# LinXueyuanStdio/LaTeX_OCR

Measured on NVIDIA H100. Metric: formula-images/sec (train step, 128x512 px, seq<=150), higher is better.
Workload: dtype bf16

## Files before the change

### include/latex_ocr_b200.h

```cpp
#ifndef LATEX_OCR_B200_H
#define LATEX_OCR_B200_H

#include <stdint.h>

#ifdef __cplusplus
extern "C" {
#endif

#define LO_F32 0
#define LO_BF16 1

#define LO_OK 0
#define LO_EINVAL (-1)
#define LO_ECUDA (-2)
#define LO_ENOTSUP (-3)

#define LO_IMPL_SIMT 0
#define LO_IMPL_TC 1

int lo_version(void);
const char* lo_last_error(void);
int64_t lo_launch_count(void);
int lo_set_option(const char* name, int value);
int lo_get_option(const char* name);
const char* lo_option_name(int i);
int lo_set_l2_window(const void* base, int64_t bytes, float hit_ratio, void* stream);
int lo_debug_buffer(void* p);
int lo_tc_available(void);

int lo_gemm(const void* A, int dtA, const void* B, int dtB, void* C, int dtC,
            int M, int N, int K,
            int64_t sam, int64_t sak, int64_t sbk, int64_t sbn, int64_t ldc,
            int batch, int64_t sA, int64_t sB, int64_t sC,
            const float* bias, int accumulate, int relu, int impl, void* stream);

int lo_colsum(const void* X, int dt, float* out, int M, int N, int64_t ld, int accumulate, void* stream);

int lo_conv1_pool_forward(const float* img, const float* w, const float* bias, void* out, int dt,
                          int N, int H, int W, void* stream);
int lo_conv1_pool_forward_u8(const uint8_t* img, const float* w, const float* bias, void* out, int dt,
                             int N, int H, int W, void* stream);
int lo_conv1_pool_wgrad_u8(const uint8_t* img, const float* w, const float* bias, const void* dpool, int dt,
                           float* dw, float* db, int N, int H, int W, void* stream);
int lo_conv1_pool_wgrad(const float* img, const float* w, const float* bias, const void* dpool, int dt,
                        float* dw, float* db, int N, int H, int W, void* stream);
int lo_conv1_pool_forward_norm(const void* img, int img_is_u8, float scale, float offset, const float* w,
                               const float* bias, void* out, int dt, int N, int H, int W, void* stream);
int lo_conv1_pool_wgrad_norm(const void* img, int img_is_u8, float scale, float offset, const float* w,
                             const float* bias, const void* dpool, int dt, float* dw, float* db, int N, int H, int W,
                             void* stream);
int lo_conv1_pool_forward_code(const void* img, int img_is_u8, float scale, float offset, const float* w, const float* bias,
                               void* out, uint8_t* code, int dt, int N, int H, int W, void* stream);
int lo_conv1_pool_wgrad_code(const void* img, int img_is_u8, float scale, float offset, const uint8_t* code, const void* dpool,
                             int dt, float* dw, float* db, int N, int H, int W, void* stream);
int lo_conv1_pool_dgrad_code(const uint8_t* code, const void* dpool, int dt, const float* w, float scale, float* dimg,
                             int N, int H, int W, void* stream);
int lo_im2col(const void* x, void* col, int dt, int N, int H, int W, int C, int R, int S, int stride, int pad,
              void* stream);
int lo_col2im(const void* dcol, const void* mask, void* dx, int dt, int N, int H, int W, int C, int R, int S,
              int stride, int pad, void* stream);
int lo_transpose(const void* in, int64_t ld_in, void* out, int64_t ld_out, int dt, int K, int N, void* stream);
int lo_conv3x3(const void* x, const void* w, const float* bias, const void* mask, void* y, int dt,
               int N, int H, int W, int Cin, int Cout, int pad, int relu, int impl, void* stream);
int lo_conv3x3_wgrad(const void* x, const void* dy, float* dw, float* db, int dt,
                     int N, int H, int W, int Cin, int Cout, int pad, int impl, void* stream);
int lo_conv_weight_flip(const void* w, void* wt, int dt, int Cin, int Cout, void* stream);
int lo_maxpool_forward(const void* x, void* y, int dt, int N, int H, int W, int C, int kh, int kw, void* stream);
int lo_maxpool_backward(const void* x, const void* y, const void* dy, void* dx, int dt,
                        int N, int H, int W, int C, int kh, int kw, void* stream);
int lo_add_table(const void* y, const float* table, void* out, int dt, int N, int64_t HWC, void* stream);
int lo_relu_mask_cast(const float* g, const void* y, void* out, int dt, int64_t n, void* stream);

int64_t lo_attention_workspace_bytes(int B, int C);
int64_t lo_decoder_workspace_bytes(int B, int C);
int lo_attention_forward(const void* att1, const void* enc, int dt, const float* att2, int64_t att2_stride,
                         const float* wf, float* alpha, int64_t alpha_stride, float* ctx,
                         float* gate_pre, int64_t gate_stride, float* gctx,
                         int B, int R, int A, int C, void* work, void* stream);
int lo_attention_forward_mask(const void* att1, const void* enc, int dt, const float* att2, int64_t att2_stride,
                              const float* wf, float* alpha, int64_t alpha_stride, float* ctx,
                              float* gate_pre, int64_t gate_stride, float* gctx, uint8_t* relu_mask_out,
                              int B, int R, int A, int C, void* work, void* stream);

int lo_attention_backward(const void* att1, const void* enc, int dt, const float* att2, const float* gate, int64_t o1_stride,
                          const float* wf, const float* alpha, int64_t alpha_stride, const float* ctx, const float* dgctx,
                          int64_t dg_stride, const float* dreg, int64_t dreg_stride, const float* sreg, int64_t sreg_stride,
                          float* de, float* datt2, float* dgp, int64_t dcat_stride, float* dctx_out, float* dwf_part,
                          const uint8_t* relu_mask, int B, int R, int A, int C, void* work, void* stream);

int64_t lo_attention_step_workspace_bytes(int B, int R, int A, int C, int dt);
int lo_attention_step_backward(const void* enc, const void* att1, int dt, const float* h, const float* att2, const void* w_enc,
                               const void* w_dec, const float* wf, const float* alpha, const float* ctx, const float* dctx,
                               const float* dalpha, float* denc, float* dh, float* g_w_enc, float* g_b_enc, float* g_w_dec,
                               float* g_b_dec, float* g_w_full, float* g_b_full, float* de, float* datt2, void* datt1,
                               int B, int R, int A, int C, int D, int impl, void* work, void* stream);

typedef struct lo_decoder_args {
  int32_t B, T, R, C, A, D, E, V;
  int32_t dt;
  int32_t impl;
  int32_t has_dropout;
  int32_t ldl;
  float alpha_c;
  int32_t rows_per_img;
  int32_t phase;
  const int32_t* bt_host;
  const int64_t* caps;
  int64_t caps_stride;
  int64_t* fed;
  const float* ss_prob;
  const float* ss_u;
  const float* ss_temp;
  const float* ss_gu;
  const void* enc;
  const void* w_enc_att; const float* b_enc_att;
  const void* wcat1; const float* bcat1;
  const float* w_full;
  const void* emb;
  const void* w_ih; const float* b_ih;
  const void* w_init; const float* b_init;
  const void* w_fc; const float* b_fc;
  void* wbwd1;
  void* wbwd2;
  void* att1;
  float* ptab;
  float* mean;
  float* hall;
  float* call;
  float* out1;
  float* alphas;
  uint8_t* att_mask;
  float* ctx;
  float* gctx;
  float* gates;
  float* gtmp;
  const float* dropout_mask;
  const uint64_t* dropout_state;
  float dropout_p;
  float* hd;
  float* logits;
  float* row_loss;
  float* loss;
  float* dlogits;
  float* dhd;
  float* dreg;
  const float* dalpha_ext;
  const float* dpred_ext;
  int64_t dpred_stride;
  float* sreg;
  float* dcat;
  float* dxh;
  float* dc;
  float* dctx;
  float* de;
  float* dptab;
  void* datt1;
  float* denc;
  float* dinit;
  float* dmean;
  float* g_w_enc_att; float* g_b_enc_att;
  float* g_wcat1; float* g_bcat1;
  float* g_w_full; float* g_b_full;
  float* g_emb;
  float* g_w_ih; float* g_b_ih;
  float* g_w_init; float* g_b_init;
  float* g_w_fc; float* g_b_fc;
  const int32_t* reg_off;
  const int32_t* reg_off_host;
  void* work;
  void* bfwork;
} lo_decoder_args;

int64_t lo_decoder_bfwork_bytes(const lo_decoder_args* a);
int64_t lo_sizeof_decoder_args(void);
int lo_decoder_forward(const lo_decoder_args* a, int with_loss, void* stream);
int lo_decoder_backward(const lo_decoder_args* a, void* stream);
int lo_decoder_pack_bwd_weights(const lo_decoder_args* a, void* stream);

int lo_decoder_greedy(const lo_decoder_args* a, int64_t start_id, int64_t end_id, int max_steps,
                      int64_t* tokens, int32_t* finished, void* stream);
int lo_decoder_greedy_hist(const lo_decoder_args* a, int64_t start_id, int64_t end_id, int max_steps,
                           int64_t* tokens, int32_t* finished, int32_t* fin_hist, void* stream);

int lo_decoder_beam(const lo_decoder_args* a, int64_t start_id, int64_t end_id, int max_steps, int64_t* ids,
                    int64_t* parents, int32_t* fin_hist, float* logp, void* stream);
int lo_decoder_beam_div(const lo_decoder_args* a, int64_t start_id, int64_t end_id, int max_steps, int64_t* ids,
                        int64_t* parents, int32_t* fin_hist, float* logp, float div_gamma, float div_prob,
                        const float* div_u, const uint64_t* div_state, void* stream);

int lo_scst_edit_reward(const int64_t* hyp, int64_t hyp_stride, int Lh, const int64_t* greedy, int64_t greedy_stride, int Lg,
                        const int64_t* ref, int64_t ref_stride, int Lr, int B, int64_t end_id, float* r_sample, float* r_greedy,
                        float* adv, int32_t* n_len, void* stream);
int lo_scst_pg_grad(const float* preds, int64_t pred_stride, const int64_t* fed, int64_t fed_stride, const float* adv,
                    const int32_t* n_len, const float* temp, const float* r_sample, const float* r_greedy, int B, int T, int V,
                    float* dpred, int64_t dpred_stride, float* partial, float* stats, void* stream);
int lo_scst_edit_reward_tf(const int64_t* hyp, int64_t hyp_stride, int Lh, const int64_t* greedy, int64_t greedy_stride, int Lg,
                           const int64_t* ref, int64_t ref_stride, int Lr, int B, int64_t end_id, float* r_sample, float* r_greedy,
                           float* adv, int32_t* n_len, void* stream);
int lo_scst_pg_grad_tf(const float* logits, int64_t ldl, const int64_t* fed, int64_t fed_stride, const float* adv,
                       const int32_t* n_len, const float* temp, const float* r_sample, const float* r_greedy, int B, int T, int V,
                       float* dpred, int64_t dpred_stride, float* partial, float* stats, void* stream);

typedef struct lo_tfdec_args {
  int32_t B, T, R, C, A, D, O, E, V;
  int32_t dt;
  int32_t impl;
  int32_t ldl;
  int32_t rows_per_img;
  float inv_n_words;
  const void* enc;
  const int64_t* formula;
  int64_t formula_stride;
  const int32_t* lengths;
  const float* keep_h;
  const float* keep_o;
  const void* w_img;
  const void* w_cat2;
  const float* beta;
  const void* w_lstm;
  const float* b_lstm;
  const void* w_oc;
  const void* w_y;
  const void* w_init;
  const float* b_init;
  const void* emb;
  float* g_w_img; float* g_w_cat2; float* g_beta; float* g_w_lstm; float* g_b_lstm; float* g_w_oc; float* g_w_y;
  float* g_w_init; float* g_b_init; float* g_emb;
  float* logits;
  float* alphas;
  uint8_t* att_mask;
  float* loss;
  float* denc;
  int64_t* fed;
  const float* ss_prob;
  const float* ss_u;
  const float* ss_temp;
  const float* ss_gu;
  const uint64_t* ss_state;
  const int32_t* reg_off;
  const int32_t* reg_off_host;
  void* ws;
  const float* dlogits_ext;
  int64_t dlogits_stride;
  const float* dalpha_ext;
} lo_tfdec_args;

int64_t lo_sizeof_tfdec_args(void);
int64_t lo_tfdec_workspace_bytes(const lo_tfdec_args* a);
int lo_tfdec_forward(const lo_tfdec_args* a, int with_loss, void* stream);
int lo_tfdec_backward(const lo_tfdec_args* a, void* stream);
int lo_tfdec_greedy(const lo_tfdec_args* a, int64_t end_id, int max_steps, int64_t* tokens, int32_t* fin_hist, void* stream);
int lo_tfdec_beam(const lo_tfdec_args* a, int64_t end_id, int max_steps, int64_t* ids, int64_t* parents, int32_t* fin_hist,
                  float* logp, void* stream);
int lo_tfdec_beam_div(const lo_tfdec_args* a, int64_t end_id, int max_steps, int64_t* ids, int64_t* parents, int32_t* fin_hist,
                      float* logp, float div_gamma, float div_prob, const float* div_u, const uint64_t* div_state, void* stream);

typedef struct lo_lstm_seq_args {
  int32_t S, M, I, H;
  int32_t dt;
  int32_t impl;
  int32_t reverse;
  int32_t dx_accumulate;
  const void* x;
  int64_t x_row, x_step;
  const void* w_ih;
  const void* w_hh;
  const float* b_ih; const float* b_hh;
  const float* h0; const float* c0;
  float* hs;
  void* hs_st;
  int64_t hs_row, hs_step;
  const float* dhs;
  float* dx;
  int64_t dx_row, dx_step;
  float* g_w_ih; float* g_w_hh; float* g_b_ih; float* g_b_hh;
  float* dh0; float* dc0;
  void* ws;
} lo_lstm_seq_args;
int64_t lo_sizeof_lstm_seq_args(void);
int64_t lo_lstm_seq_workspace_bytes(const lo_lstm_seq_args* a);
int lo_lstm_seq_forward(const lo_lstm_seq_args* a, void* stream);
int lo_lstm_seq_backward(const lo_lstm_seq_args* a, void* stream);

int lo_adam_step(float* p, const float* g, float* m, float* v, void* shadow_bf16, int64_t n,
                 float* state_dev, float beta1, float beta2, float eps, float grad_scale, void* stream);
int lo_adam_step_ranges(float* p, const float* g, float* m, float* v, void* shadow_bf16, const int64_t* ranges,
                        int n_ranges, float* state_dev, float beta1, float beta2, float eps, float grad_scale,
                        void* stream);
int lo_tf_optim_step(int kind, float* p, const float* g, float* s1, float* s2, void* shadow_bf16, int64_t n,
                     float* state_dev, float beta1, float beta2, float eps, float grad_scale, void* stream);
int lo_cast(const void* src, int dt_src, void* dst, int dt_dst, int64_t n, void* stream);

#ifdef __cplusplus
}
#endif
#endif
```

### latex_ocr_b200/csrc/lo_common.cuh

```cuda
#pragma once
#include <cuda_runtime.h>
#include <cuda_bf16.h>
#include <stdint.h>
#include <stdio.h>
#include <string.h>

#include "../../include/latex_ocr_b200.h"

typedef __nv_bfloat16 bf16;

namespace lo {

extern char g_err[512];
extern int64_t g_launches;

inline int fail(int code, const char* fmt, const char* a = "", long b = 0, long c = 0) {
  snprintf(g_err, sizeof(g_err), fmt, a, b, c);
  return code;
}

#define LO_CHECK_ARG(cond, what)                                                        \
  do {                                                                                  \
    if (!(cond)) return lo::fail(LO_EINVAL, "%s: invalid argument: " what " (line %ld)", __func__, __LINE__); \
  } while (0)

#define LO_CUDA(call)                                                                   \
  do {                                                                                  \
    cudaError_t e__ = (call);                                                           \
    if (e__ != cudaSuccess)                                                             \
      return lo::fail(LO_ECUDA, "%s: CUDA error %ld at line %ld", cudaGetErrorString(e__), (long)e__, __LINE__); \
  } while (0)

#define LO_LAUNCH_OK()                                                                  \
  do {                                                                                  \
    lo::g_launches++;                                                                   \
    cudaError_t e__ = cudaGetLastError();                                               \
    if (e__ != cudaSuccess)                                                             \
      return lo::fail(LO_ECUDA, "%s: launch failed (%ld) at line %ld", cudaGetErrorString(e__), (long)e__, __LINE__); \
  } while (0)

#define LO_TRY(call)                                                                    \
  do {                                                                                  \
    int r__ = (call);                                                                   \
    if (r__ != LO_OK) return r__;                                                       \
  } while (0)

inline int cdiv(long a, long b) { return (int)((a + b - 1) / b); }

constexpr int LO_NUM_SMS = 132;

#define LO_OPTIONS(X)                                                                                           \
  X(g_opt_att_pipe, "att_pipe", 1)                 \
  X(g_opt_pdl, "pdl", 1)                                                   \
  X(g_opt_att_abi_pdl, "att_abi_pdl", 0)             \
  X(g_opt_att_l2_keep_mb, "att_l2_keep_mb", 24)    \
  X(g_opt_att_nsplit, "att_nsplit", 0)                       \
  X(g_opt_att_cluster, "att_cluster", 1)                      \
  X(g_opt_att_maskbits, "att_maskbits", 1)                 \
  X(g_opt_att_bwd_mma, "att_bwd_mma", 1)                     \
  X(g_opt_dec_streams, "dec_streams", 1)             \
  X(g_opt_dec_fuse, "dec_fuse", 0)                                        \
  X(g_opt_dec_fuse_bwd, "dec_fuse_bwd", 0)                               \
  X(g_opt_dec_cl, "dec_cl", 0)                                                 \
  X(g_opt_dec_cl_bwd, "dec_cl_bwd", 0)                                        \
  X(g_opt_fuse_lstm, "fuse_lstm", 0)                               \
  X(g_opt_skinny_mma, "skinny_mma", 1)                               \
  X(g_opt_skinny_tma, "skinny_tma", 1)                                    \
  X(g_opt_skinny8, "skinny8", 1)                                        \
  X(g_opt_conv_persist, "conv_persist", 1)                      \
  X(g_opt_conv_mt2, "conv_mt2", 1)                            \
  X(g_opt_conv_mc, "conv_mc", 1)                                     \
  X(g_opt_wgrad256, "wgrad256", 0)                                   \
  X(g_opt_det, "deterministic", 0)                                             \
  X(g_opt_dbg_skip, "dbg_skip", 0)                                  \
  X(g_opt_l2_persist_mb, "l2_persist_mb", 0)

#define LO_OPTION_EXTERN(var, name, def) extern int var;
LO_OPTIONS(LO_OPTION_EXTERN)
#undef LO_OPTION_EXTERN

template <typename... KArgs, typename... Args>
inline cudaError_t launch_pdl(void (*kernel)(KArgs...), dim3 grid, dim3 block, size_t smem, cudaStream_t st, Args... args) {
  cudaLaunchConfig_t cfg{};
  cfg.gridDim = grid;
  cfg.blockDim = block;
  cfg.dynamicSmemBytes = smem;
  cfg.stream = st;
  cudaLaunchAttribute attr[1];
  attr[0].id = cudaLaunchAttributeProgrammaticStreamSerialization;
  attr[0].val.programmaticStreamSerializationAllowed = 1;
  cfg.attrs = attr;
  cfg.numAttrs = g_opt_pdl ? 1 : 0;
  return cudaLaunchKernelEx(&cfg, kernel, KArgs(args)...);
}
template <typename... KArgs, typename... Args>
inline cudaError_t launch_cluster(void (*kernel)(KArgs...), dim3 grid, dim3 block, size_t smem, cudaStream_t st, dim3 cl, bool pdl,
                                  Args... args) {
  cudaLaunchConfig_t cfg{};
  cfg.gridDim = grid;
  cfg.blockDim = block;
  cfg.dynamicSmemBytes = smem;
  cfg.stream = st;
  cudaLaunchAttribute attr[2];
  int n = 0;
  attr[n].id = cudaLaunchAttributeClusterDimension;
  attr[n].val.clusterDim.x = cl.x;
  attr[n].val.clusterDim.y = cl.y;
  attr[n].val.clusterDim.z = cl.z;
  n++;
  if (pdl && g_opt_pdl) {
    attr[n].id = cudaLaunchAttributeProgrammaticStreamSerialization;
    attr[n].val.programmaticStreamSerializationAllowed = 1;
    n++;
  }
  cfg.attrs = attr;
  cfg.numAttrs = n;
  return cudaLaunchKernelEx(&cfg, kernel, KArgs(args)...);
}

__device__ __forceinline__ float ldf(const float* p) { return *p; }
__device__ __forceinline__ float ldf(const bf16* p) { return __bfloat162float(*p); }
__device__ __forceinline__ void stf(float* p, float v) { *p = v; }
__device__ __forceinline__ void stf(bf16* p, float v) { *p = __float2bfloat16_rn(v); }
__device__ __forceinline__ float roundto(float v, const float*) { return v; }
__device__ __forceinline__ float roundto(float v, const bf16*) { return __bfloat162float(__float2bfloat16_rn(v)); }

__device__ __forceinline__ void ld8(const float* p, float* v) {
  float4 a = *reinterpret_cast<const float4*>(p);
  float4 b = *reinterpret_cast<const float4*>(p + 4);
  v[0] = a.x; v[1] = a.y; v[2] = a.z; v[3] = a.w; v[4] = b.x; v[5] = b.y; v[6] = b.z; v[7] = b.w;
}
__device__ __forceinline__ void ld8(const bf16* p, float* v) {
  uint4 u = *reinterpret_cast<const uint4*>(p);
  const uint32_t w[4] = {u.x, u.y, u.z, u.w};
#pragma unroll
  for (int i = 0; i < 4; i++) {
    v[2 * i] = __uint_as_float(w[i] << 16);
    v[2 * i + 1] = __uint_as_float(w[i] & 0xffff0000u);
  }
}
__device__ __forceinline__ void lds8(uint32_t saddr, float* v, const float*) {
  float4 a, b;
  asm volatile("ld.shared.v4.f32 {%0, %1, %2, %3}, [%4];" : "=f"(a.x), "=f"(a.y), "=f"(a.z), "=f"(a.w) : "r"(saddr));
  asm volatile("ld.shared.v4.f32 {%0, %1, %2, %3}, [%4];" : "=f"(b.x), "=f"(b.y), "=f"(b.z), "=f"(b.w) : "r"(saddr + 16));
  v[0] = a.x; v[1] = a.y; v[2] = a.z; v[3] = a.w; v[4] = b.x; v[5] = b.y; v[6] = b.z; v[7] = b.w;
}
__device__ __forceinline__ void lds8(uint32_t saddr, float* v, const bf16*) {
  uint32_t w[4];
  asm volatile("ld.shared.v4.b32 {%0, %1, %2, %3}, [%4];" : "=r"(w[0]), "=r"(w[1]), "=r"(w[2]), "=r"(w[3]) : "r"(saddr));
#pragma unroll
  for (int i = 0; i < 4; i++) {
    v[2 * i] = __uint_as_float(w[i] << 16);
    v[2 * i + 1] = __uint_as_float(w[i] & 0xffff0000u);
  }
}
__device__ __forceinline__ void st8(float* p, const float* v) {
  *reinterpret_cast<float4*>(p) = make_float4(v[0], v[1], v[2], v[3]);
  *reinterpret_cast<float4*>(p + 4) = make_float4(v[4], v[5], v[6], v[7]);
}
__device__ __forceinline__ void st8(bf16* p, const float* v) {
  uint32_t w[4];
#pragma unroll
  for (int i = 0; i < 4; i++) {
    __nv_bfloat162 h = __floats2bfloat162_rn(v[2 * i], v[2 * i + 1]);
    w[i] = *reinterpret_cast<uint32_t*>(&h);
  }
  *reinterpret_cast<uint4*>(p) = make_uint4(w[0], w[1], w[2], w[3]);
}

__device__ __forceinline__ float warp_sum(float v) {
#pragma unroll
  for (int o = 16; o > 0; o >>= 1) v += __shfl_xor_sync(0xffffffffu, v, o);
  return v;
}
__device__ __forceinline__ float warp_max(float v) {
#pragma unroll
  for (int o = 16; o > 0; o >>= 1) v = fmaxf(v, __shfl_xor_sync(0xffffffffu, v, o));
  return v;
}
__device__ __forceinline__ float sigmoidf_(float x) { return 1.0f / (1.0f + expf(-x)); }

__device__ __forceinline__ uint4 philox4x32_10(uint4 c, uint2 k) {
#pragma unroll
  for (int r = 0; r < 10; r++) {
    const uint32_t hi0 = __umulhi(0xD2511F53u, c.x), lo0 = 0xD2511F53u * c.x;
    const uint32_t hi1 = __umulhi(0xCD9E8D57u, c.z), lo1 = 0xCD9E8D57u * c.z;
    c = make_uint4(hi1 ^ c.y ^ k.x, lo1, hi0 ^ c.w ^ k.y, lo0);
    k.x += 0x9E3779B9u;
    k.y += 0xBB67AE85u;
  }
  return c;
}
__device__ __forceinline__ float u01(uint32_t x) { return (float)(x >> 8) * (1.0f / 16777216.0f); }
__device__ __forceinline__ float philox_dropout_mult(const unsigned long long* state, int b, int t, int j, float p, float scale) {
  const unsigned long long seed = state[0], call = state[1];
  const uint4 r = philox4x32_10(make_uint4((uint32_t)(j >> 2), (uint32_t)t, (uint32_t)b, (uint32_t)call),
                                make_uint2((uint32_t)seed, (uint32_t)(seed >> 32)));
  const uint32_t w = (j & 3) == 0 ? r.x : ((j & 3) == 1 ? r.y : ((j & 3) == 2 ? r.z : r.w));
  return u01(w) >= p ? scale : 0.f;
}

#define LO_DISPATCH_DT(dt, T, ...)                   \
  do {                                               \
    if ((dt) == LO_F32) { typedef float T; __VA_ARGS__; } \
    else if ((dt) == LO_BF16) { typedef bf16 T; __VA_ARGS__; } \
    else return lo::fail(LO_EINVAL, "%s: bad dtype %ld", __func__, (long)(dt)); \
  } while (0)

struct GemmDesc {
  int M, N, K;
  int64_t sam, sak, sbk, sbn, ldc;
  int batch;
  int64_t sA, sB, sC;
  const float* bias;
  int accumulate, relu;
};
int gemm(const void* A, int dtA, const void* B, int dtB, void* C, int dtC, const GemmDesc& d, int impl, cudaStream_t st);
int gemm_nt(const void* A, int dtA, int64_t lda, const void* W, int dtW, int64_t ldw, void* C, int dtC, int64_t ldc,
            int M, int N, int K, const float* bias, int accumulate, int relu, int impl, cudaStream_t st);
int gemm_tn(const void* A, int dtA, int64_t lda, const void* B, int dtB, int64_t ldb, void* C, int dtC, int64_t ldc,
            int M, int N, int K, int accumulate, int impl, cudaStream_t st);
int gemm_nn(const void* A, int dtA, int64_t lda, const void* B, int dtB, int64_t ldb, void* C, int dtC, int64_t ldc,
            int M, int N, int K, int accumulate, int impl, cudaStream_t st);
int colsum(const void* X, int dt, float* out, int M, int N, int64_t ld, int accumulate, cudaStream_t st);

struct AttFwdArgs {
  const void *att1, *enc;
  const float* att2; int64_t att2_stride;
  const float* wf;
  float* alpha; int64_t alpha_stride;
  float* ctx; float* gate_pre; int64_t gate_stride; float* gctx; bf16* gctx_bf;
  int B, R;
  void* work;
  int rows_per_img;
  int nsplit_hint;
  int act;
  int a_ch;
  uint8_t* mask_out;
  int abi = 0;
};
struct AttBwdArgs {
  const void *att1, *enc;
  const float *att2, *gate; int64_t o1_stride;
  const float* wf; const float* alpha; int64_t alpha_stride;
  const float* ctx; const float* dgctx; int64_t dg_stride;
  const float* dreg; int64_t dreg_stride; const float* sreg; int64_t sreg_stride;
  float* de; float* datt2; float* dgp; int64_t dcat_stride; bf16* datt2_bf; bf16* dgp_bf; float* dctx_out;
  int B, R;
  void* work;
  float* dwf_part;
  int nsplit_hint;
  int act;
  int a_ch;
  const uint8_t* mask_in;
  int abi = 0;
  void* datt1 = nullptr;
  int ordered_dwf = 0;
};
int attention_fwd_pipe(const AttFwdArgs& x, int dt, int C, cudaStream_t st);
int attention_bwd_pipe(const AttBwdArgs& x, int dt, int C, cudaStream_t st);
inline int64_t att_partials_offset(int B) { return B <= 1024 ? 4096 : ((int64_t)B * 4 + 255) / 256 * 256; }
struct AttRagged {
  const int32_t* reg_off;
  const int32_t* reg_off_host;
  void* map;
  int ctas;
};
int64_t attention_ragged_map_bytes(int B);
int attention_ragged_prepare(AttRagged& rg, int B, int rpi, cudaStream_t st);
int attention_fwd_ragged(const AttFwdArgs& x, const AttRagged& rg, int dt, int C, cudaStream_t st);

bool tc_available();
int tc_gemm_nt(const bf16* A, int64_t lda, const bf16* W, int64_t ldw, void* C, int dtC, int64_t ldc,
               int M, int N, int K, const float* bias, int accumulate, int relu, cudaStream_t st);
int tc_gemm_nt_ex(const bf16* A, int64_t lda, const bf16* W, int64_t ldw, void* C, int dtC, int64_t ldc, int M, int N, int K,
                  const float* bias, int accumulate, int relu, int splits, int atomic_acc, int small_n_tile, cudaStream_t st);
struct TcLstmEpi {
  const float* ptab; const int64_t* tok; int64_t tok_stride;
  const float* hh; int64_t hh_stride;
  const float* c_prev; float* gates; float* c_out; float* h_out; bf16* h_bf;
  float* hd; int64_t hd_stride; const float* dmask;
  int D, V;
  const unsigned long long* dstate; float dp; int row0, t_idx;
};
struct DecStepFwd {
  const bf16* gctx; int64_t ld_gctx;
  const bf16* wil; int64_t ld_wil;
  TcLstmEpi e;
  const bf16* wcat; int64_t ld_wcat;
  const float* bcat; float* o1_next; int64_t ld_o1; int N2;
  unsigned int* bar; unsigned int bar_target;
  int M, K;
};
int dec_step_fwd(const DecStepFwd& p, cudaStream_t st);
struct DecStepBwd {
  const bf16* dcat_a; int64_t ld_dcat;
  const bf16* wbwd2; int64_t ld_w2; int K2;
  int Ma;
  const float* dhd; int64_t dhd_stride; const float* dmask; const unsigned long long* dstate; float dp; int t_idx;
  float* dc; const float* gates; const float* c_prev; const float* c_cur;
  float* dG; bf16* dG_bf; int64_t dG_stride;
  const bf16* wbwd1; int64_t ld_w1; int K1;
  int Mb;
  float* dxh; int C, D;
  unsigned int* bar; unsigned int bar_target;
};
int dec_step_bwd(const DecStepBwd& p, cudaStream_t st);
bool dec_cl_fwd_ok(int D, int C, int N2);
bool dec_cl_bwd_ok(int D, int C, int A);
int dec_cl_fwd(const DecStepFwd& p, cudaStream_t st);
int dec_cl_bwd(const DecStepBwd& p, cudaStream_t st);
int cl_set_ts(long long* p);
int sk_set_ts(long long* p);
int tc_gemm_nt_lstm(const bf16* A, int64_t lda, const bf16* Wil, int64_t ldw, int M, int D, int K, const TcLstmEpi& e, cudaStream_t st);
int skinny_gemm_nt_lstm(const bf16* A, int64_t lda, const bf16* Wil, int64_t ldw, int M, int D, int K, const TcLstmEpi& e, cudaStream_t st);
int skinny_gemm_nt(const bf16* A, int64_t lda, const bf16* W, int64_t ldw, float* C, int64_t ldc, int M, int N, int K, const float* bias,
                   int splits, int atomic_acc, cudaStream_t st);
int tc_gemm_tn(const bf16* A, int64_t lda, const bf16* B, int64_t ldb, float* C, int64_t ldc, int M, int N, int K, cudaStream_t st);
int tc_gemm_tn_batched(const bf16* A, int64_t sAk, int64_t sAb, const bf16* B, int64_t sBk, int64_t sBb, float* C, int64_t ldc,
                       int64_t sCb, int M, int N, int K, int batch, cudaStream_t st);
int tc_conv3x3_wgrad(const bf16* x, const bf16* dy, float* dw, int N, int H, int W, int Cin, int Cout, int pad, cudaStream_t st);
int tc_conv3x3(const bf16* x, const bf16* w, const float* bias, const bf16* mask, bf16* y,
               int N, int H, int W, int Cin, int Cout, int pad, int relu, cudaStream_t st);

}
```

### latex_ocr_b200/csrc/lo_conv.cu

```cuda
#include "lo_common.cuh"

namespace lo {

__device__ __forceinline__ float ldpix(const float* p) { return *p; }
__device__ __forceinline__ float ldpix(const uint8_t* p) { return (float)*p; }

template <typename T, typename TI>
__global__ void __launch_bounds__(256) conv1_pool_fwd_kernel(const TI* __restrict__ img, const float* __restrict__ w,
                                                              const float* __restrict__ bias, T* __restrict__ out,
                                                              int N, int H, int W, float pscale, float poff,
                                                              uint8_t* __restrict__ code) {
  __shared__ float sw[64 * 9];
  __shared__ float sb[64];
  for (int i = threadIdx.x; i < 64 * 9; i += blockDim.x) sw[i] = w[i];
  if (threadIdx.x < 64) sb[threadIdx.x] = bias[threadIdx.x];
  __syncthreads();
  const int Hp = H / 2, Wp = W / 2;
  const int64_t total = (int64_t)N * Hp * Wp * 8;
  for (int64_t idx = blockIdx.x * (int64_t)blockDim.x + threadIdx.x; idx < total; idx += (int64_t)gridDim.x * blockDim.x) {
    const int cg = (int)(idx & 7);
    int64_t p = idx >> 3;
    const int wo = (int)(p % Wp); p /= Wp;
    const int ho = (int)(p % Hp);
    const int n = (int)(p / Hp);
// ... 198 lines not shown
#pragma unroll
    for (int a = 0; a < 2; a++) {
      const int ho = ((y + 1) >> 1) - 1 + a;
      if (ho < 0 || ho >= Hp) continue;
#pragma unroll
      for (int b = 0; b < 2; b++) {
        const int wo = ((x + 1) >> 1) - 1 + b;
        if (wo < 0 || wo >= Wp) continue;
        s += patch[((ho - h0 + 1) * C1D_EW + (wo - w0 + 1)) * C1D_PS + (y - 2 * ho + 1) * 4 + (x - 2 * wo + 1)];
      }
    }
    dimg[((int64_t)n * H + y) * W + x] = s * scale;
  }
}

template <typename T, typename TI>
__global__ void __launch_bounds__(256) conv1_pool_wgrad_kernel(const TI* __restrict__ img, const float* __restrict__ w,
                                                                const float* __restrict__ bias, const T* __restrict__ dpool,
                                                                float* __restrict__ dw, float* __restrict__ db,
                                                                int N, int H, int W, float pscale, float poff, int ordered) {
  __shared__ float sw[64 * 9];
  __shared__ float sb[64];
  for (int i = threadIdx.x; i < 64 * 9; i += blockDim.x) sw[i] = w[i];
  if (threadIdx.x < 64) sb[threadIdx.x] = bias[threadIdx.x];
  __syncthreads();
  const int Hp = H / 2, Wp = W / 2;
  const int lane = threadIdx.x & 31, cg = threadIdx.x >> 5;
  const int64_t npos = (int64_t)N * Hp * Wp;
  float gw[8][9];
  float gb[8];
#pragma unroll
  for (int c = 0; c < 8; c++) {
    gb[c] = 0.f;
#pragma unroll
    for (int k = 0; k < 9; k++) gw[c][k] = 0.f;
  }
  for (int64_t p0 = (int64_t)blockIdx.x * 32; p0 < npos; p0 += (int64_t)gridDim.x * 32) {
    const int64_t pp = p0 + lane;
    if (pp >= npos) continue;
    int64_t p = pp;
    const int wo = (int)(p % Wp); p /= Wp;
    const int ho = (int)(p % Hp);
    const int n = (int)(p / Hp);
    float x[4][4];
    const TI* ib = img + (int64_t)n * H * W;
#pragma unroll
    for (int dy = 0; dy < 4; dy++) {
      const int hi = 2 * ho - 1 + dy;
#pragma unroll
      for (int dx = 0; dx < 4; dx++) {
        const int wi = 2 * wo - 1 + dx;
        x[dy][dx] = (hi >= 0 && hi < H && wi >= 0 && wi < W) ? fmaf(ldpix(ib + (int64_t)hi * W + wi), pscale, poff) : 0.f;
      }
    }
    float g[8];
    ld8(dpool + pp * 64 + cg * 8, g);
#pragma unroll
    for (int c = 0; c < 8; c++) {
      const float* wc = sw + (cg * 8 + c) * 9;
      float best = -INFINITY;
      int bi = 0;
#pragma unroll
      for (int py = 0; py < 2; py++)
#pragma unroll
        for (int px = 0; px < 2; px++) {
          float s = sb[cg * 8 + c];
#pragma unroll
          for (int r = 0; r < 3; r++)
#pragma unroll
            for (int q = 0; q < 3; q++) s = fmaf(wc[r * 3 + q], x[py + r][px + q], s);
          if (s > best) { best = s; bi = py * 2 + px; }
        }
      const float gg = (best > 0.f) ? g[c] : 0.f;
      gb[c] += gg;
#pragma unroll
      for (int py = 0; py < 2; py++)
#pragma unroll
        for (int px = 0; px < 2; px++) {
          const float sel = (bi == py * 2 + px) ? gg : 0.f;
#pragma unroll
          for (int r = 0; r < 3; r++)
#pragma unroll
            for (int q = 0; q < 3; q++) gw[c][r * 3 + q] = fmaf(sel, x[py + r][px + q], gw[c][r * 3 + q]);
        }
    }
  }
  conv1_wgrad_block_partial(gw, gb, cg, lane, dw, db, ordered);
}

template <typename T>
__global__ void __launch_bounds__(256) conv3x3_igemm_kernel(const T* __restrict__ x, const T* __restrict__ w,
                                                             const float* __restrict__ bias, const T* __restrict__ mask,
                                                             T* __restrict__ y, int N, int H, int W, int Cin, int Cout,
                                                             int pad, int relu) {
  constexpr int BM = 64, BN = 64, BK = 16;
  __shared__ __align__(16) float As[BK][BM + 4];
  __shared__ __align__(16) float Bs[BK][BN + 4];
  const int Ho = H + 2 * pad - 2, Wo = W + 2 * pad - 2;
  const int64_t Mtot = (int64_t)N * Ho * Wo;
  const int K = 9 * Cin;
  const int tid = threadIdx.x;
  const int tx = tid % 16, ty = tid / 16;
  const int64_t m0 = (int64_t)blockIdx.y * BM;
  const int n0 = blockIdx.x * BN;
  const int lk = tid % BK;
  int a_h[4], a_w[4];
  int64_t a_img[4];
  bool a_ok[4];
#pragma unroll
  for (int j = 0; j < 4; j++) {
    const int64_t m = m0 + tid / BK + 16 * j;
    a_ok[j] = m < Mtot;
    int64_t p = a_ok[j] ? m : 0;
    a_w[j] = (int)(p % Wo); p /= Wo;
    a_h[j] = (int)(p % Ho);
    a_img[j] = (p / Ho) * (int64_t)H * W;
  }
  float acc[4][4];
#pragma unroll
  for (int i = 0; i < 4; i++)
#pragma unroll
    for (int j = 0; j < 4; j++) acc[i][j] = 0.f;

  for (int k0 = 0; k0 < K; k0 += BK) {
    const int tap = k0 / Cin, ci0 = k0 % Cin;
    const int r = tap / 3 - pad, s = tap % 3 - pad;
#pragma unroll
    for (int j = 0; j < 4; j++) {
      const int hi = a_h[j] + r, wi = a_w[j] + s;
      float v = 0.f;
      if (a_ok[j] && hi >= 0 && hi < H && wi >= 0 && wi < W)
        v = ldf(x + (a_img[j] + (int64_t)hi * W + wi) * Cin + ci0 + lk);
      As[lk][tid / BK + 16 * j] = v;
    }
#pragma unroll
    for (int j = 0; j < 4; j++) {
      const int n = tid / BK + 16 * j;
      float v = 0.f;
      if (n0 + n < Cout) v = ldf(w + (int64_t)(n0 + n) * K + k0 + lk);
      Bs[lk][n] = v;
    }
    __syncthreads();
#pragma unroll
    for (int k = 0; k < BK; k++) {
      const float4 a = *reinterpret_cast<const float4*>(&As[k][ty * 4]);
      const float4 b = *reinterpret_cast<const float4*>(&Bs[k][tx * 4]);
      const float av[4] = {a.x, a.y, a.z, a.w}, bv[4] = {b.x, b.y, b.z, b.w};
#pragma unroll
      for (int i = 0; i < 4; i++)
#pragma unroll
        for (int j = 0; j < 4; j++) acc[i][j] = fmaf(av[i], bv[j], acc[i][j]);
    }
    __syncthreads();
  }
#pragma unroll
  for (int i = 0; i < 4; i++) {
    const int64_t m = m0 + ty * 4 + i;
    if (m >= Mtot) continue;
#pragma unroll
    for (int j = 0; j < 4; j++) {
      const int n = n0 + tx * 4 + j;
      if (n >= Cout) continue;
      float v = acc[i][j];
      if (bias) v += bias[n];
      if (relu) v = fmaxf(v, 0.f);
      if (mask && !(ldf(mask + m * Cout + n) > 0.f)) v = 0.f;
      stf(y + m * Cout + n, v);
    }
  }
}

template <typename T>
__global__ void __launch_bounds__(256) conv3x3_wgrad_kernel(const T* __restrict__ x, const T* __restrict__ dy,
                                                             float* __restrict__ dw, int N, int H, int W, int Cin, int Cout,
                                                             int pad, int splits) {
  constexpr int BM = 64, BN = 64, BK = 16;
  __shared__ __align__(16) float As[BK][BM + 4];
  __shared__ __align__(16) float Bs[BK][BN + 4];
  const int Ho = H + 2 * pad - 2, Wo = W + 2 * pad - 2;
  const int64_t P = (int64_t)N * Ho * Wo;
  const int tap = blockIdx.z / splits, sp = blockIdx.z % splits;
  const int r = tap / 3 - pad, s = tap % 3 - pad;
  const int64_t per = ((P + splits - 1) / splits + BK - 1) / BK * BK;
  const int64_t pbeg = sp * per, pend = min(P, pbeg + per);
  const int tid = threadIdx.x, tx = tid % 16, ty = tid / 16;
  const int co0 = blockIdx.y * BM, ci0 = blockIdx.x * BN;
  const int lc = tid % 64;
  const int lp = tid / 64;
  float acc[4][4];
#pragma unroll
  for (int i = 0; i < 4; i++)
#pragma unroll
    for (int j = 0; j < 4; j++) acc[i][j] = 0.f;
  for (int64_t p0 = pbeg; p0 < pend; p0 += BK) {
#pragma unroll
    for (int j = 0; j < 4; j++) {
      const int kk = lp + 4 * j;
      const int64_t pos = p0 + kk;
      float va = 0.f, vb = 0.f;
      if (pos < pend) {
        if (co0 + lc < Cout) va = ldf(dy + pos * Cout + co0 + lc);
        int64_t q = pos;
        const int wo = (int)(q % Wo); q /= Wo;
        const int ho = (int)(q % Ho);
        const int64_t n = q / Ho;
        const int hi = ho + r, wi = wo + s;
        if (hi >= 0 && hi < H && wi >= 0 && wi < W && ci0 + lc < Cin)
          vb = ldf(x + ((n * H + hi) * W + wi) * Cin + ci0 + lc);
      }
      As[kk][lc] = va;
      Bs[kk][lc] = vb;
    }
    __syncthreads();
#pragma unroll
    for (int k = 0; k < BK; k++) {
      const float4 a = *reinterpret_cast<const float4*>(&As[k][ty * 4]);
      const float4 b = *reinterpret_cast<const float4*>(&Bs[k][tx * 4]);
      const float av[4] = {a.x, a.y, a.z, a.w}, bv[4] = {b.x, b.y, b.z, b.w};
#pragma unroll
      for (int i = 0; i < 4; i++)
#pragma unroll
        for (int j = 0; j < 4; j++) acc[i][j] = fmaf(av[i], bv[j], acc[i][j]);
    }
    __syncthreads();
  }
#pragma unroll
  for (int i = 0; i < 4; i++) {
    const int co = co0 + ty * 4 + i;
    if (co >= Cout) continue;
#pragma unroll
    for (int j = 0; j < 4; j++) {
      const int ci = ci0 + tx * 4 + j;
      if (ci >= Cin) continue;
      atomicAdd(dw + ((int64_t)co * 9 + tap) * Cin + ci, acc[i][j]);
    }
  }
}

template <typename T>
__global__ void weight_flip_kernel(const T* __restrict__ w, T* __restrict__ wt, int Cin, int Cout) {
  const int64_t total = (int64_t)Cin * 9 * Cout;
  for (int64_t i = blockIdx.x * (int64_t)blockDim.x + threadIdx.x; i < total; i += (int64_t)gridDim.x * blockDim.x) {
    const int co = (int)(i % Cout);
    int64_t q = i / Cout;
    const int tap = (int)(q % 9);
    const int ci = (int)(q / 9);
    wt[i] = w[((int64_t)co * 9 + (8 - tap)) * Cin + ci];
  }
}

template <typename T>
__global__ void maxpool_fwd_kernel(const T* __restrict__ x, T* __restrict__ y, int N, int H, int W, int C, int kh, int kw) {
  const int Ho = H / kh, Wo = W / kw, C8 = C / 8;
  const int64_t total = (int64_t)N * Ho * Wo * C8;
  for (int64_t idx = blockIdx.x * (int64_t)blockDim.x + threadIdx.x; idx < total; idx += (int64_t)gridDim.x * blockDim.x) {
    const int c8 = (int)(idx % C8);
    int64_t p = idx / C8;
    const int wo = (int)(p % Wo); p /= Wo;
    const int ho = (int)(p % Ho);
    const int64_t n = p / Ho;
    float best[8];
#pragma unroll
    for (int c = 0; c < 8; c++) best[c] = -INFINITY;
    for (int a = 0; a < kh; a++)
      for (int b = 0; b < kw; b++) {
        float v[8];
        ld8(x + ((n * H + ho * kh + a) * W + wo * kw + b) * C + c8 * 8, v);
#pragma unroll
        for (int c = 0; c < 8; c++) best[c] = fmaxf(best[c], v[c]);
      }
    st8(y + ((n * Ho + ho) * Wo + wo) * C + c8 * 8, best);
  }
}

template <typename T>
__global__ void maxpool_bwd_kernel(const T* __restrict__ x, const T* __restrict__ dy, T* __restrict__ dx,
                                   int N, int H, int W, int C, int kh, int kw) {
  const int Ho = H / kh, Wo = W / kw, C8 = C / 8;
  const int64_t total = (int64_t)N * Ho * Wo * C8;
  for (int64_t idx = blockIdx.x * (int64_t)blockDim.x + threadIdx.x; idx < total; idx += (int64_t)gridDim.x * blockDim.x) {
    const int c8 = (int)(idx % C8);
    int64_t p = idx / C8;
    const int wo = (int)(p % Wo); p /= Wo;
    const int ho = (int)(p % Ho);
    const int64_t n = p / Ho;
    float g[8], best[8];
    int bi[8];
    ld8(dy + ((n * Ho + ho) * Wo + wo) * C + c8 * 8, g);
#pragma unroll
    for (int c = 0; c < 8; c++) { best[c] = -INFINITY; bi[c] = 0; }
    for (int a = 0; a < kh; a++)
      for (int b = 0; b < kw; b++) {
        float v[8];
        ld8(x + ((n * H + ho * kh + a) * W + wo * kw + b) * C + c8 * 8, v);
#pragma unroll
        for (int c = 0; c < 8; c++)
          if (v[c] > best[c]) { best[c] = v[c]; bi[c] = a * kw + b; }
      }
    for (int a = 0; a < kh; a++)
      for (int b = 0; b < kw; b++) {
        float o[8];
#pragma unroll
        for (int c = 0; c < 8; c++) o[c] = (bi[c] == a * kw + b && best[c] > 0.f) ? g[c] : 0.f;
        st8(dx + ((n * H + ho * kh + a) * W + wo * kw + b) * C + c8 * 8, o);
      }
  }
}

template <typename T>
__global__ void add_table_kernel(const T* __restrict__ y, const float* __restrict__ table, T* __restrict__ out,
                                 int64_t total8, int64_t hwc8) {
  for (int64_t i = blockIdx.x * (int64_t)blockDim.x + threadIdx.x; i < total8; i += (int64_t)gridDim.x * blockDim.x) {
    float v[8], t[8];
    ld8(y + i * 8, v);
    ld8(table + (i % hwc8) * 8, t);
#pragma unroll
    for (int c = 0; c < 8; c++) v[c] += t[c];
    st8(out + i * 8, v);
  }
}

template <typename T>
__global__ void relu_mask_cast_kernel(const float* __restrict__ g, const T* __restrict__ y, T* __restrict__ out, int64_t n8) {
  for (int64_t i = blockIdx.x * (int64_t)blockDim.x + threadIdx.x; i < n8; i += (int64_t)gridDim.x * blockDim.x) {
    float a[8], b[8];
    ld8(g + i * 8, a);
    ld8(y + i * 8, b);
#pragma unroll
    for (int c = 0; c < 8; c++) a[c] = b[c] > 0.f ? a[c] : 0.f;
    st8(out + i * 8, a);
  }
}

static inline int grid_for(int64_t work, int threads) {
  int64_t b = (work + threads - 1) / threads;
  const int64_t cap = LO_NUM_SMS * 16;
  return (int)(b < 1 ? 1 : (b > cap ? cap : b));
}


template <typename T>
__global__ void im2col_kernel(const T* __restrict__ x, T* __restrict__ col, int N, int H, int W, int C, int R, int S, int stride,
                              int pad, int Ho, int Wo) {
  const int C8 = C / 8;
  const int64_t total = (int64_t)N * Ho * Wo * R * S * C8;
  for (int64_t i = blockIdx.x * (int64_t)blockDim.x + threadIdx.x; i < total; i += (int64_t)gridDim.x * blockDim.x) {
    const int c8 = (int)(i % C8);
    int64_t q = i / C8;
    const int s = (int)(q % S); q /= S;
    const int r = (int)(q % R); q /= R;
    const int wo = (int)(q % Wo); q /= Wo;
    const int ho = (int)(q % Ho);
    const int n = (int)(q / Ho);
    const int hi = ho * stride - pad + r, wi = wo * stride - pad + s;
    float v[8] = {0.f, 0.f, 0.f, 0.f, 0.f, 0.f, 0.f, 0.f};
    if (hi >= 0 && hi < H && wi >= 0 && wi < W) ld8(x + (((int64_t)n * H + hi) * W + wi) * C + c8 * 8, v);
    st8(col + i * 8, v);
  }
}
template <typename T>
__global__ void col2im_kernel(const T* __restrict__ dcol, const T* __restrict__ mask, T* __restrict__ dx, int N, int H, int W, int C,
                              int R, int S, int stride, int pad, int Ho, int Wo) {
  const int C8 = C / 8;
  const int64_t total = (int64_t)N * H * W * C8;
  for (int64_t i = blockIdx.x * (int64_t)blockDim.x + threadIdx.x; i < total; i += (int64_t)gridDim.x * blockDim.x) {
    const int c8 = (int)(i % C8);
    int64_t q = i / C8;
    const int wi = (int)(q % W); q /= W;
    const int hi = (int)(q % H);
    const int n = (int)(q / H);
    float acc[8] = {0.f, 0.f, 0.f, 0.f, 0.f, 0.f, 0.f, 0.f};
    for (int r = 0; r < R; r++) {
      const int hn = hi + pad - r;
      if (hn < 0 || hn % stride) continue;
      const int ho = hn / stride;
      if (ho >= Ho) continue;
      for (int s2 = 0; s2 < S; s2++) {
        const int wn = wi + pad - s2;
        if (wn < 0 || wn % stride) continue;
        const int wo = wn / stride;
        if (wo >= Wo) continue;
        float v[8];
        ld8(dcol + (((((int64_t)n * Ho + ho) * Wo + wo) * R + r) * S + s2) * C + c8 * 8, v);
#pragma unroll
        for (int k = 0; k < 8; k++) acc[k] += v[k];
      }
    }
    if (mask) {
      float m[8];
      ld8(mask + i * 8, m);
#pragma unroll
      for (int k = 0; k < 8; k++) acc[k] = m[k] > 0.f ? acc[k] : 0.f;
    }
    st8(dx + i * 8, acc);
  }
}
template <typename T>
__global__ void transpose2d_kernel(const T* __restrict__ in, int64_t ld_in, T* __restrict__ out, int64_t ld_out, int K, int Nn) {
  __shared__ float tile[32][33];
  const int k0 = blockIdx.y * 32, n0 = blockIdx.x * 32;
  for (int i = threadIdx.y; i < 32; i += 8)
    if (k0 + i < K && n0 + threadIdx.x < Nn) tile[i][threadIdx.x] = ldf(in + (int64_t)(k0 + i) * ld_in + n0 + threadIdx.x);
  __syncthreads();
  for (int i = threadIdx.y; i < 32; i += 8)
    if (n0 + i < Nn && k0 + threadIdx.x < K) stf(out + (int64_t)(n0 + i) * ld_out + k0 + threadIdx.x, tile[threadIdx.x][i]);
}

}

using namespace lo;

extern "C" {

static int conv1_fwd(const void* img, int u8, const float* w, const float* bias, void* out, int dt, int N, int H, int W, cudaStream_t st,
                     float pscale = 1.f, float poff = 0.f, uint8_t* code = nullptr) {
  LO_CHECK_ARG(img && w && bias && out, "null pointer");
  LO_CHECK_ARG(N > 0 && H >= 2 && W >= 2, "shape");
  const int64_t work = (int64_t)N * (H / 2) * (W / 2) * 8;
  const int grid = grid_for(work, 256);
  if (u8) {
    LO_DISPATCH_DT(dt, T, (conv1_pool_fwd_kernel<T, uint8_t><<<grid, 256, 0, st>>>((const uint8_t*)img, w, bias, (T*)out, N, H, W, pscale, poff, code)));
  } else {
    LO_DISPATCH_DT(dt, T, (conv1_pool_fwd_kernel<T, float><<<grid, 256, 0, st>>>((const float*)img, w, bias, (T*)out, N, H, W, pscale, poff, code)));
  }
  LO_LAUNCH_OK();
  return LO_OK;
}

static int conv1_wgrad(const void* img, int u8, const float* w, const float* bias, const void* dpool, int dt, float* dw, float* db,
                       int N, int H, int W, cudaStream_t st, float pscale = 1.f, float poff = 0.f, const uint8_t* code = nullptr) {
  LO_CHECK_ARG(img && w && bias && dpool && dw && db, "null pointer");
  const int ordered = g_opt_det;
  if (!ordered) {
    LO_CUDA(cudaMemsetAsync(dw, 0, 64 * 9 * sizeof(float), st));
    LO_CUDA(cudaMemsetAsync(db, 0, 64 * sizeof(float), st));
  }
  const int64_t npos = (int64_t)N * (H / 2) * (W / 2);
  int grid = (int)((npos + 31) / 32);
  if (grid > C1_MAXBLOCKS) grid = C1_MAXBLOCKS;
  if (code) {
    if (u8) {
      LO_DISPATCH_DT(dt, T, (conv1_pool_wgrad_code_kernel<T, uint8_t><<<grid, 256, 0, st>>>((const uint8_t*)img, code, (const T*)dpool, dw, db, N, H, W, pscale, poff, ordered)));
    } else {
      LO_DISPATCH_DT(dt, T, (conv1_pool_wgrad_code_kernel<T, float><<<grid, 256, 0, st>>>((const float*)img, code, (const T*)dpool, dw, db, N, H, W, pscale, poff, ordered)));
    }
    LO_LAUNCH_OK();
  } else if (u8) {
    LO_DISPATCH_DT(dt, T, (conv1_pool_wgrad_kernel<T, uint8_t><<<grid, 256, 0, st>>>((const uint8_t*)img, w, bias, (const T*)dpool, dw, db, N, H, W, pscale, poff, ordered)));
    LO_LAUNCH_OK();
  } else {
    LO_DISPATCH_DT(dt, T, (conv1_pool_wgrad_kernel<T, float><<<grid, 256, 0, st>>>((const float*)img, w, bias, (const T*)dpool, dw, db, N, H, W, pscale, poff, ordered)));
    LO_LAUNCH_OK();
  }
  if (ordered) {
    conv1_wgrad_reduce_kernel<<<cdiv(C1_PART, 128), 128, 0, st>>>(dw, db, grid);
    LO_LAUNCH_OK();
  }
  return LO_OK;
}

int lo_conv1_pool_forward(const float* img, const float* w, const float* bias, void* out, int dt, int N, int H, int W,
                          void* stream) {
  return conv1_fwd(img, 0, w, bias, out, dt, N, H, W, (cudaStream_t)stream);
}
int lo_conv1_pool_forward_u8(const uint8_t* img, const float* w, const float* bias, void* out, int dt, int N, int H, int W,
                             void* stream) {
  return conv1_fwd(img, 1, w, bias, out, dt, N, H, W, (cudaStream_t)stream);
}
int lo_conv1_pool_wgrad(const float* img, const float* w, const float* bias, const void* dpool, int dt, float* dw,
                        float* db, int N, int H, int W, void* stream) {
  return conv1_wgrad(img, 0, w, bias, dpool, dt, dw, db, N, H, W, (cudaStream_t)stream);
}
int lo_conv1_pool_wgrad_u8(const uint8_t* img, const float* w, const float* bias, const void* dpool, int dt, float* dw,
                           float* db, int N, int H, int W, void* stream) {
  return conv1_wgrad(img, 1, w, bias, dpool, dt, dw, db, N, H, W, (cudaStream_t)stream);
}

int lo_conv1_pool_forward_norm(const void* img, int img_is_u8, float scale, float offset, const float* w, const float* bias, void* out,
                               int dt, int N, int H, int W, void* stream) {
  return conv1_fwd(img, img_is_u8, w, bias, out, dt, N, H, W, (cudaStream_t)stream, scale, offset);
}
int lo_conv1_pool_forward_code(const void* img, int img_is_u8, float scale, float offset, const float* w, const float* bias, void* out,
                               uint8_t* code, int dt, int N, int H, int W, void* stream) {
  return conv1_fwd(img, img_is_u8, w, bias, out, dt, N, H, W, (cudaStream_t)stream, scale, offset, code);
}
int lo_conv1_pool_wgrad_code(const void* img, int img_is_u8, float scale, float offset, const uint8_t* code, const void* dpool, int dt,
                             float* dw, float* db, int N, int H, int W, void* stream) {
  LO_CHECK_ARG(code, "null code");
  static const float dummy[1] = {0.f};
  return conv1_wgrad(img, img_is_u8, dummy, dummy, dpool, dt, dw, db, N, H, W, (cudaStream_t)stream, scale, offset, code);
}
int lo_conv1_pool_wgrad_norm(const void* img, int img_is_u8, float scale, float offset, const float* w, const float* bias,
                             const void* dpool, int dt, float* dw, float* db, int N, int H, int W, void* stream) {
  return conv1_wgrad(img, img_is_u8, w, bias, dpool, dt, dw, db, N, H, W, (cudaStream_t)stream, scale, offset);
}
int lo_conv1_pool_dgrad_code(const uint8_t* code, const void* dpool, int dt, const float* w, float scale, float* dimg, int N, int H,
                             int W, void* stream) {
  LO_CHECK_ARG(code && dpool && w && dimg, "null pointer");
  LO_CHECK_ARG(dt == LO_F32 || dt == LO_BF16, "dt must be LO_F32 or LO_BF16");
  LO_CHECK_ARG(N >= 1 && H >= 2 && W >= 2, "shape (N >= 1, H >= 2, W >= 2)");
  LO_CHECK_ARG(N <= 65535 && (H / 2 + C1D_TH - 1) / C1D_TH <= 65535, "shape (N or H too large for the grid)");
  cudaStream_t st = (cudaStream_t)stream;
  const dim3 grid(cdiv(W / 2, C1D_TW), cdiv(H / 2, C1D_TH), N);
  LO_DISPATCH_DT(dt, T, (conv1_pool_dgrad_code_kernel<T><<<grid, 256, 0, st>>>(code, (const T*)dpool, w, scale, dimg, H, W)));
  LO_LAUNCH_OK();
  return LO_OK;
}

int lo_im2col(const void* x, void* col, int dt, int N, int H, int W, int C, int R, int S, int stride, int pad, void* stream) {
  LO_CHECK_ARG(x && col && N > 0 && C % 8 == 0 && R > 0 && S > 0 && stride > 0 && pad >= 0, "null pointer / shape (C%8)");
  const int Ho = (H + 2 * pad - R) / stride + 1, Wo = (W + 2 * pad - S) / stride + 1;
  LO_CHECK_ARG(Ho > 0 && Wo > 0, "empty output");
  cudaStream_t st = (cudaStream_t)stream;
  const int64_t work = (int64_t)N * Ho * Wo * R * S * (C / 8);
  LO_DISPATCH_DT(dt, T, (im2col_kernel<T><<<grid_for(work, 256), 256, 0, st>>>((const T*)x, (T*)col, N, H, W, C, R, S, stride, pad, Ho, Wo)));
  LO_LAUNCH_OK();
  return LO_OK;
}
int lo_col2im(const void* dcol, const void* mask, void* dx, int dt, int N, int H, int W, int C, int R, int S, int stride, int pad,
              void* stream) {
  LO_CHECK_ARG(dcol && dx && N > 0 && C % 8 == 0 && R > 0 && S > 0 && stride > 0 && pad >= 0, "null pointer / shape (C%8)");
  const int Ho = (H + 2 * pad - R) / stride + 1, Wo = (W + 2 * pad - S) / stride + 1;
  LO_CHECK_ARG(Ho > 0 && Wo > 0, "empty output");
  cudaStream_t st = (cudaStream_t)stream;
  const int64_t work = (int64_t)N * H * W * (C / 8);
  LO_DISPATCH_DT(dt, T, (col2im_kernel<T><<<grid_for(work, 256), 256, 0, st>>>((const T*)dcol, (const T*)mask, (T*)dx, N, H, W, C, R, S,
                                                                                  stride, pad, Ho, Wo)));
  LO_LAUNCH_OK();
  return LO_OK;
}
int lo_transpose(const void* in, int64_t ld_in, void* out, int64_t ld_out, int dt, int K, int N, void* stream) {
  LO_CHECK_ARG(in && out && K > 0 && N > 0 && ld_in >= N && ld_out >= K, "null pointer / shape");
  cudaStream_t st = (cudaStream_t)stream;
  LO_DISPATCH_DT(dt, T, (transpose2d_kernel<T><<<dim3(cdiv(N, 32), cdiv(K, 32)), dim3(32, 8), 0, st>>>((const T*)in, ld_in, (T*)out, ld_out,
                                                                                                          K, N)));
  LO_LAUNCH_OK();
  return LO_OK;
}

int lo_conv3x3(const void* x, const void* w, const float* bias, const void* mask, void* y, int dt, int N, int H, int W,
               int Cin, int Cout, int pad, int relu, int impl, void* stream) {
  LO_CHECK_ARG(x && w && y, "null pointer");
  LO_CHECK_ARG(pad >= 0 && pad <= 2 && Cin % 16 == 0 && Cout % 8 == 0, "pad in 0..2, Cin%16==0, Cout%8==0");
  LO_CHECK_ARG(H + 2 * pad - 2 > 0 && W + 2 * pad - 2 > 0, "output would be empty");
  cudaStream_t st = (cudaStream_t)stream;
  if (impl == LO_IMPL_TC) {
    LO_CHECK_ARG(dt == LO_BF16, "wgmma path needs bf16 storage");
    if (!tc_available()) return fail(LO_ENOTSUP, "%s: wgmma path requires an sm_90 device", __func__);
    return tc_conv3x3((const bf16*)x, (const bf16*)w, bias, (const bf16*)mask, (bf16*)y, N, H, W, Cin, Cout, pad, relu, st);
  }
  const int Ho = H + 2 * pad - 2, Wo = W + 2 * pad - 2;
  dim3 grid(cdiv(Cout, 64), cdiv((int64_t)N * Ho * Wo, 64));
  LO_DISPATCH_DT(dt, T, (conv3x3_igemm_kernel<T><<<grid, 256, 0, st>>>((const T*)x, (const T*)w, bias, (const T*)mask, (T*)y,
                                                                       N, H, W, Cin, Cout, pad, relu)));
  LO_LAUNCH_OK();
  return LO_OK;
}

int lo_conv3x3_wgrad(const void* x, const void* dy, float* dw, float* db, int dt, int N, int H, int W, int Cin, int Cout,
                     int pad, int impl, void* stream) {
  LO_CHECK_ARG(x && dy && dw, "null pointer");
  LO_CHECK_ARG(pad >= 0 && pad <= 2 && Cin % 8 == 0 && Cout % 8 == 0, "shape");
  cudaStream_t st = (cudaStream_t)stream;
  const int Ho = H + 2 * pad - 2, Wo = W + 2 * pad - 2;
  const int64_t P = (int64_t)N * Ho * Wo;
  LO_CUDA(cudaMemsetAsync(dw, 0, (size_t)Cout * 9 * Cin * sizeof(float), st));
  if (impl == LO_IMPL_TC && dt == LO_BF16 && Cin % 64 == 0 && Cout % 128 == 0 && tc_available()) {
    LO_TRY(tc_conv3x3_wgrad((const bf16*)x, (const bf16*)dy, dw, N, H, W, Cin, Cout, pad, st));
    if (db) LO_TRY(colsum(dy, dt, db, (int)P, Cout, Cout, 0, st));
    return LO_OK;
  }
  const int tiles = 9 * cdiv(Cin, 64) * cdiv(Cout, 64);
  int splits = cdiv(LO_NUM_SMS * 4, tiles);
  const int maxs = (int)((P + 511) / 512);
  if (splits > maxs) splits = maxs;
  if (splits < 1) splits = 1;
  dim3 grid(cdiv(Cin, 64), cdiv(Cout, 64), 9 * splits);
  LO_DISPATCH_DT(dt, T, (conv3x3_wgrad_kernel<T><<<grid, 256, 0, st>>>((const T*)x, (const T*)dy, dw, N, H, W, Cin, Cout, pad, splits)));
  LO_LAUNCH_OK();
  if (db) LO_TRY(colsum(dy, dt, db, (int)P, Cout, Cout, 0, st));
  return LO_OK;
}

int lo_conv_weight_flip(const void* w, void* wt, int dt, int Cin, int Cout, void* stream) {
  LO_CHECK_ARG(w && wt, "null pointer");
  cudaStream_t st = (cudaStream_t)stream;
  const int64_t total = (int64_t)Cin * 9 * Cout;
  LO_DISPATCH_DT(dt, T, (weight_flip_kernel<T><<<grid_for(total, 256), 256, 0, st>>>((const T*)w, (T*)wt, Cin, Cout)));
  LO_LAUNCH_OK();
  return LO_OK;
}

int lo_maxpool_forward(const void* x, void* y, int dt, int N, int H, int W, int C, int kh, int kw, void* stream) {
  LO_CHECK_ARG(x && y && C % 8 == 0 && kh >= 1 && kw >= 1 && H >= kh && W >= kw, "shape");
  cudaStream_t st = (cudaStream_t)stream;
  const int64_t total = (int64_t)N * (H / kh) * (W / kw) * (C / 8);
  LO_DISPATCH_DT(dt, T, (maxpool_fwd_kernel<T><<<grid_for(total, 256), 256, 0, st>>>((const T*)x, (T*)y, N, H, W, C, kh, kw)));
  LO_LAUNCH_OK();
  return LO_OK;
}

int lo_maxpool_backward(const void* x, const void* y, const void* dy, void* dx, int dt, int N, int H, int W, int C, int kh,
                        int kw, void* stream) {
  LO_CHECK_ARG(x && dy && dx && C % 8 == 0 && kh >= 1 && kw >= 1, "shape");
  (void)y;
  cudaStream_t st = (cudaStream_t)stream;
  if (H % kh || W % kw) LO_CUDA(cudaMemsetAsync(dx, 0, (size_t)N * H * W * C * (dt == LO_F32 ? 4 : 2), st));
  const int64_t total = (int64_t)N * (H / kh) * (W / kw) * (C / 8);
  LO_DISPATCH_DT(dt, T, (maxpool_bwd_kernel<T><<<grid_for(total, 256), 256, 0, st>>>((const T*)x, (const T*)dy, (T*)dx, N, H, W, C, kh, kw)));
  LO_LAUNCH_OK();
  return LO_OK;
}

int lo_add_table(const void* y, const float* table, void* out, int dt, int N, int64_t HWC, void* stream) {
  LO_CHECK_ARG(y && table && out && HWC % 8 == 0, "shape");
  cudaStream_t st = (cudaStream_t)stream;
  const int64_t total8 = (int64_t)N * HWC / 8;
  LO_DISPATCH_DT(dt, T, (add_table_kernel<T><<<grid_for(total8, 256), 256, 0, st>>>((const T*)y, table, (T*)out, total8, HWC / 8)));
  LO_LAUNCH_OK();
  return LO_OK;
}

int lo_relu_mask_cast(const float* g, const void* y, void* out, int dt, int64_t n, void* stream) {
  LO_CHECK_ARG(g && y && out && n % 8 == 0, "shape");
  cudaStream_t st = (cudaStream_t)stream;
  LO_DISPATCH_DT(dt, T, (relu_mask_cast_kernel<T><<<grid_for(n / 8, 256), 256, 0, st>>>(g, (const T*)y, (T*)out, n / 8)));
  LO_LAUNCH_OK();
  return LO_OK;
}

}
```

### latex_ocr_b200/csrc/lo_decoder.cu

```cuda
#include "lo_common.cuh"
#include "lo_ptx.cuh"

namespace lo {

#define LO_ATT_THREADS 256
#define LO_ATT_WARPS 8
#define LO_ATT_MAXSPLIT 16

static inline int att_splits(int B) {
  int s = (444 + B - 1) / B;
  if (s < 1) s = 1;
  if (s > LO_ATT_MAXSPLIT) s = LO_ATT_MAXSPLIT;
  return s;
}

__device__ __forceinline__ float ldcg_f(const float* p) { return __ldcg(p); }

template <typename T, int NV>
__global__ void __launch_bounds__(LO_ATT_THREADS) attention_fwd_kernel(
    const T* __restrict__ att1, const T* __restrict__ enc, const float* __restrict__ att2, int64_t att2_stride,
    const float* __restrict__ wf, float* __restrict__ alpha, int64_t alpha_stride, float* __restrict__ ctx,
    float* __restrict__ gate_pre, int64_t gate_stride, float* __restrict__ gctx, bf16* __restrict__ gctx_bf, int R, int nsplit,
    int* __restrict__ counters, float* __restrict__ partials, int rpi) {
  constexpr int CH = NV * 256;
// ... 1565 lines not shown
    if (tc) {
      LO_CUDA(cudaMemsetAsync(g_w_enc, 0, (size_t)A * C * 4, st));
      LO_TRY(tc_gemm_tn((const bf16*)d1, A, (const bf16*)enc, C, g_w_enc, C, A, C, (int)BR, st));
    } else {
      LO_TRY(gemm_tn(d1, dt, A, enc, dt, C, g_w_enc, LO_F32, C, A, C, (int)BR, 0, LO_IMPL_SIMT, st));
    }
  }
  if (g_b_enc) LO_TRY(colsum(d1, dt, g_b_enc, (int)BR, A, A, 0, st));
  if (denc) {
    if (tc) {
      transpose_kernel<bf16><<<dim3(cdiv(C, 32), cdiv(A, 32)), dim3(32, 8), 0, st>>>((const bf16*)w_enc, C, ws_wet, A, A, C);
      LO_LAUNCH_OK();
      LO_TRY(tc_gemm_nt((const bf16*)d1, A, ws_wet, A, denc, LO_F32, C, (int)BR, C, A, nullptr, 0, 0, st));
    } else {
      LO_TRY(gemm_nn(d1, dt, A, w_enc, dt, C, denc, LO_F32, C, (int)BR, C, A, 0, LO_IMPL_SIMT, st));
    }
    add_outer_kernel<<<LO_NUM_SMS * 8, 256, 0, st>>>(denc, alpha, dctx, R, C, BR * C);
    LO_LAUNCH_OK();
  }
  return LO_OK;
}

int lo_decoder_forward(const lo_decoder_args* a, int with_loss, void* stream) {
  LO_TRY(check_args(a));
  LO_TRY(check_reg_off(a, false));
  cudaStream_t st = (cudaStream_t)stream;
  const Dims d = dims(a);
  const bool ragged = a->bt_host[d.T - 1] < d.B;
  const bool sampling = a->ss_prob != nullptr;
  if (ragged && a->phase != 2) {
    LO_CUDA(cudaMemsetAsync(a->alphas, 0, (size_t)d.B * d.T * d.R * 4, st));
    LO_CUDA(cudaMemsetAsync(a->hd, 0, (size_t)d.B * d.T * d.D * 4, st));
    const BfViews bz = bf_views(a, d);
    if (sampling && bz.on) LO_CUDA(cudaMemsetAsync(bz.hd, 0, (size_t)d.B * d.T * d.D * 2, st));
  }
  if (sampling)
    LO_CUDA(cudaMemcpy2DAsync(a->fed, (size_t)d.T * 8, a->caps, (size_t)a->caps_stride * 8, (size_t)d.T * 8, d.B,
                              cudaMemcpyDeviceToDevice, st));
  LO_TRY(upload_dlen(a, st));
  if (a->phase != 2) {
  LO_TRY(forward_prologue(a, d, st));
  const int nchains = two_chains(a, d) && !sampling ? 2 : 1;
  if (nchains == 2) {
    LO_TRY(side_stream_init());
    LO_CUDA(cudaEventRecord(g_ev_fork, st));
    LO_CUDA(cudaStreamWaitEvent(g_side, g_ev_fork, 0));
  }
  const FwdSched sched = pick_fwd(a, d, sampling);
  switch (sched) {
  case FwdSched::Fused:
  case FwdSched::Cluster:
    LO_TRY(fused_forward(a, d, sched, st));
    break;
  case FwdSched::Chains:
    for (int chain = 0; chain < nchains; chain++) {
      cudaStream_t cs = chain == 0 ? st : g_side;
      for (int t = 0; t < d.T; t++) {
        const float* dm = (a->has_dropout == 1 && a->dropout_mask) ? a->dropout_mask + (int64_t)t * d.D : nullptr;
        const Rows rs = chain_rows(a, d, chain, nchains, a->bt_host[t]);
        LO_TRY(forward_step(a, d, t, rs, a->caps + t, a->caps_stride, a->hd + (int64_t)t * d.D, (int64_t)d.T * d.D, dm, cs));
      }
    }
    break;
  }
  if (nchains == 2) {
    LO_CUDA(cudaEventRecord(g_ev_join, g_side));
    LO_CUDA(cudaStreamWaitEvent(st, g_ev_join, 0));
  }
  }
  if (a->phase == 1) return LO_OK;
  if (g_opt_dbg_skip & 8) return LO_OK;
  const BfViews bvf = bf_views(a, d);
  const bool fc_tc = bvf.on && d.Vl % 64 == 0 && d.D % 64 == 0;
  if (sampling) {
  } else if (fc_tc) {
    LO_TRY(lo_cast(a->hd, LO_F32, bvf.hd, LO_BF16, (int64_t)d.B * d.T * d.D, stream));
    LO_TRY(tc_gemm_nt_ex(bvf.hd, d.D, (const bf16*)a->w_fc, d.D, a->logits, LO_F32, d.Vl, d.B * d.T, d.V, d.D, a->b_fc, 0, 0, 1, 0, 0, st));
  } else {
    LO_TRY(gemm_nt(a->hd, LO_F32, d.D, a->w_fc, a->dt, d.D, a->logits, LO_F32, d.Vl, d.B * d.T, d.V, d.D, a->b_fc, 0, 0, LO_IMPL_SIMT, st));
  }
  if (with_loss) {
    long nvalid = 0;
    for (int t = 0; t < d.T; t++) nvalid += a->bt_host[t];
    const float inv_n = 1.0f / (float)nvalid;
    ce_kernel<<<cdiv((long)d.B * d.T, 8), 256, 0, st>>>(a->logits, a->caps, a->caps_stride, work_dlen(a), a->row_loss, a->dlogits,
                                                         (fc_tc && a->dlogits) ? bvf.dlogits : nullptr, d.B, d.T, d.V, d.Vl, inv_n);
    LO_LAUNCH_OK();
    reg_kernel<<<cdiv((long)d.B * d.R, 256), 256, 0, st>>>(a->alphas, a->row_loss + (int64_t)d.B * d.T, a->dreg, d.B, d.T, d.R, a->alpha_c);
    LO_LAUNCH_OK();
    loss_finalize_kernel<<<1, 1024, 0, st>>>(a->row_loss, d.B * d.T, a->row_loss + (int64_t)d.B * d.T, d.B * d.R, inv_n, a->alpha_c, a->loss);
    LO_LAUNCH_OK();
  }
  return LO_OK;
}

int lo_decoder_pack_bwd_weights(const lo_decoder_args* a, void* stream) {
  LO_TRY(check_args(a));
  LO_CHECK_ARG(a->wbwd1 && a->wbwd2, "null pointer");
  cudaStream_t st = (cudaStream_t)stream;
  const Dims d = dims(a);
  const size_t es = a->dt == LO_F32 ? 4 : 2;
  dim3 blk(32, 8);
  const char* w_hh = (const char*)a->wcat1 + (size_t)(d.A + d.C) * d.D * es;
  const char* w_dec = (const char*)a->wcat1;
  const char* w_beta = (const char*)a->wcat1 + (size_t)d.A * d.D * es;
  LO_DISPATCH_DT(a->dt, T, {
    transpose_kernel<T><<<dim3(cdiv(d.C, 32), cdiv(d.G, 32)), blk, 0, st>>>((const T*)a->w_ih + d.E, d.E + d.C, (T*)a->wbwd1, d.G, d.G, d.C);
    transpose_kernel<T><<<dim3(cdiv(d.D, 32), cdiv(d.G, 32)), blk, 0, st>>>((const T*)w_hh, d.D, (T*)a->wbwd1 + (int64_t)d.C * d.G, d.G, d.G, d.D);
    transpose_kernel<T><<<dim3(cdiv(d.D, 32), cdiv(d.A, 32)), blk, 0, st>>>((const T*)w_dec, d.D, (T*)a->wbwd2, d.A + d.C, d.A, d.D);
    transpose_kernel<T><<<dim3(cdiv(d.D, 32), cdiv(d.C, 32)), blk, 0, st>>>((const T*)w_beta, d.D, (T*)a->wbwd2 + d.A, d.A + d.C, d.C, d.D);
  });
  lo::g_launches += 3;
  LO_LAUNCH_OK();
  return LO_OK;
}

int lo_decoder_backward(const lo_decoder_args* a, void* stream) {
  LO_TRY(check_args(a));
  LO_TRY(check_reg_off(a, false));
  LO_CHECK_ARG(!a->dpred_ext || a->dlogits, "dpred_ext needs dlogits");
  LO_CHECK_ARG(!a->dpred_ext || a->dpred_stride >= a->V, "dpred_stride >= V");
  LO_CHECK_ARG(a->phase != 2 || !a->dalpha_ext, "phase 2 reads no d alpha: pass dalpha_ext to the phase-1 call");
  cudaStream_t st = (cudaStream_t)stream;
  const Dims d = dims(a);
  const int dt = a->dt;
  const bool ragged = a->bt_host[d.T - 1] < d.B;
  const int64_t BT = (int64_t)d.B * d.T;
  const bool generic = a->dpred_ext != nullptr;
  const float* dal = a->dalpha_ext ? a->dalpha_ext : (generic ? nullptr : a->dreg);
  const int64_t dal_b = a->dalpha_ext ? (int64_t)d.T * d.R : (dal ? d.R : 0), dal_t = a->dalpha_ext ? d.R : 0;
  const BfViews bvf = bf_views(a, d);
  const bool fc_tc = bvf.on && d.Vl % 64 == 0 && d.D % 64 == 0;
  if (generic && a->phase != 1) {
    dpred_kernel<<<dim3(cdiv(d.Vl, 128), (unsigned)(BT < 65535 ? BT : 65535)), 128, 0, st>>>(
        a->dpred_ext, a->dpred_stride, work_dlen(a), a->dlogits, fc_tc ? bvf.dlogits : nullptr, d.T, d.V, d.Vl, BT, 0);
    LO_LAUNCH_OK();
  }
  if (a->phase != 2) {
    LO_TRY(lo_decoder_pack_bwd_weights(a, stream));
    if (dal) {
      sreg_kernel<<<cdiv(BT, 8), 256, 0, st>>>(a->alphas, dal, dal_b, dal_t, a->sreg, d.B, d.T, d.R);
      LO_LAUNCH_OK();
    } else {
      LO_CUDA(cudaMemsetAsync(a->sreg, 0, (size_t)BT * 4, st));
    }
  }
  if (a->phase == 1) {
  } else if (fc_tc) {
    LO_CUDA(cudaMemsetAsync(a->g_w_fc, 0, (size_t)d.V * d.D * 4, st));
    LO_TRY(tc_gemm_tn(bvf.dlogits, d.Vl, bvf.hd, d.D, a->g_w_fc, d.D, d.V, d.D, (int)BT, st));
    transpose_kernel<bf16><<<dim3(cdiv(d.D, 32), cdiv(d.V, 32)), dim3(32, 8), 0, st>>>((const bf16*)a->w_fc, d.D, bvf.wfct, d.Vl, d.V, d.D);
    LO_LAUNCH_OK();
    LO_TRY(tc_gemm_nt_ex(bvf.dlogits, d.Vl, bvf.wfct, d.Vl, a->dhd, LO_F32, d.D, (int)BT, d.D, d.Vl, nullptr, 0, 0, 1, 0, 0, st));
  } else {
    LO_TRY(gemm_tn(a->dlogits, LO_F32, d.Vl, a->hd, LO_F32, d.D, a->g_w_fc, LO_F32, d.D, d.V, d.D, (int)BT, 0, LO_IMPL_SIMT, st));
    LO_TRY(gemm_nn(a->dlogits, LO_F32, d.Vl, a->w_fc, dt, d.D, a->dhd, LO_F32, d.D, (int)BT, d.D, d.V, 0, LO_IMPL_SIMT, st));
  }
  if (a->phase != 1) LO_TRY(colsum(a->dlogits, LO_F32, a->g_b_fc, (int)BT, d.V, d.Vl, 0, st));
  if (a->phase == 2) return LO_OK;
  LO_CUDA(cudaMemsetAsync(a->dxh, 0, (size_t)d.B * (d.C + d.D) * 4, st));
  LO_CUDA(cudaMemsetAsync(a->dc, 0, (size_t)d.B * d.D * 4, st));
  if (ragged) {
    LO_CUDA(cudaMemsetAsync(a->dcat, 0, (size_t)d.T * d.B * d.O1 * 4, st));
    LO_CUDA(cudaMemsetAsync(a->de, 0, (size_t)BT * d.R * 4, st));
    LO_CUDA(cudaMemsetAsync(a->dctx, 0, (size_t)d.T * d.B * d.C * 4, st));
    const BfViews bz = bf_views(a, d);
    if (bz.on) LO_CUDA(cudaMemsetAsync(bz.dcat, 0, (size_t)d.T * d.B * d.O1 * 2, st));
  }
  const BfViews bv = bf_views(a, d);
  if (g_opt_att_pipe) LO_CUDA(cudaMemsetAsync(a->dmean, 0, (size_t)d.B * d.A * 4, st));
  const int nchains = two_chains(a, d) ? 2 : 1;
  if (nchains == 2) {
    LO_TRY(side_stream_init());
    LO_CUDA(cudaEventRecord(g_ev_fork, st));
    LO_CUDA(cudaStreamWaitEvent(g_side, g_ev_fork, 0));
  }
  const BwdSched sched = pick_bwd(a, d);
  switch (sched) {
  case BwdSched::Fused:
  case BwdSched::Cluster:
    LO_TRY(fused_backward(a, d, sched, dal, dal_b, dal_t, st));
    break;
  case BwdSched::Chains:
    for (int chain = 0; chain < nchains; chain++) {
      cudaStream_t cs = chain == 0 ? st : g_side;
      for (int t = d.T - 1; t >= 0; t--)
        LO_TRY(backward_step(a, d, t, chain_rows(a, d, chain, nchains, a->bt_host[t]), dal, dal_b, dal_t, cs));
    }
    break;
  }
  if (nchains == 2) {
    LO_CUDA(cudaEventRecord(g_ev_join, g_side));
    LO_CUDA(cudaStreamWaitEvent(st, g_ev_join, 0));
  }
  LO_CUDA(cudaMemcpy2DAsync(a->dinit, (size_t)2 * d.D * 4, a->dxh + d.C, (size_t)(d.C + d.D) * 4, (size_t)d.D * 4, d.B,
                            cudaMemcpyDeviceToDevice, st));
  LO_CUDA(cudaMemcpy2DAsync(a->dinit + d.D, (size_t)2 * d.D * 4, a->dc, (size_t)d.D * 4, (size_t)d.D * 4, d.B,
                            cudaMemcpyDeviceToDevice, st));
  if (g_opt_dbg_skip & 1) return LO_OK;
  const bool tc = bv.on;
  bf16* dcat_bf = bv.dcat;
  bf16* hall_bf = bv.hall;
  bf16* gctx_bf = bv.gctx;
  bf16* wet_bf = bv.wet;
  if (tc) {
    LO_CUDA(cudaMemsetAsync(a->g_wcat1, 0, (size_t)d.O1 * d.D * 4, st));
    LO_TRY(tc_gemm_tn(dcat_bf, d.O1, hall_bf, d.D, a->g_wcat1, d.D, d.O1, d.D, d.T * d.B, st));
  } else {
    LO_TRY(gemm_tn(a->dcat, LO_F32, d.O1, a->hall, LO_F32, d.D, a->g_wcat1, LO_F32, d.D, d.O1, d.D, d.T * d.B, 0, LO_IMPL_SIMT, st));
  }
  LO_TRY(colsum(a->dcat, LO_F32, a->g_bcat1, d.T * d.B, d.O1, d.O1, 0, st));
  if (tc) {
    LO_CUDA(cudaMemset2DAsync(a->g_w_ih + d.E, (size_t)(d.E + d.C) * 4, 0, (size_t)d.C * 4, d.G, st));
    LO_TRY(tc_gemm_tn(dcat_bf + d.A + d.C, d.O1, gctx_bf, d.C, a->g_w_ih + d.E, d.E + d.C, d.G, d.C, d.T * d.B, st));
  } else {
    LO_TRY(gemm_tn(a->dcat + d.A + d.C, LO_F32, d.O1, a->gctx, LO_F32, d.C, a->g_w_ih + d.E, LO_F32, d.E + d.C, d.G, d.C, d.T * d.B, 0,
                   LO_IMPL_SIMT, st));
  }
  LO_TRY(colsum(a->dcat + d.A + d.C, LO_F32, a->g_b_ih, d.T * d.B, d.G, d.O1, 0, st));
  const int64_t* in_tok = a->ss_prob ? a->fed : a->caps;
  const int64_t in_stride = a->ss_prob ? (int64_t)d.T : a->caps_stride;
  if (tc) {
    const int Vp = (d.V + 7) / 8 * 8;
    onehot_kernel<<<LO_NUM_SMS * 8, 256, 0, st>>>(in_tok, in_stride, work_dlen(a), bv.onehot, d.B, d.T, Vp);
    LO_LAUNCH_OK();
    LO_CUDA(cudaMemsetAsync(a->dptab, 0, (size_t)d.V * d.G * 4, st));
    LO_TRY(tc_gemm_tn(bv.onehot, Vp, dcat_bf + d.A + d.C, d.O1, a->dptab, d.G, d.V, d.G, d.T * d.B, st));
  } else {
    dim3 grid(cdiv(d.G, 256), d.V);
    dptab_kernel<<<grid, 256, 0, st>>>(a->dcat, d.O1, (int64_t)d.B * d.O1, d.A + d.C, in_tok, in_stride, work_dlen(a), a->dptab,
                                       d.B, d.T, d.G);
    LO_LAUNCH_OK();
  }
  if (tc && d.E % 64 == 0 && d.G % 64 == 0 && d.V >= 64) {
    LO_TRY(lo_cast(a->dptab, LO_F32, bv.dptab, LO_BF16, (int64_t)d.V * d.G, stream));
    transpose_kernel<bf16><<<dim3(cdiv(d.E, 32), cdiv(d.G, 32)), dim3(32, 8), 0, st>>>((const bf16*)a->w_ih, d.E + d.C, bv.wihT, d.G, d.G, d.E);
    LO_LAUNCH_OK();
    LO_TRY(tc_gemm_nt(bv.dptab, d.G, bv.wihT, d.G, a->g_emb, LO_F32, d.E, d.V, d.E, d.G, nullptr, 0, 0, st));
    LO_CUDA(cudaMemset2DAsync(a->g_w_ih, (size_t)(d.E + d.C) * 4, 0, (size_t)d.E * 4, d.G, st));
    LO_TRY(tc_gemm_tn(bv.dptab, d.G, (const bf16*)a->emb, d.E, a->g_w_ih, d.E + d.C, d.G, d.E, d.V, st));
  } else {
    LO_TRY(gemm_nn(a->dptab, LO_F32, d.G, a->w_ih, dt, d.E + d.C, a->g_emb, LO_F32, d.E, d.V, d.E, d.G, 0, LO_IMPL_SIMT, st));
    LO_TRY(gemm_tn(a->dptab, LO_F32, d.G, a->emb, dt, d.E, a->g_w_ih, LO_F32, d.E + d.C, d.G, d.E, d.V, 0, LO_IMPL_SIMT, st));
  }
  LO_CUDA(cudaMemsetAsync(a->g_b_full, 0, 4, st));
  const bool pipe_dwf = g_opt_att_pipe && !att_mask_at(a, 0, 0);
  if (!g_opt_det) {
    dim3 grid(d.A / 64, cdiv(d.R, 32), d.B);
    if (g_opt_att_pipe) {
      LO_TRY(colsum(a->dmean, LO_F32, a->g_w_full, d.B, d.A, d.A, 0, st));
    } else {
      LO_CUDA(cudaMemsetAsync(a->g_w_full, 0, (size_t)d.A * 4, st));
    }
    if (pipe_dwf) {
      LO_DISPATCH_DT(dt, T, (datt1_kernel<T, 0><<<grid, 128, 0, st>>>((const T*)a->att1, a->out1, d.O1, (int64_t)d.B * d.O1, a->de,
                                                                       a->w_full, (T*)a->datt1, nullptr, d.T, d.R, d.A, 1, 0)));
    } else if (g_opt_att_pipe) {
      LO_DISPATCH_DT(dt, T, (datt1_kernel<T, 2><<<grid, 128, 0, st>>>((const T*)a->att1, a->out1, d.O1, (int64_t)d.B * d.O1, a->de,
                                                                       a->w_full, (T*)a->datt1, a->g_w_full, d.T, d.R, d.A, 1, 0)));
    } else {
      LO_DISPATCH_DT(dt, T, (datt1_kernel<T, 1><<<grid, 128, 0, st>>>((const T*)a->att1, a->out1, d.O1, (int64_t)d.B * d.O1, a->de,
                                                                       a->w_full, (T*)a->datt1, a->g_w_full, d.T, d.R, d.A, 1, 0)));
    }
    LO_LAUNCH_OK();
  } else {
    const int nch = cdiv(cdiv(d.R, 32), 16);
    static bool attr = false;
    if (!attr) {
      LO_CUDA(cudaFuncSetAttribute(datt1_kernel<float, 1>, cudaFuncAttributeNonPortableClusterSizeAllowed, 1));
      LO_CUDA(cudaFuncSetAttribute(datt1_kernel<bf16, 1>, cudaFuncAttributeNonPortableClusterSizeAllowed, 1));
      LO_CUDA(cudaFuncSetAttribute(datt1_kernel<float, 2>, cudaFuncAttributeNonPortableClusterSizeAllowed, 1));
      LO_CUDA(cudaFuncSetAttribute(datt1_kernel<bf16, 2>, cudaFuncAttributeNonPortableClusterSizeAllowed, 1));
      attr = true;
    }
    dim3 grid(d.A / 64, cdiv(d.R, 32 * nch), d.B);
    const dim3 cl(1, grid.y, 1);
    if (pipe_dwf) {
      LO_DISPATCH_DT(dt, T, (datt1_kernel<T, 0><<<grid, 128, 0, st>>>((const T*)a->att1, a->out1, d.O1, (int64_t)d.B * d.O1, a->de,
                                                                       a->w_full, (T*)a->datt1, nullptr, d.T, d.R, d.A, nch, 0)));
    } else if (g_opt_att_pipe) {
      LO_DISPATCH_DT(dt, T, LO_CUDA(launch_cluster(datt1_kernel<T, 2>, grid, dim3(128), 0, st, cl, false, (const T*)a->att1,
                                                   (const float*)a->out1, (int64_t)d.O1, (int64_t)d.B * d.O1, (const float*)a->de,
                                                   (const float*)a->w_full, (T*)a->datt1, a->dmean, d.T, d.R, d.A, nch, 1)));
    } else {
      LO_CUDA(cudaMemsetAsync(a->dmean, 0, (size_t)d.B * d.A * 4, st));
      LO_DISPATCH_DT(dt, T, LO_CUDA(launch_cluster(datt1_kernel<T, 1>, grid, dim3(128), 0, st, cl, false, (const T*)a->att1,
                                                   (const float*)a->out1, (int64_t)d.O1, (int64_t)d.B * d.O1, (const float*)a->de,
                                                   (const float*)a->w_full, (T*)a->datt1, a->dmean, d.T, d.R, d.A, nch, 1)));
    }
    LO_LAUNCH_OK();
    LO_TRY(colsum(a->dmean, LO_F32, a->g_w_full, d.B, d.A, d.A, 0, st));
  }
  if (tc) {
    LO_CUDA(cudaMemsetAsync(a->g_w_enc_att, 0, (size_t)d.A * d.C * 4, st));
    LO_TRY(tc_gemm_tn((const bf16*)a->datt1, d.A, (const bf16*)a->enc, d.C, a->g_w_enc_att, d.C, d.A, d.C, d.B * d.R, st));
    transpose_kernel<bf16><<<dim3(cdiv(d.C, 32), cdiv(d.A, 32)), dim3(32, 8), 0, st>>>((const bf16*)a->w_enc_att, d.C, wet_bf, d.A, d.A, d.C);
    LO_LAUNCH_OK();
    LO_TRY(tc_gemm_nt((const bf16*)a->datt1, d.A, wet_bf, d.A, a->denc, LO_F32, d.C, d.B * d.R, d.C, d.A, nullptr, 0, 0, st));
  } else {
    LO_TRY(gemm_tn(a->datt1, dt, d.A, a->enc, dt, d.C, a->g_w_enc_att, LO_F32, d.C, d.A, d.C, d.B * d.R, 0, LO_IMPL_SIMT, st));
    LO_TRY(gemm_nn(a->datt1, dt, d.A, a->w_enc_att, dt, d.C, a->denc, LO_F32, d.C, d.B * d.R, d.C, d.A, 0, LO_IMPL_SIMT, st));
  }
  LO_TRY(colsum(a->datt1, dt, a->g_b_enc_att, d.B * d.R, d.A, d.A, 0, st));
  if (tc && d.C % 8 == 0) {
    const int Rp = (int)rpad8(d.R);
    cast_pad_rows_kernel<<<LO_NUM_SMS * 8, 256, 0, st>>>(a->alphas, bv.alphas, BT, d.R, Rp);
    LO_LAUNCH_OK();
    cast_tb_to_bt_kernel<<<LO_NUM_SMS * 8, 256, 0, st>>>(a->dctx, bv.dctx, d.T, d.B, d.C);
    LO_LAUNCH_OK();
    LO_TRY(tc_gemm_tn_batched(bv.alphas, Rp, (int64_t)d.T * Rp, bv.dctx, d.C, (int64_t)d.T * d.C, a->denc, d.C, (int64_t)d.R * d.C, d.R,
                              d.C, d.T, d.B, st));
  } else {
    GemmDesc g{d.R, d.C, d.T, 1, d.R, (int64_t)d.B * d.C, 1, d.C, d.B, (int64_t)d.T * d.R, d.C, (int64_t)d.R * d.C, nullptr, 1, 0};
    LO_TRY(gemm(a->alphas, LO_F32, a->dctx, LO_F32, a->denc, LO_F32, g, LO_IMPL_SIMT, st));
  }
  LO_TRY(gemm_tn(a->dinit, LO_F32, 2 * d.D, a->mean, LO_F32, d.C, a->g_w_init, LO_F32, d.C, 2 * d.D, d.C, d.B, 0, LO_IMPL_SIMT, st));
  LO_TRY(colsum(a->dinit, LO_F32, a->g_b_init, d.B, 2 * d.D, 2 * d.D, 0, st));
  LO_TRY(gemm_nn(a->dinit, LO_F32, 2 * d.D, a->w_init, dt, d.C, a->dmean, LO_F32, d.C, d.B, d.C, 2 * d.D, 0, LO_IMPL_SIMT, st));
  {
    const int64_t total = (int64_t)d.B * d.R * d.C;
    add_rowbcast_kernel<<<LO_NUM_SMS * 8, 256, 0, st>>>(a->denc, a->dmean, d.R, d.C, 1.0f / (float)d.R, total);
    LO_LAUNCH_OK();
  }
  if (a->has_dropout == 2 || (a->ss_prob && a->dropout_state)) {
    bump_counter_kernel<<<1, 1, 0, st>>>((unsigned long long*)a->dropout_state + 1);
    LO_LAUNCH_OK();
  }
  return LO_OK;
}

int lo_decoder_greedy_hist(const lo_decoder_args* a, int64_t start_id, int64_t end_id, int max_steps, int64_t* tokens,
                           int32_t* finished, int32_t* fin_hist, void* stream) {
  LO_TRY(check_args(a));
  LO_TRY(check_reg_off(a, true));
  LO_CHECK_ARG(!a->ss_prob, "scheduled sampling (ss_prob) is a training mode: greedy decode feeds its own argmax already");
  LO_CHECK_ARG(tokens && finished && max_steps > 0 && max_steps <= a->T, "tokens/finished/max_steps (<= T capacity)");
  cudaStream_t st = (cudaStream_t)stream;
  const Dims d = dims(a);
  int64_t* next_tok = (int64_t*)a->sreg;
  fill_i64_kernel<<<cdiv(d.B, 128), 128, 0, st>>>(next_tok, start_id, d.B);
  LO_LAUNCH_OK();
  LO_CUDA(cudaMemsetAsync(finished, 0, (size_t)d.B * 4, st));
  LO_TRY(forward_prologue(a, d, st));
  AttRagged rg = ragged_of(a);
  if (a->reg_off) LO_TRY(attention_ragged_prepare(rg, d.B, a->rows_per_img > 1 ? a->rows_per_img : 1, st));
  const BfViews bvg = bf_views(a, d);
  for (int t = 0; t < max_steps; t++) {
    LO_TRY(forward_step(a, d, t, Rows{0, d.B, a->work, 0, a->reg_off ? &rg : nullptr}, next_tok, 1, nullptr, 0, nullptr, st));
    const int64_t h_t = (int64_t)(t + 1) * d.B * d.D;
    LO_TRY(head_nt(a, bvg.on, a->hall + h_t, bvg.on ? bvg.hall + h_t : nullptr, d.D, a->logits, d.V, d.B, st));
    argmax_kernel<<<cdiv(d.B, 8), 256, 0, st>>>(a->logits, d.V, tokens + t, max_steps, next_tok, finished, end_id, d.B);
    LO_LAUNCH_OK();
    if (fin_hist) {
      fin_hist_kernel<<<cdiv(d.B, 128), 128, 0, st>>>(finished, fin_hist + t, max_steps, d.B);
      LO_LAUNCH_OK();
    }
  }
  return LO_OK;
}

int lo_decoder_greedy(const lo_decoder_args* a, int64_t start_id, int64_t end_id, int max_steps, int64_t* tokens,
                      int32_t* finished, void* stream) {
  return lo_decoder_greedy_hist(a, start_id, end_id, max_steps, tokens, finished, nullptr, stream);
}

int lo_decoder_beam(const lo_decoder_args* a, int64_t start_id, int64_t end_id, int max_steps, int64_t* ids, int64_t* parents,
                    int32_t* fin_hist, float* logp, void* stream) {
  return lo_decoder_beam_div(a, start_id, end_id, max_steps, ids, parents, fin_hist, logp, 1.f, 0.f, nullptr, nullptr, stream);
}

int lo_decoder_beam_div(const lo_decoder_args* a, int64_t start_id, int64_t end_id, int max_steps, int64_t* ids, int64_t* parents,
                        int32_t* fin_hist, float* logp, float div_gamma, float div_prob, const float* div_u,
                        const uint64_t* div_state, void* stream) {
  LO_TRY(check_args(a));
  LO_TRY(check_reg_off(a, true));
  LO_CHECK_ARG(!a->ss_prob, "scheduled sampling (ss_prob) is a training mode: not available in beam search");
  const bool div_on = !(div_gamma == 1.f || div_prob == 0.f);
  LO_CHECK_ARG(!div_on || (div_gamma > 0.f && (div_u || div_state)), "diversity penalty needs gamma > 0 and div_u or div_state");
  const int beam = a->rows_per_img;
  LO_CHECK_ARG(beam >= 1 && beam <= LO_BEAM_MAX && a->B % beam == 0, "1 <= beam (rows_per_img) <= 16, B % beam == 0");
  LO_CHECK_ARG(ids && parents && fin_hist && logp && max_steps > 0 && max_steps <= a->T, "outputs / max_steps (<= T capacity)");
  LO_CHECK_ARG((size_t)beam * a->V * 4 * (div_on ? 2 : 1) <= 200 * 1024, "beam*V too large for the shared-memory top-k");
  cudaStream_t st = (cudaStream_t)stream;
  const Dims d = dims(a);
  const int n_img = d.B / beam;
  int64_t* next_tok = (int64_t*)a->sreg;
  int32_t* finished = (int32_t*)a->row_loss;
  int32_t* parent_rows = finished + d.B;
  LO_CHECK_ARG((int64_t)d.B * d.T >= 2 * d.B, "row_loss scratch too small");
  fill_i64_kernel<<<cdiv(d.B, 128), 128, 0, st>>>(next_tok, start_id, d.B);
  LO_LAUNCH_OK();
  LO_CUDA(cudaMemsetAsync(finished, 0, (size_t)d.B * 4, st));
  LO_CUDA(cudaMemsetAsync(logp, 0, (size_t)d.B * 4, st));
  LO_TRY(forward_prologue(a, d, st));
  AttRagged rg = ragged_of(a);
  if (a->reg_off) LO_TRY(attention_ragged_prepare(rg, d.B, beam, st));
  const BfViews bv = bf_views(a, d);
  for (int t = 0; t < max_steps; t++) {
    LO_TRY(forward_step(a, d, t, Rows{0, d.B, a->work, 0, a->reg_off ? &rg : nullptr}, next_tok, 1, nullptr, 0, nullptr, st));
    float* h_new = a->hall + (int64_t)(t + 1) * d.B * d.D;
    float* c_new = a->call + (int64_t)(t + 1) * d.B * d.D;
    LO_TRY(head_nt(a, bv.on, h_new, bv.on ? bv.hall + (int64_t)(t + 1) * d.B * d.D : nullptr, d.D, a->logits, d.V, d.B, st));
    LO_TRY(beam_select(a->logits, d.V, beam, n_img, t, max_steps, end_id, logp, finished, ids, parents, fin_hist, next_tok, parent_rows,
                       div_on, div_gamma, div_prob, div_u ? div_u + (int64_t)t * d.B * d.V : nullptr, div_state, st));
    gather_rows_kernel<<<cdiv((long)d.B * d.D, 256), 256, 0, st>>>(h_new, parent_rows, a->gtmp, d.B, d.D);
    LO_LAUNCH_OK();
    gather_rows_kernel<<<cdiv((long)d.B * d.D, 256), 256, 0, st>>>(c_new, parent_rows, a->gtmp + (int64_t)d.B * d.D, d.B, d.D);
    LO_LAUNCH_OK();
    LO_CUDA(cudaMemcpyAsync(h_new, a->gtmp, (size_t)d.B * d.D * 4, cudaMemcpyDeviceToDevice, st));
    LO_CUDA(cudaMemcpyAsync(c_new, a->gtmp + (int64_t)d.B * d.D, (size_t)d.B * d.D * 4, cudaMemcpyDeviceToDevice, st));
    if (bv.on) LO_TRY(lo_cast(h_new, LO_F32, bv.hall + (int64_t)(t + 1) * d.B * d.D, LO_BF16, (int64_t)d.B * d.D, stream));
  }
  return LO_OK;
}

}

#include "lo_tfdecoder.cuh"
#include "lo_lstmseq.cuh"
```

### latex_ocr_b200/csrc/lo_tc.cu

```cuda
#include <cuda.h>

#include <mutex>
#include <unordered_map>

#include "lo_common.cuh"
#include "lo_ptx.cuh"
#include "lo_wgmma.cuh"

namespace lo {

__device__ __forceinline__ void tma_load_2d(void* dst, const CUtensorMap* map, uint64_t* bar, int c0, int c1) {
  asm volatile("cp.async.bulk.tensor.2d.shared::cluster.global.mbarrier::complete_tx::bytes [%0], [%1, {%3, %4}], [%2];" ::"r"(
                   smem_u32(dst)),
               "l"(reinterpret_cast<uint64_t>(map)), "r"(smem_u32(bar)), "r"(c0), "r"(c1)
               : "memory");
}
__device__ __forceinline__ void tma_load_2d_hint(void* dst, const CUtensorMap* map, uint64_t* bar, int c0, int c1, uint64_t policy) {
  asm volatile(
      "cp.async.bulk.tensor.2d.shared::cluster.global.mbarrier::complete_tx::bytes.L2::cache_hint [%0], [%1, {%3, %4}], [%2], %5;" ::"r"(
          smem_u32(dst)),
      "l"(reinterpret_cast<uint64_t>(map)), "r"(smem_u32(bar)), "r"(c0), "r"(c1), "l"(policy)
      : "memory");
}
__device__ __forceinline__ void tma_load_3d(void* dst, const CUtensorMap* map, uint64_t* bar, int c0, int c1, int c2) {
  asm volatile(
      "cp.async.bulk.tensor.3d.shared::cluster.global.mbarrier::complete_tx::bytes [%0], [%1, {%3, %4, %5}], [%2];" ::"r"(
          smem_u32(dst)),
      "l"(reinterpret_cast<uint64_t>(map)), "r"(smem_u32(bar)), "r"(c0), "r"(c1), "r"(c2)
      : "memory");
}
__device__ __forceinline__ void tma_load_4d(void* dst, const CUtensorMap* map, uint64_t* bar, int c0, int c1, int c2, int c3) {
  asm volatile(
      "cp.async.bulk.tensor.4d.shared::cluster.global.mbarrier::complete_tx::bytes [%0], [%1, {%3, %4, %5, %6}], [%2];" ::"r"(
          smem_u32(dst)),
      "l"(reinterpret_cast<uint64_t>(map)), "r"(smem_u32(bar)), "r"(c0), "r"(c1), "r"(c2), "r"(c3)
      : "memory");
}
__device__ __forceinline__ void tma_load_2d_mc(void* dst, const CUtensorMap* map, uint64_t* bar, int c0, int c1, uint16_t mask) {
  asm volatile(
      "cp.async.bulk.tensor.2d.shared::cluster.global.mbarrier::complete_tx::bytes.multicast::cluster [%0], [%1, {%4, %5}], [%2], %3;" ::"r"(
          smem_u32(dst)),
      "l"(reinterpret_cast<uint64_t>(map)), "r"(smem_u32(bar)), "h"(mask), "r"(c0), "r"(c1)
      : "memory");
}
__device__ __forceinline__ void tma_load_4d_mc(void* dst, const CUtensorMap* map, uint64_t* bar, int c0, int c1, int c2, int c3,
                                               uint16_t mask) {
  asm volatile(
      "cp.async.bulk.tensor.4d.shared::cluster.global.mbarrier::complete_tx::bytes.multicast::cluster [%0], [%1, {%4, %5, %6, %7}], [%2], %3;" ::"r"(
          smem_u32(dst)),
      "l"(reinterpret_cast<uint64_t>(map)), "r"(smem_u32(bar)), "h"(mask), "r"(c0), "r"(c1), "r"(c2), "r"(c3)
      : "memory");
}
__device__ __forceinline__ void mbar_arrive_cta(uint64_t* bar, uint32_t cta) {
  uint32_t remote;
  asm volatile("mapa.shared::cluster.u32 %0, %1, %2;" : "=r"(remote) : "r"(smem_u32(bar)), "r"(cta));
  asm volatile("mbarrier.arrive.release.cluster.shared::cluster.b64 _, [%0];" ::"r"(remote) : "memory");
}
__device__ __forceinline__ void cluster_sync_all() {
  asm volatile("barrier.cluster.arrive.release.aligned;\n\tbarrier.cluster.wait.acquire.aligned;" ::: "memory");
}
__device__ __forceinline__ uint32_t cluster_ctarank() {
  uint32_t r;
  asm volatile("mov.u32 %0, %%cluster_ctarank;" : "=r"(r));
  return r;
}
__device__ __forceinline__ void tma_prefetch_desc(const CUtensorMap* map) {
  asm volatile("prefetch.tensormap [%0];" ::"l"(reinterpret_cast<uint64_t>(map)) : "memory");
}

__device__ __forceinline__ uint64_t make_kmajor_sw128_desc(uint32_t saddr) {
  uint64_t d = 0;
  d |= (uint64_t)((saddr & 0x3FFFF) >> 4);
  d |= (uint64_t)1 << 16;
  d |= (uint64_t)(1024 >> 4) << 32;
  d |= (uint64_t)1 << 62;
  return d;
}

struct TcParams {
  int M, N, K;
  int conv;
  int Ho, Wo, Cin, pad;
  int BW, BH, tiles_w, tiles_h;
  const float* bias;
  const bf16* mask;
  void* out;
  int64_t ldc;
  int out_f32, accumulate, relu;
  int kb_per_split, atomic;
  int w_evict_last;
  int half_w, half_h;
  long long* dbg;
  int lstm;
  const float* l_ptab; const int64_t* l_tok; int64_t l_tok_stride;
  const float* l_hh; int64_t l_hh_stride;
  const float* l_cprev; float* l_gates; float* l_c; float* l_h; bf16* l_hbf;
  float* l_hd; int64_t l_hd_stride; const float* l_dmask;
  int l_D, l_V;
};

constexpr int TC_BM = 128, TC_BK = 64;
constexpr int TC_CWARPS = 8;
constexpr int TC_THREADS = (TC_CWARPS + 2) * 32;

template <int NT, int STAGES>
struct TcSmem {
  static constexpr int A_BYTES = TC_BM * TC_BK * 2;
  static constexpr int B_BYTES = NT * TC_BK * 2;
  static constexpr int STAGE_BYTES = A_BYTES + B_BYTES;
  static constexpr int TOTAL = STAGES * STAGE_BYTES + 1024  + 256 ;
};

template <int NT>
__device__ __forceinline__ void tc_mma_kblock(float* acc, uint32_t sa, uint32_t sb, bool first) {
  const uint64_t da = make_kmajor_sw128_desc(sa), db = make_kmajor_sw128_desc(sb);
#pragma unroll
  for (int k = 0; k < TC_BK / 16; k++)
    Wgmma<NT, 0, 0>::mma(acc, da + (uint64_t)(2 * k), db + (uint64_t)(2 * k), (first && k == 0) ? 0u : 1u);
}

__device__ __forceinline__ void tc_store_pair(const TcParams& p, int64_t off, float f0, float f1, bool use_mask) {
  if (p.atomic) {
    float* o = reinterpret_cast<float*>(p.out) + off;
    atomicAdd(o, f0);
    atomicAdd(o + 1, f1);
  } else if (p.out_f32) {
    float2* o = reinterpret_cast<float2*>(reinterpret_cast<float*>(p.out) + off);
    if (p.accumulate) { const float2 old = *o; f0 += old.x; f1 += old.y; }
    if (p.relu) { f0 = fmaxf(f0, 0.f); f1 = fmaxf(f1, 0.f); }
    *o = make_float2(f0, f1);
  } else {
    uint32_t* o = reinterpret_cast<uint32_t*>(reinterpret_cast<bf16*>(p.out) + off);
    if (p.accumulate) { const uint32_t old = *o; f0 += __uint_as_float(old << 16); f1 += __uint_as_float(old & 0xffff0000u); }
    if (p.relu) { f0 = fmaxf(f0, 0.f); f1 = fmaxf(f1, 0.f); }
    if (use_mask) {
      const uint32_t w = *reinterpret_cast<const uint32_t*>(p.mask + off);
      if (!(__uint_as_float(w << 16) > 0.f)) f0 = 0.f;
      if (!(__uint_as_float(w & 0xffff0000u) > 0.f)) f1 = 0.f;
    }
    __nv_bfloat162 h = __floats2bfloat162_rn(f0, f1);
    *o = *reinterpret_cast<uint32_t*>(&h);
  }
}

template <int NT, int STAGES, int MC>
__global__ void __launch_bounds__(TC_THREADS, 1) tc_gemm_conv_kernel(const __grid_constant__ CUtensorMap mapA,
                                                                      const __grid_constant__ CUtensorMap mapB, TcParams p) {
  using SM = TcSmem<NT, STAGES>;
  extern __shared__ uint8_t smem_raw[];
  uint8_t* smem = reinterpret_cast<uint8_t*>((reinterpret_cast<uintptr_t>(smem_raw) + 1023) & ~(uintptr_t)1023);
  uint64_t* full_bar = reinterpret_cast<uint64_t*>(smem + STAGES * SM::STAGE_BYTES);
  uint64_t* empty_bar = full_bar + STAGES;
  __shared__ __align__(16) float s_bias[NT];

  const int warp = threadIdx.x >> 5, lane = threadIdx.x & 31;
  const int n0 = blockIdx.x * NT;
  const int mt = blockIdx.y;
  const int KB_all = p.K / TC_BK;
  const int kb0 = blockIdx.z * p.kb_per_split;
  const int KB = min(KB_all, kb0 + p.kb_per_split) - kb0;

  int img = 0, h0 = 0, w0 = 0, m0 = mt * TC_BM;
  if (p.conv) {
    const int per_img = p.tiles_w * p.tiles_h;
    img = mt / per_img;
    const int rem = mt % per_img;
    h0 = (rem / p.tiles_w) * p.BH;
    w0 = (rem % p.tiles_w) * p.BW;
  }

  const bool dbg = p.dbg && blockIdx.x == 0 && blockIdx.y == 0 && blockIdx.z == 0;
  if (dbg && threadIdx.x == 0) p.dbg[0] = clock64();
  if (warp == TC_CWARPS && lane == 0) {
    tma_prefetch_desc(&mapA);
    tma_prefetch_desc(&mapB);
    for (int s = 0; s < STAGES; s++) {
      mbar_init(full_bar + s, 2);
      mbar_init(empty_bar + s, MC ? 2 * TC_CWARPS : TC_CWARPS);
    }
    fence_barrier_init();
  }
  pdl_wait();
  pdl_trigger();
  if (MC) cluster_sync_all(); else __syncthreads();
  const uint32_t crank = MC ? cluster_ctarank() : 0;
  if (dbg && threadIdx.x == 0) p.dbg[1] = clock64();

  if (warp == TC_CWARPS) {
    if (lane == 0) {
      const int cpb = p.conv ? p.Cin / TC_BK : 1;
      for (int kb = 0; kb < KB; kb++) {
        const int s = kb % STAGES;
        const uint32_t ph = (kb / STAGES) & 1;
        mbar_wait(empty_bar + s, ph ^ 1);
        uint8_t* sa = smem + s * SM::STAGE_BYTES;
        mbar_expect_tx(full_bar + s, SM::A_BYTES);
        const int kg = kb0 + kb;
        if (MC) {
          uint8_t* sh = sa + crank * (SM::A_BYTES / 2);
          if (p.conv) {
            const int tap = kg / cpb, cb = kg % cpb;
            const int r = tap / 3, q = tap % 3;
            tma_load_4d_mc(sh, &mapA, full_bar + s, cb * TC_BK, w0 + (int)crank * p.half_w + q - p.pad,
                           h0 + (int)crank * p.half_h + r - p.pad, img, (uint16_t)3);
          } else {
            tma_load_2d_mc(sh, &mapA, full_bar + s, kg * TC_BK, m0 + (int)crank * (TC_BM / 2), (uint16_t)3);
          }
        } else if (p.conv) {
          const int tap = kg / cpb, cb = kg % cpb;
          const int r = tap / 3, q = tap % 3;
          tma_load_4d(sa, &mapA, full_bar + s, cb * TC_BK, w0 + q - p.pad, h0 + r - p.pad, img);
        } else {
          tma_load_2d(sa, &mapA, full_bar + s, kg * TC_BK, m0);
        }
        if (dbg && kb == 0) p.dbg[2] = clock64();
        if (dbg && kb < 40) p.dbg[64 + kb] = clock64();
      }
      if (dbg) p.dbg[3] = clock64();
    }
    __syncwarp();
  } else if (warp == TC_CWARPS + 1) {
    if (lane == 0) {
      const uint64_t polB = p.w_evict_last ? l2_policy_evict_last() : l2_policy_evict_normal();
      for (int kb = 0; kb < KB; kb++) {
        const int s = kb % STAGES;
        const uint32_t ph = (kb / STAGES) & 1;
        mbar_wait(empty_bar + s, ph ^ 1);
        uint8_t* sb = smem + s * SM::STAGE_BYTES + SM::A_BYTES;
        mbar_expect_tx(full_bar + s, SM::B_BYTES);
        tma_load_2d_hint(sb, &mapB, full_bar + s, (kb0 + kb) * TC_BK, n0, polB);
      }
    }
    __syncwarp();
  } else {
    const int wg = warp >> 2;
    for (int c = threadIdx.x; c < NT; c += TC_CWARPS * 32)
      s_bias[c] = (p.bias && blockIdx.z == 0 && n0 + c < p.N) ? __ldg(p.bias + n0 + c) : 0.f;
    asm volatile("bar.sync 1, 256;" ::: "memory");
    float acc[NT / 2];
    for (int kb = 0; kb < KB; kb++) {
      const int s = kb % STAGES;
      const uint32_t ph = (kb / STAGES) & 1;
      mbar_wait(full_bar + s, ph);
      if (dbg && threadIdx.x == 0 && kb == 0) p.dbg[4] = clock64();
      if (dbg && threadIdx.x == 0 && kb < 40) p.dbg[16 + kb] = clock64();
      const uint32_t sa = smem_u32(smem + s * SM::STAGE_BYTES);
      wgmma_fence();
      tc_mma_kblock<NT>(acc, sa + wg * (SM::A_BYTES / 2), sa + SM::A_BYTES, kb == 0);
      wgmma_commit();
      wgmma_wait0();
      wgmma_acc_fence<NT / 2>(acc);
      __syncwarp();
      if (lane == 0) {
        if (MC) { mbar_arrive_cta(empty_bar + s, 0); mbar_arrive_cta(empty_bar + s, 1); }
        else mbar_arrive(empty_bar + s);
      }
    }
    if (dbg && threadIdx.x == 0) p.dbg[5] = clock64();
    const int rbase = wg * 64 + (warp & 3) * 16 + (lane >> 2);
    const int cq = 2 * (lane & 3);
    if (p.lstm) {
      const int D = p.l_D;
#pragma unroll
      for (int h = 0; h < 2; h++) {
        const int b = m0 + rbase + 8 * h;
#pragma unroll
        for (int i = 0; i < NT / 8; i++) {
          const float a0 = acc[4 * i + 2 * h], a1 = acc[4 * i + 2 * h + 1];
          const float o0 = __shfl_xor_sync(0xffffffffu, a0, 1), o1 = __shfl_xor_sync(0xffffffffu, a1, 1);
          const int j = (n0 + 8 * i + cq) / 4;
          if ((lane & 1) || b >= p.M || j >= D) continue;
          int64_t tk = p.l_tok[(int64_t)b * p.l_tok_stride];
          tk = tk < 0 ? 0 : (tk >= p.l_V ? p.l_V - 1 : tk);
          const float* pt = p.l_ptab + tk * 4 * D;
          const float* hh = p.l_hh + (int64_t)b * p.l_hh_stride;
          const float pi = a0 + pt[j] + hh[j];
          const float pf = a1 + pt[D + j] + hh[D + j];
          const float pg = o0 + pt[2 * D + j] + hh[2 * D + j];
          const float po = o1 + pt[3 * D + j] + hh[3 * D + j];
          const float ig = sigmoidf_(pi), fg = sigmoidf_(pf), gg = tanhf(pg), og = sigmoidf_(po);
          const float cn = fg * p.l_cprev[(int64_t)b * D + j] + ig * gg;
          const float hn = og * tanhf(cn);
          float* gt = p.l_gates + (int64_t)b * 4 * D;
          gt[j] = ig; gt[D + j] = fg; gt[2 * D + j] = gg; gt[3 * D + j] = og;
          p.l_c[(int64_t)b * D + j] = cn;
          p.l_h[(int64_t)b * D + j] = hn;
          if (p.l_hbf) p.l_hbf[(int64_t)b * D + j] = __float2bfloat16_rn(hn);
          if (p.l_hd) p.l_hd[(int64_t)b * p.l_hd_stride + j] = p.l_dmask ? hn * p.l_dmask[(int64_t)b * p.l_hd_stride + j] : hn;
        }
      }
    } else {
      const bool use_mask = p.mask && !p.out_f32 && !p.atomic;
#pragma unroll
      for (int h = 0; h < 2; h++) {
        const int row = rbase + 8 * h;
        bool row_ok;
        int64_t row_off;
        if (p.conv) {
          const int hh = h0 + row / p.BW, ww = w0 + row % p.BW;
          row_ok = (hh < p.Ho) && (ww < p.Wo);
          row_off = (((int64_t)img * p.Ho + hh) * p.Wo + ww) * p.ldc;
        } else {
          row_ok = (m0 + row) < p.M;
          row_off = (int64_t)(m0 + row) * p.ldc;
        }
        if (!row_ok) continue;
#pragma unroll
        for (int i = 0; i < NT / 8; i++) {
          if (n0 + 8 * i >= p.N) continue;
          const int c = 8 * i + cq;
          tc_store_pair(p, row_off + n0 + c, acc[4 * i + 2 * h] + s_bias[c], acc[4 * i + 2 * h + 1] + s_bias[c + 1], use_mask);
        }
      }
    }
    if (dbg && threadIdx.x == 0) p.dbg[6] = clock64();
  }
  if (MC) cluster_sync_all();
  if (dbg && threadIdx.x == 0) p.dbg[7] = clock64();
}

template <int NT, int STAGES, int MT>
struct TcPSmem {
  static constexpr int A_BYTES = TC_BM * TC_BK * 2;
  static constexpr int B_BYTES = NT * TC_BK * 2;
  static constexpr int STAGE_BYTES = MT * A_BYTES + B_BYTES;
  static constexpr int TOTAL = STAGES * STAGE_BYTES + 1024  + 256  + 2 * NT * 4 ;
};

template <int NT, int STAGES, int MT>
__global__ void __launch_bounds__(TC_THREADS, 1) tc_conv_p_kernel(const __grid_constant__ CUtensorMap mapA,
                                                                 const __grid_constant__ CUtensorMap mapB, TcParams p, int ntiles_n,
                                                                 int total_tiles, int mtiles) {
  using SM = TcPSmem<NT, STAGES, MT>;
  static_assert(MT * NT <= 256, "accumulator registers");
  extern __shared__ uint8_t smem_raw[];
  uint8_t* smem = reinterpret_cast<uint8_t*>((reinterpret_cast<uintptr_t>(smem_raw) + 1023) & ~(uintptr_t)1023);
  uint64_t* full_bar = reinterpret_cast<uint64_t*>(smem + STAGES * SM::STAGE_BYTES);
  uint64_t* empty_bar = full_bar + STAGES;
  float* s_bias = reinterpret_cast<float*>(smem + STAGES * SM::STAGE_BYTES + 256);

  const int warp = threadIdx.x >> 5, lane = threadIdx.x & 31;
  const int KB = p.K / TC_BK;
  const int cpb = p.Cin / TC_BK;
  const int per_img = p.tiles_w * p.tiles_h;

  if (warp == TC_CWARPS && lane == 0) {
    tma_prefetch_desc(&mapA);
    tma_prefetch_desc(&mapB);
    for (int s = 0; s < STAGES; s++) {
      mbar_init(full_bar + s, 2);
      mbar_init(empty_bar + s, TC_CWARPS);
    }
    fence_barrier_init();
  }
  pdl_wait();
  pdl_trigger();
  __syncthreads();

  if (warp == TC_CWARPS) {
    if (lane == 0) {
      uint32_t it = 0;
      for (int tile = blockIdx.x; tile < total_tiles; tile += gridDim.x) {
        const int mt0 = (tile / ntiles_n) * MT;
        const int nsub = min(MT, mtiles - mt0);
        int img[MT], h0[MT], w0[MT];
#pragma unroll
        for (int j = 0; j < MT; j++) {
          const int mt = min(mt0 + j, mtiles - 1);
          img[j] = mt / per_img;
          const int rem = mt % per_img;
          h0[j] = (rem / p.tiles_w) * p.BH;
          w0[j] = (rem % p.tiles_w) * p.BW;
        }
        for (int kb = 0; kb < KB; kb++, it++) {
          const int s = it % STAGES;
          const uint32_t ph = (it / STAGES) & 1;
          mbar_wait(empty_bar + s, ph ^ 1);
          mbar_expect_tx(full_bar + s, (uint32_t)nsub * SM::A_BYTES);
          const int tap = kb / cpb, cb = kb % cpb;
          const int r = tap / 3, q = tap % 3;
#pragma unroll
          for (int j = 0; j < MT; j++)
            if (j < nsub)
              tma_load_4d(smem + s * SM::STAGE_BYTES + j * SM::A_BYTES, &mapA, full_bar + s, cb * TC_BK, w0[j] + q - p.pad,
                          h0[j] + r - p.pad, img[j]);
        }
      }
    }
    __syncwarp();
  } else if (warp == TC_CWARPS + 1) {
    if (lane == 0) {
      const uint64_t polB = l2_policy_evict_last();
      uint32_t it = 0;
      for (int tile = blockIdx.x; tile < total_tiles; tile += gridDim.x) {
        const int n0 = (tile % ntiles_n) * NT;
        for (int kb = 0; kb < KB; kb++, it++) {
          const int s = it % STAGES;
          const uint32_t ph = (it / STAGES) & 1;
          mbar_wait(empty_bar + s, ph ^ 1);
          mbar_expect_tx(full_bar + s, SM::B_BYTES);
          tma_load_2d_hint(smem + s * SM::STAGE_BYTES + MT * SM::A_BYTES, &mapB, full_bar + s, kb * TC_BK, n0, polB);
        }
      }
    }
    __syncwarp();
  } else {
    const int wg = warp >> 2;
    const int rbase = wg * 64 + (warp & 3) * 16 + (lane >> 2);
    const int cq = 2 * (lane & 3);
    const bool use_mask = p.mask != nullptr;
    uint32_t it = 0, lt = 0;
    for (int tile = blockIdx.x; tile < total_tiles; tile += gridDim.x, lt++) {
      const int n0 = (tile % ntiles_n) * NT;
      const int mt0 = (tile / ntiles_n) * MT;
      const int nsub = min(MT, mtiles - mt0);
      float* sb = s_bias + (lt & 1) * NT;
      for (int c = threadIdx.x; c < NT; c += TC_CWARPS * 32) sb[c] = (p.bias && n0 + c < p.N) ? __ldg(p.bias + n0 + c) : 0.f;
      asm volatile("bar.sync 1, 256;" ::: "memory");
      float acc[MT][NT / 2];
      for (int kb = 0; kb < KB; kb++, it++) {
        const int s = it % STAGES;
        const uint32_t ph = (it / STAGES) & 1;
        mbar_wait(full_bar + s, ph);
        const uint32_t sa = smem_u32(smem + s * SM::STAGE_BYTES);
        wgmma_fence();
#pragma unroll
        for (int j = 0; j < MT; j++)
          tc_mma_kblock<NT>(acc[j], sa + j * SM::A_BYTES + wg * (SM::A_BYTES / 2), sa + MT * SM::A_BYTES, kb == 0);
        wgmma_commit();
        wgmma_wait0();
#pragma unroll
        for (int j = 0; j < MT; j++) wgmma_acc_fence<NT / 2>(acc[j]);
        __syncwarp();
        if (lane == 0) mbar_arrive(empty_bar + s);
      }
#pragma unroll
      for (int j = 0; j < MT; j++) {
        if (j >= nsub) continue;
        const int mt = mt0 + j;
        const int img = mt / per_img, rem = mt % per_img;
#pragma unroll
        for (int h = 0; h < 2; h++) {
          const int row = rbase + 8 * h;
          const int hh = (rem / p.tiles_w) * p.BH + row / p.BW, ww = (rem % p.tiles_w) * p.BW + row % p.BW;
          if (hh >= p.Ho || ww >= p.Wo) continue;
          const int64_t row_off = (((int64_t)img * p.Ho + hh) * p.Wo + ww) * p.ldc;
#pragma unroll
          for (int i = 0; i < NT / 8; i++) {
            if (n0 + 8 * i >= p.N) continue;
            const int c = 8 * i + cq;
            float f0 = acc[j][4 * i + 2 * h] + sb[c], f1 = acc[j][4 * i + 2 * h + 1] + sb[c + 1];
            if (p.relu) { f0 = fmaxf(f0, 0.f); f1 = fmaxf(f1, 0.f); }
            if (use_mask) {
              const uint32_t w = *reinterpret_cast<const uint32_t*>(p.mask + row_off + n0 + c);
              if (!(__uint_as_float(w << 16) > 0.f)) f0 = 0.f;
              if (!(__uint_as_float(w & 0xffff0000u) > 0.f)) f1 = 0.f;
            }
            __nv_bfloat162 hv = __floats2bfloat162_rn(f0, f1);
            *reinterpret_cast<__nv_bfloat162*>(reinterpret_cast<bf16*>(p.out) + row_off + n0 + c) = hv;
          }
        }
      }
    }
  }
}

__device__ __forceinline__ uint64_t make_mnmajor_sw128_desc(uint32_t saddr, uint32_t lbo_bytes) {
  uint64_t d = 0;
  d |= (uint64_t)((saddr & 0x3FFFF) >> 4);
  d |= (uint64_t)((lbo_bytes >> 4) & 0x3FFF) << 16;
  d |= (uint64_t)(1024 >> 4) << 32;
  d |= (uint64_t)1 << 62;
  return d;
}

struct WgParams {
  int Cin, Cout, Ho, Wo, pad;
  int BW, BH, tiles_w, tiles_h, kstages, per_split, ci_tiles;
  float* dw;
  int plain;
  int64_t ldc;
  int64_t batch_c;
  int ordered;
};

template <int NT, int STAGES>
__global__ void __launch_bounds__(TC_THREADS, 1) tc_wgrad_kernel(const __grid_constant__ CUtensorMap mapDY,
                                                                  const __grid_constant__ CUtensorMap mapX, WgParams p) {
  constexpr int BOX = 128 * 64 * 2;
  constexpr int A_BYTES = 2 * BOX, B_BYTES = (NT / 64) * BOX, STAGE_BYTES = A_BYTES + B_BYTES;
  extern __shared__ uint8_t smem_raw[];
  uint8_t* smem = reinterpret_cast<uint8_t*>((reinterpret_cast<uintptr_t>(smem_raw) + 1023) & ~(uintptr_t)1023);
  uint64_t* full_bar = reinterpret_cast<uint64_t*>(smem + STAGES * STAGE_BYTES);
  uint64_t* empty_bar = full_bar + STAGES;
  const int warp = threadIdx.x >> 5, lane = threadIdx.x & 31;
  const int co0 = (blockIdx.x / p.ci_tiles) * 128, ci0 = (blockIdx.x % p.ci_tiles) * NT;
  const int tap = p.plain == 2 ? 0 : blockIdx.y, r = tap / 3, q = tap % 3;
  const int bz = p.plain == 2 ? blockIdx.y : 0;
  const int ks0 = blockIdx.z * p.per_split;
  const int ks1 = min(p.kstages, ks0 + p.per_split);
  const int KS = ks1 - ks0;
  if (warp == TC_CWARPS && lane == 0) {
    tma_prefetch_desc(&mapDY);
    tma_prefetch_desc(&mapX);
    for (int s = 0; s < STAGES; s++) { mbar_init(full_bar + s, 2); mbar_init(empty_bar + s, TC_CWARPS); }
    fence_barrier_init();
  }
  __syncthreads();
  float acc[NT / 2];
  if (warp == TC_CWARPS) {
    if (lane == 0) {
      const int per_img = p.tiles_w * p.tiles_h;
      for (int i = 0; i < KS; i++) {
        const int s = i % STAGES;
        const uint32_t ph = (i / STAGES) & 1;
        mbar_wait(empty_bar + s, ph ^ 1);
        const int ks = ks0 + i;
        const int img = ks / per_img, rem = ks % per_img;
        const int h0 = (rem / p.tiles_w) * p.BH, w0 = (rem % p.tiles_w) * p.BW;
        uint8_t* sa = smem + s * STAGE_BYTES;
        mbar_expect_tx(full_bar + s, A_BYTES);
        if (p.plain == 2) {
          tma_load_3d(sa, &mapDY, full_bar + s, co0, ks * 128, bz);
          tma_load_3d(sa + BOX, &mapDY, full_bar + s, co0 + 64, ks * 128, bz);
        } else if (p.plain) {
          tma_load_2d(sa, &mapDY, full_bar + s, co0, ks * 128);
          tma_load_2d(sa + BOX, &mapDY, full_bar + s, co0 + 64, ks * 128);
        } else {
          tma_load_4d(sa, &mapDY, full_bar + s, co0, w0, h0, img);
          tma_load_4d(sa + BOX, &mapDY, full_bar + s, co0 + 64, w0, h0, img);
        }
      }
    }
    __syncwarp();
  } else if (warp == TC_CWARPS + 1) {
    if (lane == 0) {
      const int per_img = p.tiles_w * p.tiles_h;
      for (int i = 0; i < KS; i++) {
        const int s = i % STAGES;
        const uint32_t ph = (i / STAGES) & 1;
        mbar_wait(empty_bar + s, ph ^ 1);
        const int ks = ks0 + i;
        const int img = ks / per_img, rem = ks % per_img;
        const int h0 = (rem / p.tiles_w) * p.BH, w0 = (rem % p.tiles_w) * p.BW;
        uint8_t* sb = smem + s * STAGE_BYTES + A_BYTES;
        mbar_expect_tx(full_bar + s, B_BYTES);
        if (p.plain == 2) {
#pragma unroll
          for (int j = 0; j < NT / 64; j++) tma_load_3d(sb + j * BOX, &mapX, full_bar + s, ci0 + 64 * j, ks * 128, bz);
        } else if (p.plain) {
#pragma unroll
          for (int j = 0; j < NT / 64; j++) tma_load_2d(sb + j * BOX, &mapX, full_bar + s, ci0 + 64 * j, ks * 128);
        } else {
#pragma unroll
          for (int j = 0; j < NT / 64; j++)
            tma_load_4d(sb + j * BOX, &mapX, full_bar + s, ci0 + 64 * j, w0 + q - p.pad, h0 + r - p.pad, img);
        }
      }
    }
    __syncwarp();
  } else {
    const int wg = warp >> 2;
#pragma unroll
    for (int i = 0; i < NT / 2; i++) acc[i] = 0.f;
    for (int i = 0; i < KS; i++) {
      const int s = i % STAGES;
      const uint32_t ph = (i / STAGES) & 1;
      mbar_wait(full_bar + s, ph);
      const uint32_t sa = smem_u32(smem + s * STAGE_BYTES) + wg * BOX;
      const uint32_t sb = smem_u32(smem + s * STAGE_BYTES) + A_BYTES;
      wgmma_fence();
#pragma unroll
      for (int k = 0; k < 8; k++)
        Wgmma<NT, 1, 1>::mma(acc, make_mnmajor_sw128_desc(sa + k * 2048, BOX), make_mnmajor_sw128_desc(sb + k * 2048, BOX), 1u);
      wgmma_commit();
      wgmma_wait0();
      wgmma_acc_fence<NT / 2>(acc);
      __syncwarp();
      if (lane == 0) mbar_arrive(empty_bar + s);
    }
  }
  if (p.ordered && gridDim.z > 1) {
    float* part = reinterpret_cast<float*>(smem);
    if (warp < TC_CWARPS) {
      asm volatile("bar.sync 1, 256;" ::: "memory");
#pragma unroll
      for (int i = 0; i < NT / 2; i++) part[i * 256 + threadIdx.x] = acc[i];
    }
    cl_sync();
    if (cl_rank() == 0 && warp < TC_CWARPS) {
#pragma unroll
      for (int i = 0; i < NT / 2; i += 16) cl_sum_n<16>(part + i * 256 + threadIdx.x, 256, acc + i);
    }
    cl_sync();
    if (cl_rank() != 0) return;
  }
  if (warp < TC_CWARPS) {
    const int wg = warp >> 2, cq = 2 * (lane & 3);
#pragma unroll
    for (int h = 0; h < 2; h++) {
      const int co = co0 + wg * 64 + (warp & 3) * 16 + (lane >> 2) + 8 * h;
      if (co >= p.Cout) continue;
      float* orow = p.plain ? p.dw + (int64_t)bz * p.batch_c + (int64_t)co * p.ldc : p.dw + ((int64_t)co * 9 + tap) * p.Cin;
#pragma unroll
      for (int i = 0; i < NT / 8; i++) {
        const int ci = ci0 + 8 * i + cq;
        if (ci < p.Cin) atomicAdd(orow + ci, acc[4 * i + 2 * h]);
        if (ci + 1 < p.Cin) atomicAdd(orow + ci + 1, acc[4 * i + 2 * h + 1]);
      }
    }
  }
}

typedef CUresult (*PFN_tmapEncodeTiled)(CUtensorMap*, CUtensorMapDataType, cuuint32_t, void*, const cuuint64_t*, const cuuint64_t*,
                                        const cuuint32_t*, const cuuint32_t*, CUtensorMapInterleave, CUtensorMapSwizzle,
                                        CUtensorMapL2promotion, CUtensorMapFloatOOBfill);
static PFN_tmapEncodeTiled g_encode = nullptr;
static int g_tc_state = -1;

bool tc_available() {
  if (g_tc_state >= 0) return g_tc_state == 1;
  g_tc_state = 0;
  int dev = 0, major = 0;
  if (cudaGetDevice(&dev) != cudaSuccess) return false;
  if (cudaDeviceGetAttribute(&major, cudaDevAttrComputeCapabilityMajor, dev) != cudaSuccess || major != 9) return false;
  void* fn = nullptr;
  cudaDriverEntryPointQueryResult qres;
  if (cudaGetDriverEntryPoint("cuTensorMapEncodeTiled", &fn, cudaEnableDefault, &qres) != cudaSuccess || fn == nullptr ||
      qres != cudaDriverEntryPointSuccess)
    return false;
  g_encode = (PFN_tmapEncodeTiled)fn;
  g_tc_state = 1;
  return true;
}

struct MapKey {
  const void* base; int rank; cuuint64_t dims[4]; cuuint64_t str[3]; cuuint32_t box[4];
  bool operator==(const MapKey& o) const { return memcmp(this, &o, sizeof(MapKey)) == 0; }
};
struct MapKeyHash {
  size_t operator()(const MapKey& k) const {
    const uint64_t* w = reinterpret_cast<const uint64_t*>(&k);
    uint64_t h = 1469598103934665603ull;
    for (size_t i = 0; i < sizeof(MapKey) / 8; i++) { h ^= w[i]; h *= 1099511628211ull; }
    return (size_t)h;
  }
};
static std::unordered_map<MapKey, CUtensorMap, MapKeyHash> g_map_cache;
static std::mutex g_map_mutex;

static int make_map(CUtensorMap* m, const void* base, int rank, const cuuint64_t* dims, const cuuint64_t* strides_bytes,
                    const cuuint32_t* box) {
  MapKey key;
  memset(&key, 0, sizeof(key));
  key.base = base; key.rank = rank;
  for (int i = 0; i < rank; i++) { key.dims[i] = dims[i]; key.box[i] = box[i]; }
  for (int i = 0; i + 1 < rank; i++) key.str[i] = strides_bytes[i];
  {
    std::lock_guard<std::mutex> lk(g_map_mutex);
    auto it = g_map_cache.find(key);
    if (it != g_map_cache.end()) { *m = it->second; return LO_OK; }
  }
  cuuint32_t estr[4] = {1, 1, 1, 1};
  CUresult r = g_encode(m, CU_TENSOR_MAP_DATA_TYPE_BFLOAT16, (cuuint32_t)rank, const_cast<void*>(base), dims, strides_bytes, box, estr,
                        CU_TENSOR_MAP_INTERLEAVE_NONE, CU_TENSOR_MAP_SWIZZLE_128B, CU_TENSOR_MAP_L2_PROMOTION_L2_256B,
                        CU_TENSOR_MAP_FLOAT_OOB_FILL_NONE);
  if (r != CUDA_SUCCESS) return fail(LO_ECUDA, "%s: cuTensorMapEncodeTiled failed (%ld)", "tc", (long)r);
  std::lock_guard<std::mutex> lk(g_map_mutex);
  if (g_map_cache.size() > 20000) g_map_cache.clear();
  g_map_cache.emplace(key, *m);
  return LO_OK;
}

long long* g_tc_dbg = nullptr;

template <int NT, int STAGES, int MC>
static int launch_tc(const CUtensorMap& mA, const CUtensorMap& mB, const TcParams& p, int mtiles, int splits, cudaStream_t st) {
  using SM = TcSmem<NT, STAGES>;
  static bool attr_set = false;
  if (!attr_set) {
    LO_CUDA(cudaFuncSetAttribute(tc_gemm_conv_kernel<NT, STAGES, MC>, cudaFuncAttributeMaxDynamicSharedMemorySize, SM::TOTAL));
    attr_set = true;
  }
  dim3 grid(cdiv(p.N, NT), mtiles, splits);
  cudaLaunchConfig_t cfg{};
  cfg.gridDim = grid;
  cfg.blockDim = dim3(TC_THREADS);
  cfg.dynamicSmemBytes = SM::TOTAL;
  cfg.stream = st;
  cudaLaunchAttribute attr[2];
  int n = 0;
  if (g_opt_pdl) {
    attr[n].id = cudaLaunchAttributeProgrammaticStreamSerialization;
    attr[n].val.programmaticStreamSerializationAllowed = 1;
    n++;
  }
  if (MC) {
    attr[n].id = cudaLaunchAttributeClusterDimension;
    attr[n].val.clusterDim.x = 2;
    attr[n].val.clusterDim.y = 1;
    attr[n].val.clusterDim.z = 1;
    n++;
  }
  cfg.attrs = attr;
  cfg.numAttrs = n;
  LO_CUDA(cudaLaunchKernelEx(&cfg, tc_gemm_conv_kernel<NT, STAGES, MC>, mA, mB, p));
  LO_LAUNCH_OK();
  return LO_OK;
}

static int launch_tc_any(const CUtensorMap& mA, const CUtensorMap& mB, TcParams& p, int mtiles, int splits, int nt, cudaStream_t st,
                         int mc = 0) {
  const int KB = p.K / TC_BK;
  if (splits < 1) splits = 1;
  if (splits > KB) splits = KB;
  p.kb_per_split = cdiv(KB, splits);
  splits = cdiv(KB, p.kb_per_split);
  p.atomic = splits > 1 ? 1 : p.atomic;
  if (nt == 64 && mtiles == 1 && p.kb_per_split > 4 && g_opt_skinny8) return launch_tc<64, 8, 0>(mA, mB, p, mtiles, splits, st);
  if (nt == 64) return launch_tc<64, 4, 0>(mA, mB, p, mtiles, splits, st);
  if (mc) return launch_tc<128, 3, 1>(mA, mB, p, mtiles, splits, st);
  return launch_tc<128, 3, 0>(mA, mB, p, mtiles, splits, st);
}

static TcLstmEpi g_lstm_epi;
static bool g_lstm_epi_on = false;

int tc_gemm_nt_ex(const bf16* A, int64_t lda, const bf16* W, int64_t ldw, void* C, int dtC, int64_t ldc, int M, int N, int K,
                  const float* bias, int accumulate, int relu, int splits, int atomic_acc, int small_n_tile, cudaStream_t st) {
  if (!tc_available()) return fail(LO_ENOTSUP, "%s: needs an sm_90 device", __func__);
  LO_CHECK_ARG(K % 64 == 0 && lda % 8 == 0 && ldw % 8 == 0 && ldc % 8 == 0 && ldc >= (N + 7) / 8 * 8, "K%64, ld%8, ldc >= roundup8(N)");
  LO_CHECK_ARG(((uintptr_t)A & 15) == 0 && ((uintptr_t)W & 15) == 0 && ((uintptr_t)C & 15) == 0, "16-byte alignment");
  CUtensorMap mA, mB;
  const int NT = (N <= 64 || small_n_tile) ? 64 : 128;
  const int mc = (g_opt_conv_mc && NT == 128 && cdiv(N, 128) % 2 == 0 && splits <= 1 && !atomic_acc) ? 1 : 0;
  {
    cuuint64_t dims[2] = {(cuuint64_t)K, (cuuint64_t)M};
    cuuint64_t str[1] = {(cuuint64_t)lda * 2};
    cuuint32_t box[2] = {64, (cuuint32_t)(mc ? 64 : 128)};
    LO_TRY(make_map(&mA, A, 2, dims, str, box));
  }
  {
    cuuint64_t dims[2] = {(cuuint64_t)K, (cuuint64_t)N};
    cuuint64_t str[1] = {(cuuint64_t)ldw * 2};
    cuuint32_t box[2] = {64, (cuuint32_t)NT};
    LO_TRY(make_map(&mB, W, 2, dims, str, box));
  }
  LO_CHECK_ARG(!(splits > 1 || atomic_acc) || (dtC == LO_F32 && !relu), "split-K needs fp32 output without ReLU");
  TcParams p{};
  p.M = M; p.N = N; p.K = K; p.conv = 0;
  p.bias = bias; p.mask = nullptr; p.out = C; p.ldc = ldc;
  p.out_f32 = (dtC == LO_F32); p.accumulate = accumulate; p.relu = relu; p.atomic = atomic_acc;
  p.w_evict_last = (M <= 128) ? 1 : 0;
  p.dbg = g_tc_dbg;
  if (g_lstm_epi_on) {
    const TcLstmEpi& e = g_lstm_epi;
    p.lstm = 1;
    p.l_ptab = e.ptab; p.l_tok = e.tok; p.l_tok_stride = e.tok_stride; p.l_hh = e.hh; p.l_hh_stride = e.hh_stride;
    p.l_cprev = e.c_prev; p.l_gates = e.gates; p.l_c = e.c_out; p.l_h = e.h_out; p.l_hbf = e.h_bf;
    p.l_hd = e.hd; p.l_hd_stride = e.hd_stride; p.l_dmask = e.dmask; p.l_D = e.D; p.l_V = e.V;
  }
  return launch_tc_any(mA, mB, p, cdiv(M, TC_BM), splits, NT, st, mc);
}

int tc_gemm_nt_lstm(const bf16* A, int64_t lda, const bf16* Wil, int64_t ldw, int M, int D, int K, const TcLstmEpi& e, cudaStream_t st) {
  g_lstm_epi = e;
  g_lstm_epi_on = true;
  const int r = tc_gemm_nt_ex(A, lda, Wil, ldw, e.gates , LO_F32, 4 * D, M, 4 * D, K, nullptr, 0, 0, 1, 0, 1, st);
  g_lstm_epi_on = false;
  return r;
}

int tc_gemm_nt(const bf16* A, int64_t lda, const bf16* W, int64_t ldw, void* C, int dtC, int64_t ldc, int M, int N, int K,
               const float* bias, int accumulate, int relu, cudaStream_t st) {
  return tc_gemm_nt_ex(A, lda, W, ldw, C, dtC, ldc, M, N, K, bias, accumulate, relu, 1, 0, 0, st);
}

template <int NT, int STAGES, int MT>
static int launch_conv_p(const CUtensorMap& mA, const CUtensorMap& mB, const TcParams& p, int mtiles, cudaStream_t st) {
  using SM = TcPSmem<NT, STAGES, MT>;
  static bool attr_set = false;
  static int n_sm = 0;
  if (!attr_set) {
    LO_CUDA(cudaFuncSetAttribute(tc_conv_p_kernel<NT, STAGES, MT>, cudaFuncAttributeMaxDynamicSharedMemorySize, SM::TOTAL));
    int dev = 0;
    LO_CUDA(cudaGetDevice(&dev));
    LO_CUDA(cudaDeviceGetAttribute(&n_sm, cudaDevAttrMultiProcessorCount, dev));
    attr_set = true;
  }
  const int ntn = cdiv(p.N, NT);
  const int total = cdiv(mtiles, MT) * ntn;
  const int grid = total < n_sm ? total : n_sm;
  LO_CUDA(launch_pdl(tc_conv_p_kernel<NT, STAGES, MT>, dim3(grid), dim3(TC_THREADS), (size_t)SM::TOTAL, st, mA, mB, p, ntn, total, mtiles));
  LO_LAUNCH_OK();
  return LO_OK;
}

int tc_conv3x3(const bf16* x, const bf16* w, const float* bias, const bf16* mask, bf16* y, int N, int H, int W, int Cin, int Cout,
               int pad, int relu, cudaStream_t st) {
  if (!tc_available()) return fail(LO_ENOTSUP, "%s: needs an sm_90 device", __func__);
  LO_CHECK_ARG(Cin % 64 == 0 && Cout % 8 == 0, "Cin%64==0, Cout%8==0");
  const int Ho = H + 2 * pad - 2, Wo = W + 2 * pad - 2;
  int BW = 128;
  while (BW > 8 && BW / 2 >= Wo) BW /= 2;
  const int BH = 128 / BW;
  if (g_opt_conv_persist) {
    const int NTp = Cout % 256 == 0 ? 256 : (Cout > 64 ? 128 : 64);
    CUtensorMap mA, mB;
    {
      cuuint64_t dims[4] = {(cuuint64_t)Cin, (cuuint64_t)W, (cuuint64_t)H, (cuuint64_t)N};
      cuuint64_t str[3] = {(cuuint64_t)Cin * 2, (cuuint64_t)W * Cin * 2, (cuuint64_t)H * W * Cin * 2};
      cuuint32_t box[4] = {64, (cuuint32_t)BW, (cuuint32_t)BH, 1};
      LO_TRY(make_map(&mA, x, 4, dims, str, box));
    }
    {
      cuuint64_t dims[2] = {(cuuint64_t)9 * Cin, (cuuint64_t)Cout};
      cuuint64_t str[1] = {(cuuint64_t)9 * Cin * 2};
      cuuint32_t box[2] = {64, (cuuint32_t)NTp};
      LO_TRY(make_map(&mB, w, 2, dims, str, box));
    }
    TcParams p{};
    p.M = N * Ho * Wo; p.N = Cout; p.K = 9 * Cin; p.conv = 1;
    p.Ho = Ho; p.Wo = Wo; p.Cin = Cin; p.pad = pad;
    p.BW = BW; p.BH = BH; p.tiles_w = cdiv(Wo, BW); p.tiles_h = cdiv(Ho, BH);
    p.bias = bias; p.mask = mask; p.out = y; p.ldc = Cout; p.relu = relu;
    const int mtiles = N * p.tiles_w * p.tiles_h;
    if (NTp == 256) return launch_conv_p<256, 4, 1>(mA, mB, p, mtiles, st);
    if (NTp == 128) return g_opt_conv_mt2 ? launch_conv_p<128, 4, 2>(mA, mB, p, mtiles, st) : launch_conv_p<128, 6, 1>(mA, mB, p, mtiles, st);
    return g_opt_conv_mt2 ? launch_conv_p<64, 4, 2>(mA, mB, p, mtiles, st) : launch_conv_p<64, 8, 1>(mA, mB, p, mtiles, st);
  }
  CUtensorMap mA, mB;
  const int NT = Cout <= 64 ? 64 : 128;
  const int mc = (g_opt_conv_mc && NT == 128 && cdiv(Cout, 128) % 2 == 0) ? 1 : 0;
  const int hbw = mc ? (BH >= 2 ? BW : BW / 2) : BW, hbh = mc ? (BH >= 2 ? BH / 2 : 1) : BH;
  {
    cuuint64_t dims[4] = {(cuuint64_t)Cin, (cuuint64_t)W, (cuuint64_t)H, (cuuint64_t)N};
    cuuint64_t str[3] = {(cuuint64_t)Cin * 2, (cuuint64_t)W * Cin * 2, (cuuint64_t)H * W * Cin * 2};
    cuuint32_t box[4] = {64, (cuuint32_t)hbw, (cuuint32_t)hbh, 1};
    LO_TRY(make_map(&mA, x, 4, dims, str, box));
  }
  {
    cuuint64_t dims[2] = {(cuuint64_t)9 * Cin, (cuuint64_t)Cout};
    cuuint64_t str[1] = {(cuuint64_t)9 * Cin * 2};
    cuuint32_t box[2] = {64, (cuuint32_t)NT};
    LO_TRY(make_map(&mB, w, 2, dims, str, box));
  }
  TcParams p{};
  p.M = N * Ho * Wo; p.N = Cout; p.K = 9 * Cin; p.conv = 1;
  p.Ho = Ho; p.Wo = Wo; p.Cin = Cin; p.pad = pad;
  p.BW = BW; p.BH = BH; p.tiles_w = cdiv(Wo, BW); p.tiles_h = cdiv(Ho, BH);
  p.bias = bias; p.mask = mask; p.out = y; p.ldc = Cout;
  p.out_f32 = 0; p.accumulate = 0; p.relu = relu;
  p.dbg = g_tc_dbg;
  p.half_w = (mc && BH < 2) ? BW / 2 : 0;
  p.half_h = (mc && BH >= 2) ? BH / 2 : 0;
  const int mtiles = N * p.tiles_w * p.tiles_h;
  LO_CHECK_ARG(mtiles <= 65535, "too many M tiles for grid.y");
  return launch_tc_any(mA, mB, p, mtiles, 1, NT, st, mc);
}


template <int NT, int STAGES>
static int launch_wgrad(const CUtensorMap& mDY, const CUtensorMap& mX, const WgParams& p, dim3 grid, cudaStream_t st) {
  constexpr int TOTAL = STAGES * (2 + NT / 64) * 16384 + 1024 + 256;
  static bool attr_set = false;
  if (!attr_set) {
    LO_CUDA(cudaFuncSetAttribute(tc_wgrad_kernel<NT, STAGES>, cudaFuncAttributeMaxDynamicSharedMemorySize, TOTAL));
    attr_set = true;
  }
  if (p.ordered)
    LO_CUDA(launch_cluster(tc_wgrad_kernel<NT, STAGES>, grid, dim3(TC_THREADS), (size_t)TOTAL, st, dim3(1, 1, grid.z), false, mDY, mX, p));
  else
    tc_wgrad_kernel<NT, STAGES><<<grid, TC_THREADS, TOTAL, st>>>(mDY, mX, p);
  LO_LAUNCH_OK();
  return LO_OK;
}

int tc_conv3x3_wgrad(const bf16* x, const bf16* dy, float* dw, int N, int H, int W, int Cin, int Cout, int pad, cudaStream_t st) {
  if (!tc_available()) return fail(LO_ENOTSUP, "%s: needs an sm_90 device", __func__);
  LO_CHECK_ARG(Cin % 64 == 0 && Cout % 128 == 0, "Cin%64==0, Cout%128==0");
  const int Ho = H + 2 * pad - 2, Wo = W + 2 * pad - 2;
  int BW = 128;
  while (BW > 8 && BW / 2 >= Wo) BW /= 2;
  const int BH = 128 / BW;
  CUtensorMap mDY, mX;
  {
    cuuint64_t dims[4] = {(cuuint64_t)Cout, (cuuint64_t)Wo, (cuuint64_t)Ho, (cuuint64_t)N};
    cuuint64_t str[3] = {(cuuint64_t)Cout * 2, (cuuint64_t)Wo * Cout * 2, (cuuint64_t)Ho * Wo * Cout * 2};
    cuuint32_t box[4] = {64, (cuuint32_t)BW, (cuuint32_t)BH, 1};
    LO_TRY(make_map(&mDY, dy, 4, dims, str, box));
  }
  {
    cuuint64_t dims[4] = {(cuuint64_t)Cin, (cuuint64_t)W, (cuuint64_t)H, (cuuint64_t)N};
    cuuint64_t str[3] = {(cuuint64_t)Cin * 2, (cuuint64_t)W * Cin * 2, (cuuint64_t)H * W * Cin * 2};
    cuuint32_t box[4] = {64, (cuuint32_t)BW, (cuuint32_t)BH, 1};
    LO_TRY(make_map(&mX, x, 4, dims, str, box));
  }
  WgParams p{};
  p.Cin = Cin; p.Cout = Cout; p.Ho = Ho; p.Wo = Wo; p.pad = pad;
  p.BW = BW; p.BH = BH; p.tiles_w = cdiv(Wo, BW); p.tiles_h = cdiv(Ho, BH);
  p.kstages = N * p.tiles_w * p.tiles_h;
  p.dw = dw;
  const int NT = (g_opt_wgrad256 && Cin % 256 == 0) ? 256 : (Cin >= 128 ? 128 : 64);
  p.ci_tiles = Cin / NT;
  const int tiles = (Cout / 128) * p.ci_tiles * 9;
  int splits = cdiv(NT == 256 ? LO_NUM_SMS : LO_NUM_SMS * 2, tiles);
  if (g_opt_det && splits > 8) splits = 8;
  if (splits > p.kstages) splits = p.kstages;
  if (splits < 1) splits = 1;
  p.per_split = cdiv(p.kstages, splits);
  splits = cdiv(p.kstages, p.per_split);
  p.ordered = g_opt_det && splits > 1;
  dim3 grid((Cout / 128) * p.ci_tiles, 9, splits);
  if (NT == 256) return launch_wgrad<256, 2>(mDY, mX, p, grid, st);
  if (NT == 128) return launch_wgrad<128, 3>(mDY, mX, p, grid, st);
  return launch_wgrad<64, 4>(mDY, mX, p, grid, st);
}

int tc_gemm_tn(const bf16* A, int64_t lda, const bf16* B, int64_t ldb, float* C, int64_t ldc, int M, int N, int K, cudaStream_t st) {
  if (!tc_available()) return fail(LO_ENOTSUP, "%s: needs an sm_90 device", __func__);
  LO_CHECK_ARG(lda % 8 == 0 && ldb % 8 == 0, "lda%8, ldb%8");
  LO_CHECK_ARG(((uintptr_t)A & 15) == 0 && ((uintptr_t)B & 15) == 0, "16-byte alignment");
  CUtensorMap mA, mB;
  {
    cuuint64_t dims[2] = {(cuuint64_t)M, (cuuint64_t)K};
    cuuint64_t str[1] = {(cuuint64_t)lda * 2};
    cuuint32_t box[2] = {64, 128};
    LO_TRY(make_map(&mA, A, 2, dims, str, box));
  }
  {
    cuuint64_t dims[2] = {(cuuint64_t)N, (cuuint64_t)K};
    cuuint64_t str[1] = {(cuuint64_t)ldb * 2};
    cuuint32_t box[2] = {64, 128};
    LO_TRY(make_map(&mB, B, 2, dims, str, box));
  }
  WgParams p{};
  p.plain = 1; p.Cout = M; p.Cin = N; p.dw = C; p.ldc = ldc;
  p.tiles_w = p.tiles_h = 1; p.BW = 128; p.BH = 1;
  p.kstages = cdiv(K, 128);
  const int NT = N > 64 ? 128 : 64;
  p.ci_tiles = cdiv(N, NT);
  const int mt = cdiv(M, 128);
  const int tiles = mt * p.ci_tiles;
  int splits = cdiv(LO_NUM_SMS * 2, tiles);
  if (g_opt_det && splits > 8) splits = 8;
  if (splits > p.kstages) splits = p.kstages;
  if (splits < 1) splits = 1;
  p.per_split = cdiv(p.kstages, splits);
  splits = cdiv(p.kstages, p.per_split);
  p.ordered = g_opt_det && splits > 1;
  dim3 grid(mt * p.ci_tiles, 1, splits);
  if (NT == 128) return launch_wgrad<128, 3>(mA, mB, p, grid, st);
  return launch_wgrad<64, 4>(mA, mB, p, grid, st);
}

int tc_gemm_tn_batched(const bf16* A, int64_t sAk, int64_t sAb, const bf16* B, int64_t sBk, int64_t sBb, float* C, int64_t ldc,
                       int64_t sCb, int M, int N, int K, int batch, cudaStream_t st) {
  if (!tc_available()) return fail(LO_ENOTSUP, "%s: needs an sm_90 device", __func__);
  LO_CHECK_ARG(sAk % 8 == 0 && sAb % 8 == 0 && sBk % 8 == 0 && sBb % 8 == 0, "strides must be multiples of 8 elements");
  LO_CHECK_ARG(((uintptr_t)A & 15) == 0 && ((uintptr_t)B & 15) == 0 && batch >= 1 && batch <= 65535, "alignment / batch");
  CUtensorMap mA, mB;
  {
    cuuint64_t dims[3] = {(cuuint64_t)M, (cuuint64_t)K, (cuuint64_t)batch};
    cuuint64_t str[2] = {(cuuint64_t)sAk * 2, (cuuint64_t)sAb * 2};
    cuuint32_t box[3] = {64, 128, 1};
    LO_TRY(make_map(&mA, A, 3, dims, str, box));
  }
  {
    cuuint64_t dims[3] = {(cuuint64_t)N, (cuuint64_t)K, (cuuint64_t)batch};
    cuuint64_t str[2] = {(cuuint64_t)sBk * 2, (cuuint64_t)sBb * 2};
    cuuint32_t box[3] = {64, 128, 1};
    LO_TRY(make_map(&mB, B, 3, dims, str, box));
  }
  WgParams p{};
  p.plain = 2; p.Cout = M; p.Cin = N; p.dw = C; p.ldc = ldc; p.batch_c = sCb;
  p.tiles_w = p.tiles_h = 1; p.BW = 128; p.BH = 1;
  p.kstages = cdiv(K, 128);
  p.per_split = p.kstages;
  const int NT = N > 64 ? 128 : 64;
  p.ci_tiles = cdiv(N, NT);
  dim3 grid(cdiv(M, 128) * p.ci_tiles, batch, 1);
  if (NT == 128) return launch_wgrad<128, 3>(mA, mB, p, grid, st);
  return launch_wgrad<64, 4>(mA, mB, p, grid, st);
}

}
```

### latex_ocr_b200/encoder.py

```python
import math

import torch
import torch.nn as nn

from . import _lib
from ._lib import check, dtype_code, impl_code, ptr, stream_ptr
from .kernel_module import kernel_forward, stamp
from .params import FlatStore, LRUCache, ParamHolder

_LAYERS = (("0", 1, 64, 1, (2, 2)), ("3", 64, 128, 1, (2, 2)), ("6", 128, 256, 1, None),
           ("8", 256, 256, 1, (2, 1)), ("11", 256, 512, 1, (1, 2)), ("14", 512, 512, 0, None))
_LAYERS_CNN = (("0", 1, 64, 1, (2, 2)), ("3", 64, 128, 1, (2, 2)), ("6", 128, 256, 1, None), ("8", 256, 256, 1, None),
               ("10", 256, 512, 1, None), ("12", 512, 512, 1, None, (2, 4, 2)), ("14", 512, 512, 0, None))


def _geom(layer):
    return layer[5] if len(layer) > 5 else (3, 3, 1)


def timing_signal_table(channels, height, width, device):
    nts = channels // 4
    inc = math.log(1.0e4 / 1.0) / (float(nts) - 1)
    inv = 1.0 * torch.exp(torch.arange(nts).float() * (-inc))
    table = torch.zeros(channels, height, width)
    for dim, length in enumerate((height, width)):
        st = inv.unsqueeze(1) * torch.arange(length).float().unsqueeze(0)
        sig = torch.cat([torch.sin(st), torch.cos(st)], dim=0)
        lo = dim * 2 * nts
        table[lo:lo + 2 * nts] += sig[:, :, None] if dim == 0 else sig[:, None, :]
    return table.permute(1, 2, 0).contiguous().to(device)


class EncoderCNN(nn.Module):
    def __init__(self, config, training=False, device="cuda", precision=None, impl=None):
        super().__init__()
        self._config = config
        name = getattr(config, "encoder_cnn", "vanilla")
        if name not in ("vanilla", "cnn"):
            raise NotImplementedError("encoder_cnn=%r: 'vanilla' and 'cnn' are the reference's stacks" % name)
        self.layers = _LAYERS if name == "vanilla" else _LAYERS_CNN
        self.precision = precision or getattr(config, "precision", "bf16")
        if self.precision not in ("fp32", "bf16"):
            raise NotImplementedError("precision must be 'fp32' or 'bf16'")
        self.impl = impl if impl is not None else getattr(config, "conv_impl", "tc" if self.precision == "bf16" else "simt")
        self.tdtype = torch.float32 if self.precision == "fp32" else torch.bfloat16
        self.input_norm = getattr(config, "input_norm", None)
        if self.input_norm not in (None, "tf"):
            raise NotImplementedError("input_norm=%r" % (self.input_norm,))
        specs = []
        for l in self.layers:
            idx, cin, cout = l[:3]
            R, S_, _ = _geom(l)
            specs.append(("cnn.%s.weight" % idx, (cout, R, S_, cin)))
            specs.append(("cnn.%s.bias" % idx, (cout,)))
        self.store = FlatStore(specs, device, bf16_shadow=(self.precision == "bf16"))
        self.cnn = nn.ModuleDict()
        for idx in (l[0] for l in self.layers):
            h = ParamHolder()
            h.bind("weight", self.store, "cnn.%s.weight" % idx, permute=(0, 3, 1, 2))
            h.bind("bias", self.store, "cnn.%s.bias" % idx)
            self.cnn[idx] = h
        self.reset_parameters()
        self._ws = LRUCache()

    def reset_parameters(self):
        with torch.no_grad():
            for l in self.layers:
                idx, cin = l[0], l[1]
                R, S_, _ = _geom(l)
                b = 1.0 / math.sqrt(cin * R * S_)
                self.cnn[idx].weight.uniform_(-b, b)
                self.cnn[idx].bias.uniform_(-b, b)

    def fine_tune(self, fine_tune=True):
        for p in self.cnn.parameters():
            p.requires_grad = False
        for idx in list(self.cnn.keys())[2:]:
            for p in self.cnn[idx].parameters():
                p.requires_grad = fine_tune

    def out_hw(self, H, W):
        h, w = H, W
        for l in self.layers:
            pad, pool = l[3], l[4]
            R, S_, stride = _geom(l)
            h, w = (h + 2 * pad - R) // stride + 1, (w + 2 * pad - S_) // stride + 1
            if pool:
                h, w = h // pool[0], w // pool[1]
        return h, w

    def _workspace(self, N, H, W, need_grad):
        key = (N, H, W)
        ws = self._ws.get(key)
        if ws is None:
            dev, td = self.store.device, self.tdtype
            ws = {"acts": {}, "grads": None}
            h, w = H, W
            shapes = {}
            for l in self.layers:
                idx, cin, cout, pad, pool = l[:5]
                R, S_, stride = _geom(l)
                if (R, S_, stride) != (3, 3, 1):
                    ws["col" + idx] = torch.empty(N * ((h + 2 * pad - R) // stride + 1) * ((w + 2 * pad - S_) // stride + 1), R * S_ * cin,
                                                  dtype=td, device=dev)
                h, w = (h + 2 * pad - R) // stride + 1, (w + 2 * pad - S_) // stride + 1
                if idx == "0":
                    h, w = h // 2, w // 2
                    shapes["P0"] = (N, h, w, cout)
                    continue
                shapes["Y" + idx] = (N, h, w, cout)
                if pool:
                    h, w = h // pool[0], w // pool[1]
                    shapes["P" + idx] = (N, h, w, cout)
            if h < 1 or w < 1:
                raise ValueError("image %dx%d too small for the vanilla encoder" % (H, W))
            ws["shapes"] = shapes
            for k, s in shapes.items():
                ws["acts"][k] = torch.empty(s, dtype=td, device=dev)
            ws["out"] = torch.empty(shapes["Y14"], dtype=td, device=dev)
            ws["table"] = timing_signal_table(512, shapes["Y14"][1], shapes["Y14"][2], dev)
            self._ws[key] = ws
        if need_grad and ws["grads"] is None:
            dev, td = self.store.device, self.tdtype
            ws["grads"] = {k: torch.empty(s, dtype=td, device=dev) for k, s in ws["shapes"].items()}
            ws["wflip"] = {l[0]: torch.empty(l[1] * _geom(l)[0] * _geom(l)[1] * l[2], dtype=td, device=dev)
                           for l in self.layers if l[0] != "0"}
        return ws

    def _impl(self):
        return impl_code(self.impl, self.precision)

    def forward_raw(self, img, need_grad=False):
        L = _lib.lib()
        if img.dim() != 4 or img.size(1) != 1:
            raise ValueError("img must be [N,1,H,W]")
        if not img.is_cuda:
            raise _lib.LatexOcrB200Error("EncoderCNN runs on CUDA tensors only (no CPU fallback)")
        if img.dtype != torch.uint8:
            img = img.float()
        img = img.contiguous()
        N, _, H, W = img.shape
        ws = stamp(self._workspace(N, H, W, need_grad))
        self.store.refresh_shadow()
        st, dt, impl, S = stream_ptr(), dtype_code(self.precision), self._impl(), self.store
        A = ws["acts"]
        ws["img"] = img
        sc, of = (1.0 / 128.0, -1.0) if self.input_norm == "tf" else (1.0, 0.0)
        if need_grad:
            if ws.get("code0") is None:
                ws["code0"] = torch.empty(A["P0"].shape, dtype=torch.uint8, device=img.device)
            check(L.lo_conv1_pool_forward_code(ptr(img), int(img.dtype == torch.uint8), sc, of, ptr(S.f32("cnn.0.weight")),
                                               ptr(S.f32("cnn.0.bias")), ptr(A["P0"]), ptr(ws["code0"]), dt, N, H, W, st))
        elif self.input_norm == "tf":
            check(L.lo_conv1_pool_forward_norm(ptr(img), int(img.dtype == torch.uint8), 1.0 / 128.0, -1.0, ptr(S.f32("cnn.0.weight")),
                                               ptr(S.f32("cnn.0.bias")), ptr(A["P0"]), dt, N, H, W, st))
        else:
            conv1 = L.lo_conv1_pool_forward_u8 if img.dtype == torch.uint8 else L.lo_conv1_pool_forward
            check(conv1(ptr(img), ptr(S.f32("cnn.0.weight")), ptr(S.f32("cnn.0.bias")), ptr(A["P0"]), dt, N, H, W, st))
        x = A["P0"]
        for l in self.layers[1:]:
            idx, cin, cout, pad, pool = l[:5]
            R, S_, stride = _geom(l)
            y = A["Y" + idx]
            if (R, S_, stride) == (3, 3, 1):
                check(L.lo_conv3x3(ptr(x), ptr(S.w("cnn.%s.weight" % idx)), ptr(S.f32("cnn.%s.bias" % idx)), None, ptr(y), dt,
                                   N, x.shape[1], x.shape[2], cin, cout, pad, 1, impl, st))
            else:
                col = ws["col" + idx]
                M, K = col.shape
                check(L.lo_im2col(ptr(x), ptr(col), dt, N, x.shape[1], x.shape[2], cin, R, S_, stride, pad, st))
                check(L.lo_gemm(ptr(col), dt, ptr(S.w("cnn.%s.weight" % idx)), dt, ptr(y), dt, M, cout, K, K, 1, 1, K, cout, 1, 0, 0, 0,
                                ptr(S.f32("cnn.%s.bias" % idx)), 0, 1, impl, st))
            x = y
            if pool:
                p = A["P" + idx]
                check(L.lo_maxpool_forward(ptr(y), ptr(p), dt, N, y.shape[1], y.shape[2], cout, pool[0], pool[1], st))
                x = p
        if getattr(self._config, "positional_embeddings", True):
            hwc = x.shape[1] * x.shape[2] * x.shape[3]
            check(L.lo_add_table(ptr(x), ptr(ws["table"]), ptr(ws["out"]), dt, N, hwc, st))
            return ws["out"]
        return x

    def grad_range(self, idx):
        ow, nw, _ = self.store.offsets["cnn.%s.weight" % idx]
        ob, nb, _ = self.store.offsets["cnn.%s.bias" % idx]
        return ow, ob + nb - ow

    def backward_raw(self, img_shape, denc, on_layer_grad=None, ws=None, dimg=None):
        L = _lib.lib()
        N, _, H, W = img_shape
        ws = ws if ws is not None else self._workspace(N, H, W, True)
        if dimg is not None:
            if ws.get("code0") is None:
                raise _lib.LatexOcrB200Error("EncoderCNN.backward_raw: the image gradient needs the arg-max codes of a training "
                                             "forward (forward_raw(img, need_grad=True)); this workspace has none")
            if dimg.dtype != torch.float32 or not dimg.is_contiguous() or dimg.numel() != N * H * W:
                raise ValueError("dimg must be a contiguous float32 tensor of N*H*W elements")
        st, dt, impl, S = stream_ptr(), dtype_code(self.precision), self._impl(), self.store
        A, G = ws["acts"], ws["grads"]
        for l in self.layers[1:]:
            idx, cin, cout = l[:3]
            R, S_, stride = _geom(l)
            if (R, S_, stride) == (3, 3, 1):
                check(L.lo_conv_weight_flip(ptr(S.w("cnn.%s.weight" % idx)), ptr(ws["wflip"][idx]), dt, cin, cout, st))
            else:
                check(L.lo_transpose(ptr(S.w("cnn.%s.weight" % idx)), R * S_ * cin, ptr(ws["wflip"][idx]), cout, dt, cout, R * S_ * cin, st))
        last = "Y" + self.layers[-1][0]
        y6 = A[last]
        check(L.lo_relu_mask_cast(ptr(denc), ptr(y6), ptr(G[last]), dt, y6.numel(), st))
        plan = []
        for i in range(len(self.layers) - 1, 0, -1):
            prev = self.layers[i - 1]
            plan.append((self.layers[i], ("P" if prev[4] else "Y") + prev[0]))
        cfg = {l[0]: l for l in self.layers}
        for l, xin in plan:
            idx, cin, cout, pad, pool = l[:5]
            R, S_, stride = _geom(l)
            x = A[xin]
            dy = G["Y" + idx]
            mask = A[xin] if xin.startswith("Y") else None
            if (R, S_, stride) == (3, 3, 1):
                check(L.lo_conv3x3_wgrad(ptr(x), ptr(dy), ptr(S.g("cnn.%s.weight" % idx)), ptr(S.g("cnn.%s.bias" % idx)), dt,
                                         N, x.shape[1], x.shape[2], cin, cout, pad, impl, st))
                check(L.lo_conv3x3(ptr(dy), ptr(ws["wflip"][idx]), None, ptr(mask), ptr(G[xin]), dt,
                                   N, dy.shape[1], dy.shape[2], cout, cin, 2 - pad, 0, impl, st))
            else:
                col = ws["col" + idx]
                M, K = col.shape
                check(L.lo_gemm(ptr(dy), dt, ptr(col), dt, ptr(S.g("cnn.%s.weight" % idx)), _lib.LO_F32, cout, K, M, 1, cout, K, 1, K, 1,
                                0, 0, 0, None, 0, 0, impl, st))
                check(L.lo_colsum(ptr(dy), dt, ptr(S.g("cnn.%s.bias" % idx)), M, cout, cout, 0, st))
                check(L.lo_gemm(ptr(dy), dt, ptr(ws["wflip"][idx]), dt, ptr(col), dt, M, K, cout, cout, 1, 1, cout, K, 1, 0, 0, 0, None,
                                0, 0, impl, st))
                check(L.lo_col2im(ptr(col), ptr(mask), ptr(G[xin]), dt, N, x.shape[1], x.shape[2], cin, R, S_, stride, pad, st))
            if on_layer_grad is not None:
                on_layer_grad(idx)
            if xin.startswith("P") and xin != "P0":
                src = "Y" + xin[1:]
                pool_k = cfg[xin[1:]][4]
                ysrc = A[src]
                check(L.lo_maxpool_backward(ptr(ysrc), ptr(A[xin]), ptr(G[xin]), ptr(G[src]), dt, N, ysrc.shape[1], ysrc.shape[2],
                                            ysrc.shape[3], pool_k[0], pool_k[1], st))
        sc, of = (1.0 / 128.0, -1.0) if self.input_norm == "tf" else (1.0, 0.0)
        if ws.get("code0") is not None:
            check(L.lo_conv1_pool_wgrad_code(ptr(ws["img"]), int(ws["img"].dtype == torch.uint8), sc, of, ptr(ws["code0"]), ptr(G["P0"]), dt,
                                             ptr(S.g("cnn.0.weight")), ptr(S.g("cnn.0.bias")), N, H, W, st))
        elif self.input_norm == "tf":
            check(L.lo_conv1_pool_wgrad_norm(ptr(ws["img"]), int(ws["img"].dtype == torch.uint8), 1.0 / 128.0, -1.0,
                                             ptr(S.f32("cnn.0.weight")), ptr(S.f32("cnn.0.bias")), ptr(G["P0"]), dt,
                                             ptr(S.g("cnn.0.weight")), ptr(S.g("cnn.0.bias")), N, H, W, st))
        else:
            wg1 = L.lo_conv1_pool_wgrad_u8 if ws["img"].dtype == torch.uint8 else L.lo_conv1_pool_wgrad
            check(wg1(ptr(ws["img"]), ptr(S.f32("cnn.0.weight")), ptr(S.f32("cnn.0.bias")), ptr(G["P0"]), dt,
                      ptr(S.g("cnn.0.weight")), ptr(S.g("cnn.0.bias")), N, H, W, st))
        if on_layer_grad is not None:
            on_layer_grad("0")
        if dimg is not None:
            check(L.lo_conv1_pool_dgrad_code(ptr(ws["code0"]), ptr(G["P0"]), dt, ptr(S.f32("cnn.0.weight")), sc, ptr(dimg),
                                             N, H, W, st))

    def forward(self, img):
        return kernel_forward(self, (img,), (img,))[0][0]

    def _forward_impl(self, img, need_grad):
        out = self.forward_raw(img, need_grad=need_grad)
        if not need_grad:
            return (out.float(),), None, None
        N, _, H, W = img.shape
        ws = self._ws.get((N, H, W))
        return (out.to(torch.float32, copy=True),), None, {"entries": [ws], "ws": ws, "shape": tuple(img.shape), "dtype": img.dtype}

    def _backward_impl(self, saved, dout, need):
        dimg = torch.empty(saved["shape"], dtype=torch.float32, device=dout.device) if need[0] else None
        self.backward_raw(saved["shape"], dout.float().contiguous(), ws=saved["ws"], dimg=dimg)
        return (dimg.to(saved["dtype"]) if dimg is not None else None,)
```

Baseline: 2445.

## Fuse maxpool and positional table into conv3x3 epilogues, fold mean grad into batched GEMM

Adds conv epilogue variants that apply ReLU and max-pooling in registers, writing pooled output plus a compact argmax code, and a variant that adds the positional table while storing. The backward pass uses the codes to unpool the dgrad output without rereading the pre-pool activation. The decoder folds the mean-broadcast gradient add into the batched TN GEMM epilogue. This removes several full-size activation round trips and kernel launches, at the cost of more epilogue register pressure and more kernel template instances.

After: 2484 (median of 6 runs). 1.02x the previous value.

```diff
diff --git a/include/latex_ocr_b200.h b/include/latex_ocr_b200.h
--- a/include/latex_ocr_b200.h
+++ b/include/latex_ocr_b200.h
@@ -68,6 +68,13 @@
 int lo_maxpool_forward(const void* x, void* y, int dt, int N, int H, int W, int C, int kh, int kw, void* stream);
 int lo_maxpool_backward(const void* x, const void* y, const void* dy, void* dx, int dt,
                         int N, int H, int W, int C, int kh, int kw, void* stream);
+int lo_conv3x3_pool(const void* x, const void* w, const float* bias, void* y, void* p, uint8_t* code, int dt,
+                    int N, int H, int W, int Cin, int Cout, int pad, int kh, int kw, int impl, void* stream);
+int lo_conv3x3_dgrad_unpool(const void* dy, const void* wt, const void* y, const uint8_t* code, void* dp, void* dx, int dt,
+                            int N, int H, int W, int Cin, int Cout, int pad, int Hf, int Wf, int kh, int kw, int impl,
+                            void* stream);
+int lo_conv3x3_table(const void* x, const void* w, const float* bias, void* y, const float* table, void* out, int dt,
+                     int N, int H, int W, int Cin, int Cout, int pad, int impl, void* stream);
 int lo_add_table(const void* y, const float* table, void* out, int dt, int N, int64_t HWC, void* stream);
 int lo_relu_mask_cast(const float* g, const void* y, void* out, int dt, int64_t n, void* stream);
 
diff --git a/latex_ocr_b200/csrc/lo_common.cuh b/latex_ocr_b200/csrc/lo_common.cuh
--- a/latex_ocr_b200/csrc/lo_common.cuh
+++ b/latex_ocr_b200/csrc/lo_common.cuh
@@ -318,9 +318,13 @@
                    int splits, int atomic_acc, cudaStream_t st);
 int tc_gemm_tn(const bf16* A, int64_t lda, const bf16* B, int64_t ldb, float* C, int64_t ldc, int M, int N, int K, cudaStream_t st);
 int tc_gemm_tn_batched(const bf16* A, int64_t sAk, int64_t sAb, const bf16* B, int64_t sBk, int64_t sBb, float* C, int64_t ldc,
-                       int64_t sCb, int M, int N, int K, int batch, cudaStream_t st);
+                       int64_t sCb, int M, int N, int K, int batch, const float* rowb, float rowb_scale, cudaStream_t st);
 int tc_conv3x3_wgrad(const bf16* x, const bf16* dy, float* dw, int N, int H, int W, int Cin, int Cout, int pad, cudaStream_t st);
 int tc_conv3x3(const bf16* x, const bf16* w, const float* bias, const bf16* mask, bf16* y,
                int N, int H, int W, int Cin, int Cout, int pad, int relu, cudaStream_t st);
-
-}
+int tc_conv3x3_table(const bf16* x, const bf16* w, const float* bias, bf16* y, const float* table, bf16* out, int N, int H, int W,
+                     int Cin, int Cout, int pad, int relu, cudaStream_t st);
+int tc_conv3x3_pool(const bf16* x, const bf16* w, const float* bias, bf16* p, uint8_t* code, int N, int H, int W, int Cin, int Cout,
+                    int pad, int kh, int kw, int relu, cudaStream_t st);
+
+}
diff --git a/latex_ocr_b200/csrc/lo_conv.cu b/latex_ocr_b200/csrc/lo_conv.cu
--- a/latex_ocr_b200/csrc/lo_conv.cu
+++ b/latex_ocr_b200/csrc/lo_conv.cu
@@ -524,6 +524,34 @@
         float o[8];
 #pragma unroll
         for (int c = 0; c < 8; c++) o[c] = (bi[c] == a * kw + b && best[c] > 0.f) ? g[c] : 0.f;
+        st8(dx + ((n * H + ho * kh + a) * W + wo * kw + b) * C + c8 * 8, o);
+      }
+  }
+}
+
+template <typename T>
+__global__ void unpool_code_kernel(const uint8_t* __restrict__ code, const T* __restrict__ dy, T* __restrict__ dx,
+                                   int N, int H, int W, int C, int kh, int kw) {
+  const int Ho = H / kh, Wo = W / kw, C8 = C / 8;
+  const int64_t total = (int64_t)N * Ho * Wo * C8;
+  for (int64_t idx = blockIdx.x * (int64_t)blockDim.x + threadIdx.x; idx < total; idx += (int64_t)gridDim.x * blockDim.x) {
+    const int c8 = (int)(idx % C8);
+    int64_t p = idx / C8;
+    const int wo = (int)(p % Wo); p /= Wo;
+    const int ho = (int)(p % Ho);
+    const int64_t n = p / Ho;
+    float g[8];
+    bool py[8], px[8];
+    ld8(dy + ((n * Ho + ho) * Wo + wo) * C + c8 * 8, g);
+    const uint2 cw2 = *reinterpret_cast<const uint2*>(code + ((n * Ho + ho) * Wo + wo) * C + c8 * 8);
+    const uint32_t cw[2] = {cw2.x, cw2.y};
+#pragma unroll
+    for (int c = 0; c < 8; c++) g[c] = conv1_code_decode((cw[c >> 2] >> (8 * (c & 3))) & 0xffu, g[c], py[c], px[c]);
+    for (int a = 0; a < kh; a++)
+      for (int b = 0; b < kw; b++) {
+        float o[8];
+#pragma unroll
+        for (int c = 0; c < 8; c++) o[c] = ((int)py[c] == a && (int)px[c] == b) ? g[c] : 0.f;
         st8(dx + ((n * H + ho * kh + a) * W + wo * kw + b) * C + c8 * 8, o);
       }
   }
@@ -834,6 +862,53 @@
   return LO_OK;
 }
 
+static bool pool_fused(int dt, int impl, int kh, int kw) {
+  return impl == LO_IMPL_TC && dt == LO_BF16 && g_opt_conv_persist && tc_available() &&
+         ((kh == 2 && kw == 2) || (kh == 2 && kw == 1) || (kh == 1 && kw == 2));
+}
+
+int lo_conv3x3_pool(const void* x, const void* w, const float* bias, void* y, void* p, uint8_t* code, int dt, int N, int H, int W,
+                    int Cin, int Cout, int pad, int kh, int kw, int impl, void* stream) {
+  LO_CHECK_ARG(x && w && p, "null pointer");
+  LO_CHECK_ARG(pad >= 0 && pad <= 2 && H + 2 * pad - 2 > 0 && W + 2 * pad - 2 > 0, "pad in 0..2, output would be empty");
+  cudaStream_t st = (cudaStream_t)stream;
+  const int Ho = H + 2 * pad - 2, Wo = W + 2 * pad - 2;
+  if (pool_fused(dt, impl, kh, kw))
+    return tc_conv3x3_pool((const bf16*)x, (const bf16*)w, bias, (bf16*)p, code, N, H, W, Cin, Cout, pad, kh, kw, 1, st);
+  LO_CHECK_ARG(y != nullptr, "this form needs the pre-pool map y");
+  LO_TRY(lo_conv3x3(x, w, bias, nullptr, y, dt, N, H, W, Cin, Cout, pad, 1, impl, stream));
+  return lo_maxpool_forward(y, p, dt, N, Ho, Wo, Cout, kh, kw, stream);
+}
+
+int lo_conv3x3_dgrad_unpool(const void* dy, const void* wt, const void* y, const uint8_t* code, void* dp, void* dx, int dt, int N, int H,
+                            int W, int Cin, int Cout, int pad, int Hf, int Wf, int kh, int kw, int impl, void* stream) {
+  LO_CHECK_ARG(dy && wt && dx, "null pointer");
+  LO_CHECK_ARG(pad >= 0 && pad <= 2 && H + 2 * pad - 2 > 0 && W + 2 * pad - 2 > 0, "pad in 0..2, output would be empty");
+  cudaStream_t st = (cudaStream_t)stream;
+  const bool fused = pool_fused(dt, impl, kh, kw);
+  LO_CHECK_ARG(dp && (fused ? code != nullptr : y != nullptr), "needs dp, and the codes of lo_conv3x3_pool (fused) or y");
+  LO_CHECK_ARG(Hf / kh == H + 2 * pad - 2 && Wf / kw == W + 2 * pad - 2 && Cout % 8 == 0, "pre-pool map does not pool to dp");
+  LO_TRY(lo_conv3x3(dy, wt, nullptr, nullptr, dp, dt, N, H, W, Cin, Cout, pad, 0, impl, stream));
+  if (!fused) return lo_maxpool_backward(y, nullptr, dp, dx, dt, N, Hf, Wf, Cout, kh, kw, stream);
+  if (Hf % kh || Wf % kw) LO_CUDA(cudaMemsetAsync(dx, 0, (size_t)N * Hf * Wf * Cout * sizeof(bf16), st));
+  const int64_t total = (int64_t)N * (Hf / kh) * (Wf / kw) * (Cout / 8);
+  unpool_code_kernel<bf16><<<grid_for(total, 256), 256, 0, st>>>(code, (const bf16*)dp, (bf16*)dx, N, Hf, Wf, Cout, kh, kw);
+  LO_LAUNCH_OK();
+  return LO_OK;
+}
+
+int lo_conv3x3_table(const void* x, const void* w, const float* bias, void* y, const float* table, void* out, int dt, int N, int H,
+                     int W, int Cin, int Cout, int pad, int impl, void* stream) {
+  LO_CHECK_ARG(x && w && y && table && out, "null pointer");
+  LO_CHECK_ARG(pad >= 0 && pad <= 2 && H + 2 * pad - 2 > 0 && W + 2 * pad - 2 > 0, "pad in 0..2, output would be empty");
+  const int Ho = H + 2 * pad - 2, Wo = W + 2 * pad - 2;
+  if (impl == LO_IMPL_TC && dt == LO_BF16 && g_opt_conv_persist && tc_available())
+    return tc_conv3x3_table((const bf16*)x, (const bf16*)w, bias, (bf16*)y, table, (bf16*)out, N, H, W, Cin, Cout, pad, 1,
+                            (cudaStream_t)stream);
+  LO_TRY(lo_conv3x3(x, w, bias, nullptr, y, dt, N, H, W, Cin, Cout, pad, 1, impl, stream));
+  return lo_add_table(y, table, out, dt, N, (int64_t)Ho * Wo * Cout, stream);
+}
+
 int lo_add_table(const void* y, const float* table, void* out, int dt, int N, int64_t HWC, void* stream) {
   LO_CHECK_ARG(y && table && out && HWC % 8 == 0, "shape");
   cudaStream_t st = (cudaStream_t)stream;
diff --git a/latex_ocr_b200/csrc/lo_decoder.cu b/latex_ocr_b200/csrc/lo_decoder.cu
--- a/latex_ocr_b200/csrc/lo_decoder.cu
+++ b/latex_ocr_b200/csrc/lo_decoder.cu
@@ -1891,6 +1891,9 @@
     LO_TRY(gemm_nn(a->datt1, dt, d.A, a->w_enc_att, dt, d.C, a->denc, LO_F32, d.C, d.B * d.R, d.C, d.A, 0, LO_IMPL_SIMT, st));
   }
   LO_TRY(colsum(a->datt1, dt, a->g_b_enc_att, d.B * d.R, d.A, d.A, 0, st));
+  LO_TRY(gemm_tn(a->dinit, LO_F32, 2 * d.D, a->mean, LO_F32, d.C, a->g_w_init, LO_F32, d.C, 2 * d.D, d.C, d.B, 0, LO_IMPL_SIMT, st));
+  LO_TRY(colsum(a->dinit, LO_F32, a->g_b_init, d.B, 2 * d.D, 2 * d.D, 0, st));
+  LO_TRY(gemm_nn(a->dinit, LO_F32, 2 * d.D, a->w_init, dt, d.C, a->dmean, LO_F32, d.C, d.B, d.C, 2 * d.D, 0, LO_IMPL_SIMT, st));
   if (tc && d.C % 8 == 0) {
     const int Rp = (int)rpad8(d.R);
     cast_pad_rows_kernel<<<LO_NUM_SMS * 8, 256, 0, st>>>(a->alphas, bv.alphas, BT, d.R, Rp);
@@ -1898,15 +1901,10 @@
     cast_tb_to_bt_kernel<<<LO_NUM_SMS * 8, 256, 0, st>>>(a->dctx, bv.dctx, d.T, d.B, d.C);
     LO_LAUNCH_OK();
     LO_TRY(tc_gemm_tn_batched(bv.alphas, Rp, (int64_t)d.T * Rp, bv.dctx, d.C, (int64_t)d.T * d.C, a->denc, d.C, (int64_t)d.R * d.C, d.R,
-                              d.C, d.T, d.B, st));
+                              d.C, d.T, d.B, a->dmean, 1.0f / (float)d.R, st));
   } else {
     GemmDesc g{d.R, d.C, d.T, 1, d.R, (int64_t)d.B * d.C, 1, d.C, d.B, (int64_t)d.T * d.R, d.C, (int64_t)d.R * d.C, nullptr, 1, 0};
     LO_TRY(gemm(a->alphas, LO_F32, a->dctx, LO_F32, a->denc, LO_F32, g, LO_IMPL_SIMT, st));
-  }
-  LO_TRY(gemm_tn(a->dinit, LO_F32, 2 * d.D, a->mean, LO_F32, d.C, a->g_w_init, LO_F32, d.C, 2 * d.D, d.C, d.B, 0, LO_IMPL_SIMT, st));
-  LO_TRY(colsum(a->dinit, LO_F32, a->g_b_init, d.B, 2 * d.D, 2 * d.D, 0, st));
-  LO_TRY(gemm_nn(a->dinit, LO_F32, 2 * d.D, a->w_init, dt, d.C, a->dmean, LO_F32, d.C, d.B, d.C, 2 * d.D, 0, LO_IMPL_SIMT, st));
-  {
     const int64_t total = (int64_t)d.B * d.R * d.C;
     add_rowbcast_kernel<<<LO_NUM_SMS * 8, 256, 0, st>>>(a->denc, a->dmean, d.R, d.C, 1.0f / (float)d.R, total);
     LO_LAUNCH_OK();
diff --git a/latex_ocr_b200/csrc/lo_tc.cu b/latex_ocr_b200/csrc/lo_tc.cu
--- a/latex_ocr_b200/csrc/lo_tc.cu
+++ b/latex_ocr_b200/csrc/lo_tc.cu
@@ -97,7 +97,15 @@
   const float* l_cprev; float* l_gates; float* l_c; float* l_h; bf16* l_hbf;
   float* l_hd; int64_t l_hd_stride; const float* l_dmask;
   int l_D, l_V;
+  int pool_h, pool_w;
+  uint8_t* code;
+  const float* table;
+  bf16* out2;
 };
+
+constexpr int TC_EPI_PLAIN = 0;
+constexpr int TC_EPI_POOL = 1;
+constexpr int TC_EPI_TABLE = 2;
 
 constexpr int TC_BM = 128, TC_BK = 64;
 constexpr int TC_CWARPS = 8;
@@ -327,7 +335,72 @@
   static constexpr int TOTAL = STAGES * STAGE_BYTES + 1024  + 256  + 2 * NT * 4 ;
 };
 
-template <int NT, int STAGES, int MT>
+template <int NM>
+__device__ __forceinline__ void tc_pool_window(const uint32_t (&v)[NM], const uint32_t (&wcode)[NM], uint32_t& out, uint32_t& code) {
+  out = 0;
+  code = 0;
+#pragma unroll
+  for (int k = 0; k < 2; k++) {
+    uint32_t bb = (v[0] >> (16 * k)) & 0xffffu, cd = wcode[0];
+    float best = __uint_as_float(bb << 16);
+#pragma unroll
+    for (int m = 1; m < NM; m++) {
+      const uint32_t b = (v[m] >> (16 * k)) & 0xffffu;
+      const float f = __uint_as_float(b << 16);
+      if (f > best) { best = f; bb = b; cd = wcode[m]; }
+    }
+    out |= bb << (16 * k);
+    code |= (cd | (best > 0.f ? 4u : 0u)) << (8 * k);
+  }
+}
+
+template <int NT, int KH, int KW>
+__device__ __forceinline__ void tc_pool_store(const TcParams& p, const float* acc, const float* sb, int n0, int img, int th0, int tw0,
+                                              int rbase, int cq, int lane) {
+  constexpr int NWIN = KH == 2 ? 1 : 2;
+  const int Hp = p.Ho / KH, Wp = p.Wo / KW;
+  const bool lead = KW == 1 || !(lane & 4);
+  int64_t off[NWIN];
+#pragma unroll
+  for (int h = 0; h < NWIN; h++) {
+    const int row = rbase + 8 * h;
+    const int hp = (th0 + row / p.BW) / KH, wp = (tw0 + row % p.BW) / KW;
+    off[h] = (lead && hp < Hp && wp < Wp) ? (((int64_t)img * Hp + hp) * Wp + wp) * p.ldc + n0 + cq : -1;
+  }
+#pragma unroll
+  for (int i = 0; i < NT / 8; i++) {
+    if (n0 + 8 * i >= p.N) continue;
+    const int c = 8 * i + cq;
+    uint32_t v[2], u[2];
+#pragma unroll
+    for (int h = 0; h < 2; h++) {
+      float f0 = acc[4 * i + 2 * h] + sb[c], f1 = acc[4 * i + 2 * h + 1] + sb[c + 1];
+      if (p.relu) { f0 = fmaxf(f0, 0.f); f1 = fmaxf(f1, 0.f); }
+      __nv_bfloat162 hv = __floats2bfloat162_rn(f0, f1);
+      v[h] = *reinterpret_cast<uint32_t*>(&hv);
+      if (KW == 2) u[h] = __shfl_xor_sync(0xffffffffu, v[h], 4);
+    }
+#pragma unroll
+    for (int h = 0; h < NWIN; h++) {
+      if (off[h] < 0) continue;
+      uint32_t o, cd;
+      if (KH == 2 && KW == 2) {
+        const uint32_t win[4] = {v[0], u[0], v[1], u[1]}, wc[4] = {0u, 1u, 2u, 3u};
+        tc_pool_window<4>(win, wc, o, cd);
+      } else if (KH == 2) {
+        const uint32_t win[2] = {v[0], v[1]}, wc[2] = {0u, 2u};
+        tc_pool_window<2>(win, wc, o, cd);
+      } else {
+        const uint32_t win[2] = {v[h], u[h]}, wc[2] = {0u, 1u};
+        tc_pool_window<2>(win, wc, o, cd);
+      }
+      *reinterpret_cast<uint32_t*>(reinterpret_cast<bf16*>(p.out) + off[h] + 8 * i) = o;
+      if (p.code) *reinterpret_cast<uint16_t*>(p.code + off[h] + 8 * i) = (uint16_t)cd;
+    }
+  }
+}
+
+template <int NT, int STAGES, int MT, int EPI>
 __global__ void __launch_bounds__(TC_THREADS, 1) tc_conv_p_kernel(const __grid_constant__ CUtensorMap mapA,
                                                                  const __grid_constant__ CUtensorMap mapB, TcParams p, int ntiles_n,
                                                                  int total_tiles, int mtiles) {
@@ -439,6 +512,13 @@
         if (j >= nsub) continue;
         const int mt = mt0 + j;
         const int img = mt / per_img, rem = mt % per_img;
+        if constexpr (EPI == TC_EPI_POOL) {
+          const int th0 = (rem / p.tiles_w) * p.BH, tw0 = (rem % p.tiles_w) * p.BW;
+          if (p.pool_h == 2 && p.pool_w == 2) tc_pool_store<NT, 2, 2>(p, acc[j], sb, n0, img, th0, tw0, rbase, cq, lane);
+          else if (p.pool_h == 2) tc_pool_store<NT, 2, 1>(p, acc[j], sb, n0, img, th0, tw0, rbase, cq, lane);
+          else tc_pool_store<NT, 1, 2>(p, acc[j], sb, n0, img, th0, tw0, rbase, cq, lane);
+          continue;
+        }
 #pragma unroll
         for (int h = 0; h < 2; h++) {
           const int row = rbase + 8 * h;
@@ -458,6 +538,11 @@
             }
             __nv_bfloat162 hv = __floats2bfloat162_rn(f0, f1);
             *reinterpret_cast<__nv_bfloat162*>(reinterpret_cast<bf16*>(p.out) + row_off + n0 + c) = hv;
+            if constexpr (EPI == TC_EPI_TABLE) {
+              const float2 t = *reinterpret_cast<const float2*>(p.table + ((int64_t)hh * p.Wo + ww) * p.ldc + n0 + c);
+              *reinterpret_cast<__nv_bfloat162*>(p.out2 + row_off + n0 + c) =
+                  __floats2bfloat162_rn(__low2float(hv) + t.x, __high2float(hv) + t.y);
+            }
           }
         }
       }
@@ -482,6 +567,8 @@
   int64_t ldc;
   int64_t batch_c;
   int ordered;
+  const float* rowb;
+  float rowb_scale;
 };
 
 template <int NT, int STAGES>
@@ -602,6 +689,16 @@
       const int co = co0 + wg * 64 + (warp & 3) * 16 + (lane >> 2) + 8 * h;
       if (co >= p.Cout) continue;
       float* orow = p.plain ? p.dw + (int64_t)bz * p.batch_c + (int64_t)co * p.ldc : p.dw + ((int64_t)co * 9 + tap) * p.Cin;
+      if (p.rowb) {
+        const float* rb = p.rowb + (int64_t)bz * p.Cin;
+#pragma unroll
+        for (int i = 0; i < NT / 8; i++) {
+          const int ci = ci0 + 8 * i + cq;
+          if (ci < p.Cin) orow[ci] = fmaf(rb[ci], p.rowb_scale, orow[ci] + acc[4 * i + 2 * h]);
+          if (ci + 1 < p.Cin) orow[ci + 1] = fmaf(rb[ci + 1], p.rowb_scale, orow[ci + 1] + acc[4 * i + 2 * h + 1]);
+        }
+        continue;
+      }
 #pragma unroll
       for (int i = 0; i < NT / 8; i++) {
         const int ci = ci0 + 8 * i + cq;
@@ -776,13 +873,13 @@
   return tc_gemm_nt_ex(A, lda, W, ldw, C, dtC, ldc, M, N, K, bias, accumulate, relu, 1, 0, 0, st);
 }
 
-template <int NT, int STAGES, int MT>
+template <int NT, int STAGES, int MT, int EPI = TC_EPI_PLAIN>
 static int launch_conv_p(const CUtensorMap& mA, const CUtensorMap& mB, const TcParams& p, int mtiles, cudaStream_t st) {
   using SM = TcPSmem<NT, STAGES, MT>;
   static bool attr_set = false;
   static int n_sm = 0;
   if (!attr_set) {
-    LO_CUDA(cudaFuncSetAttribute(tc_conv_p_kernel<NT, STAGES, MT>, cudaFuncAttributeMaxDynamicSharedMemorySize, SM::TOTAL));
+    LO_CUDA(cudaFuncSetAttribute(tc_conv_p_kernel<NT, STAGES, MT, EPI>, cudaFuncAttributeMaxDynamicSharedMemorySize, SM::TOTAL));
     int dev = 0;
     LO_CUDA(cudaGetDevice(&dev));
     LO_CUDA(cudaDeviceGetAttribute(&n_sm, cudaDevAttrMultiProcessorCount, dev));
@@ -791,9 +888,77 @@
   const int ntn = cdiv(p.N, NT);
   const int total = cdiv(mtiles, MT) * ntn;
   const int grid = total < n_sm ? total : n_sm;
-  LO_CUDA(launch_pdl(tc_conv_p_kernel<NT, STAGES, MT>, dim3(grid), dim3(TC_THREADS), (size_t)SM::TOTAL, st, mA, mB, p, ntn, total, mtiles));
+  LO_CUDA(launch_pdl(tc_conv_p_kernel<NT, STAGES, MT, EPI>, dim3(grid), dim3(TC_THREADS), (size_t)SM::TOTAL, st, mA, mB, p, ntn, total,
+                     mtiles));
   LO_LAUNCH_OK();
   return LO_OK;
+}
+
+static int conv_p_setup(const bf16* x, const bf16* w, int N, int H, int W, int Cin, int Cout, int pad, int BW, CUtensorMap* mA,
+                        CUtensorMap* mB, TcParams* p, int* ntp) {
+  const int Ho = H + 2 * pad - 2, Wo = W + 2 * pad - 2, BH = 128 / BW;
+  const int NTp = Cout % 256 == 0 ? 256 : (Cout > 64 ? 128 : 64);
+  {
+    cuuint64_t dims[4] = {(cuuint64_t)Cin, (cuuint64_t)W, (cuuint64_t)H, (cuuint64_t)N};
+    cuuint64_t str[3] = {(cuuint64_t)Cin * 2, (cuuint64_t)W * Cin * 2, (cuuint64_t)H * W * Cin * 2};
+    cuuint32_t box[4] = {64, (cuuint32_t)BW, (cuuint32_t)BH, 1};
+    LO_TRY(make_map(mA, x, 4, dims, str, box));
+  }
+  {
+    cuuint64_t dims[2] = {(cuuint64_t)9 * Cin, (cuuint64_t)Cout};
+    cuuint64_t str[1] = {(cuuint64_t)9 * Cin * 2};
+    cuuint32_t box[2] = {64, (cuuint32_t)NTp};
+    LO_TRY(make_map(mB, w, 2, dims, str, box));
+  }
+  *p = TcParams{};
+  p->M = N * Ho * Wo; p->N = Cout; p->K = 9 * Cin; p->conv = 1;
+  p->Ho = Ho; p->Wo = Wo; p->Cin = Cin; p->pad = pad;
+  p->BW = BW; p->BH = BH; p->tiles_w = cdiv(Wo, BW); p->tiles_h = cdiv(Ho, BH);
+  p->ldc = Cout;
+  *ntp = NTp;
+  return LO_OK;
+}
+
+template <int EPI>
+static int launch_conv_p_epi(const CUtensorMap& mA, const CUtensorMap& mB, const TcParams& p, int NTp, cudaStream_t st) {
+  const int mtiles = p.M / (p.Ho * p.Wo) * p.tiles_w * p.tiles_h;
+  if (NTp == 256) return launch_conv_p<256, 4, 1, EPI>(mA, mB, p, mtiles, st);
+  if (NTp == 128) return launch_conv_p<128, 4, 2, EPI>(mA, mB, p, mtiles, st);
+  return launch_conv_p<64, 4, 2, EPI>(mA, mB, p, mtiles, st);
+}
+
+int tc_conv3x3_pool(const bf16* x, const bf16* w, const float* bias, bf16* pout, uint8_t* code, int N, int H, int W, int Cin, int Cout,
+                    int pad, int kh, int kw, int relu, cudaStream_t st) {
+  if (!tc_available()) return fail(LO_ENOTSUP, "%s: needs an sm_90 device", __func__);
+  LO_CHECK_ARG(Cin % 64 == 0 && Cout % 8 == 0, "Cin%64==0, Cout%8==0");
+  LO_CHECK_ARG((kh == 2 && kw == 2) || (kh == 2 && kw == 1) || (kh == 1 && kw == 2), "pool window (2,2), (2,1) or (1,2)");
+  const int Ho = H + 2 * pad - 2, Wo = W + 2 * pad - 2;
+  LO_CHECK_ARG(Ho >= kh && Wo >= kw, "pooled map would be empty");
+  int BW = 128;
+  while (BW > 8 && BW / 2 >= Wo) BW /= 2;
+  if (kh == 2) BW = 8;
+  CUtensorMap mA, mB;
+  TcParams p;
+  int NTp;
+  LO_TRY(conv_p_setup(x, w, N, H, W, Cin, Cout, pad, BW, &mA, &mB, &p, &NTp));
+  p.bias = bias; p.out = pout; p.relu = relu;
+  p.pool_h = kh; p.pool_w = kw; p.code = code;
+  return launch_conv_p_epi<TC_EPI_POOL>(mA, mB, p, NTp, st);
+}
+
+int tc_conv3x3_table(const bf16* x, const bf16* w, const float* bias, bf16* y, const float* table, bf16* out, int N, int H, int W,
+                     int Cin, int Cout, int pad, int relu, cudaStream_t st) {
+  if (!tc_available()) return fail(LO_ENOTSUP, "%s: needs an sm_90 device", __func__);
+  LO_CHECK_ARG(Cin % 64 == 0 && Cout % 8 == 0, "Cin%64==0, Cout%8==0");
+  const int Wo = W + 2 * pad - 2;
+  int BW = 128;
+  while (BW > 8 && BW / 2 >= Wo) BW /= 2;
+  CUtensorMap mA, mB;
+  TcParams p;
+  int NTp;
+  LO_TRY(conv_p_setup(x, w, N, H, W, Cin, Cout, pad, BW, &mA, &mB, &p, &NTp));
+  p.bias = bias; p.out = y; p.relu = relu; p.table = table; p.out2 = out;
+  return launch_conv_p_epi<TC_EPI_TABLE>(mA, mB, p, NTp, st);
 }
 
 int tc_conv3x3(const bf16* x, const bf16* w, const float* bias, const bf16* mask, bf16* y, int N, int H, int W, int Cin, int Cout,
@@ -805,25 +970,11 @@
   while (BW > 8 && BW / 2 >= Wo) BW /= 2;
   const int BH = 128 / BW;
   if (g_opt_conv_persist) {
-    const int NTp = Cout % 256 == 0 ? 256 : (Cout > 64 ? 128 : 64);
     CUtensorMap mA, mB;
-    {
-      cuuint64_t dims[4] = {(cuuint64_t)Cin, (cuuint64_t)W, (cuuint64_t)H, (cuuint64_t)N};
-      cuuint64_t str[3] = {(cuuint64_t)Cin * 2, (cuuint64_t)W * Cin * 2, (cuuint64_t)H * W * Cin * 2};
-      cuuint32_t box[4] = {64, (cuuint32_t)BW, (cuuint32_t)BH, 1};
-      LO_TRY(make_map(&mA, x, 4, dims, str, box));
-    }
-    {
-      cuuint64_t dims[2] = {(cuuint64_t)9 * Cin, (cuuint64_t)Cout};
-      cuuint64_t str[1] = {(cuuint64_t)9 * Cin * 2};
-      cuuint32_t box[2] = {64, (cuuint32_t)NTp};
-      LO_TRY(make_map(&mB, w, 2, dims, str, box));
-    }
-    TcParams p{};
-    p.M = N * Ho * Wo; p.N = Cout; p.K = 9 * Cin; p.conv = 1;
-    p.Ho = Ho; p.Wo = Wo; p.Cin = Cin; p.pad = pad;
-    p.BW = BW; p.BH = BH; p.tiles_w = cdiv(Wo, BW); p.tiles_h = cdiv(Ho, BH);
-    p.bias = bias; p.mask = mask; p.out = y; p.ldc = Cout; p.relu = relu;
+    TcParams p;
+    int NTp;
+    LO_TRY(conv_p_setup(x, w, N, H, W, Cin, Cout, pad, BW, &mA, &mB, &p, &NTp));
+    p.bias = bias; p.mask = mask; p.out = y; p.relu = relu;
     const int mtiles = N * p.tiles_w * p.tiles_h;
     if (NTp == 256) return launch_conv_p<256, 4, 1>(mA, mB, p, mtiles, st);
     if (NTp == 128) return g_opt_conv_mt2 ? launch_conv_p<128, 4, 2>(mA, mB, p, mtiles, st) : launch_conv_p<128, 6, 1>(mA, mB, p, mtiles, st);
@@ -955,7 +1106,7 @@
 }
 
 int tc_gemm_tn_batched(const bf16* A, int64_t sAk, int64_t sAb, const bf16* B, int64_t sBk, int64_t sBb, float* C, int64_t ldc,
-                       int64_t sCb, int M, int N, int K, int batch, cudaStream_t st) {
+                       int64_t sCb, int M, int N, int K, int batch, const float* rowb, float rowb_scale, cudaStream_t st) {
   if (!tc_available()) return fail(LO_ENOTSUP, "%s: needs an sm_90 device", __func__);
   LO_CHECK_ARG(sAk % 8 == 0 && sAb % 8 == 0 && sBk % 8 == 0 && sBb % 8 == 0, "strides must be multiples of 8 elements");
   LO_CHECK_ARG(((uintptr_t)A & 15) == 0 && ((uintptr_t)B & 15) == 0 && batch >= 1 && batch <= 65535, "alignment / batch");
@@ -974,6 +1125,7 @@
   }
   WgParams p{};
   p.plain = 2; p.Cout = M; p.Cin = N; p.dw = C; p.ldc = ldc; p.batch_c = sCb;
+  p.rowb = rowb; p.rowb_scale = rowb_scale;
   p.tiles_w = p.tiles_h = 1; p.BW = 128; p.BH = 1;
   p.kstages = cdiv(K, 128);
   p.per_split = p.kstages;
diff --git a/latex_ocr_b200/encoder.py b/latex_ocr_b200/encoder.py
--- a/latex_ocr_b200/encoder.py
+++ b/latex_ocr_b200/encoder.py
@@ -158,10 +158,25 @@
             conv1 = L.lo_conv1_pool_forward_u8 if img.dtype == torch.uint8 else L.lo_conv1_pool_forward
             check(conv1(ptr(img), ptr(S.f32("cnn.0.weight")), ptr(S.f32("cnn.0.bias")), ptr(A["P0"]), dt, N, H, W, st))
         x = A["P0"]
+        positional = getattr(self._config, "positional_embeddings", True)
         for l in self.layers[1:]:
             idx, cin, cout, pad, pool = l[:5]
             R, S_, stride = _geom(l)
             y = A["Y" + idx]
+            if (R, S_, stride) == (3, 3, 1) and pool:
+                p, code = A["P" + idx], None
+                if need_grad:
+                    code = ws.get("code" + idx)
+                    if code is None:
+                        code = ws["code" + idx] = torch.empty(p.shape, dtype=torch.uint8, device=img.device)
+                check(L.lo_conv3x3_pool(ptr(x), ptr(S.w("cnn.%s.weight" % idx)), ptr(S.f32("cnn.%s.bias" % idx)), ptr(y), ptr(p),
+                                        ptr(code), dt, N, x.shape[1], x.shape[2], cin, cout, pad, pool[0], pool[1], impl, st))
+                x = p
+                continue
+            if (R, S_, stride) == (3, 3, 1) and not pool and l is self.layers[-1] and positional:
+                check(L.lo_conv3x3_table(ptr(x), ptr(S.w("cnn.%s.weight" % idx)), ptr(S.f32("cnn.%s.bias" % idx)), ptr(y),
+                                         ptr(ws["table"]), ptr(ws["out"]), dt, N, x.shape[1], x.shape[2], cin, cout, pad, impl, st))
+                return ws["out"]
             if (R, S_, stride) == (3, 3, 1):
                 check(L.lo_conv3x3(ptr(x), ptr(S.w("cnn.%s.weight" % idx)), ptr(S.f32("cnn.%s.bias" % idx)), None, ptr(y), dt,
                                    N, x.shape[1], x.shape[2], cin, cout, pad, 1, impl, st))
@@ -176,7 +191,7 @@
                 p = A["P" + idx]
                 check(L.lo_maxpool_forward(ptr(y), ptr(p), dt, N, y.shape[1], y.shape[2], cout, pool[0], pool[1], st))
                 x = p
-        if getattr(self._config, "positional_embeddings", True):
+        if positional:
             hwc = x.shape[1] * x.shape[2] * x.shape[3]
             check(L.lo_add_table(ptr(x), ptr(ws["table"]), ptr(ws["out"]), dt, N, hwc, st))
             return ws["out"]
@@ -220,11 +235,18 @@
             x = A[xin]
             dy = G["Y" + idx]
             mask = A[xin] if xin.startswith("Y") else None
+            pooled = xin.startswith("P") and xin != "P0"
             if (R, S_, stride) == (3, 3, 1):
                 check(L.lo_conv3x3_wgrad(ptr(x), ptr(dy), ptr(S.g("cnn.%s.weight" % idx)), ptr(S.g("cnn.%s.bias" % idx)), dt,
                                          N, x.shape[1], x.shape[2], cin, cout, pad, impl, st))
-                check(L.lo_conv3x3(ptr(dy), ptr(ws["wflip"][idx]), None, ptr(mask), ptr(G[xin]), dt,
-                                   N, dy.shape[1], dy.shape[2], cout, cin, 2 - pad, 0, impl, st))
+                if pooled:
+                    src, pool_k = "Y" + xin[1:], cfg[xin[1:]][4]
+                    check(L.lo_conv3x3_dgrad_unpool(ptr(dy), ptr(ws["wflip"][idx]), ptr(A[src]), ptr(ws.get("code" + xin[1:])),
+                                                    ptr(G[xin]), ptr(G[src]), dt, N, dy.shape[1], dy.shape[2], cout, cin, 2 - pad,
+                                                    A[src].shape[1], A[src].shape[2], pool_k[0], pool_k[1], impl, st))
+                else:
+                    check(L.lo_conv3x3(ptr(dy), ptr(ws["wflip"][idx]), None, ptr(mask), ptr(G[xin]), dt,
+                                       N, dy.shape[1], dy.shape[2], cout, cin, 2 - pad, 0, impl, st))
             else:
                 col = ws["col" + idx]
                 M, K = col.shape
@@ -236,7 +258,7 @@
                 check(L.lo_col2im(ptr(col), ptr(mask), ptr(G[xin]), dt, N, x.shape[1], x.shape[2], cin, R, S_, stride, pad, st))
             if on_layer_grad is not None:
                 on_layer_grad(idx)
-            if xin.startswith("P") and xin != "P0":
+            if pooled and (R, S_, stride) != (3, 3, 1):
                 src = "Y" + xin[1:]
                 pool_k = cfg[xin[1:]][4]
                 ysrc = A[src]
```
